# HugoVuach/Dense-linear-app

Measured on AMD Instinct MI355X. Metric: fp64 TFLOP/s for NxN SPD Cholesky (N^3/3 flops / factorisation time), higher is better.
Workload: dtype f64

## Files before the change

### dense_linear_app_amd/_lib.py

```python
from __future__ import annotations

import ctypes as C
import os

_HERE = os.path.dirname(os.path.abspath(__file__))
LIB_PATH = os.environ.get("LIBCHOLMI_PATH") or os.path.join(_HERE, "libcholmi.so")

_lib = None


class CholmiError(RuntimeError):

    def __init__(self, fn: str, code: int, msg: str):
        super().__init__(f"{fn} failed with status {code}: {msg}")
        self.fn, self.code, self.msg = fn, code, msg


def lib() -> C.CDLL:
    global _lib
    if _lib is not None:
        return _lib
    if not os.path.exists(LIB_PATH):
        raise ImportError(
            f"{LIB_PATH} is missing: build it with `python -c 'import __graft_entry__ as g; g.build()'` "
# ... 14 lines not shown
        "chol_desc_destroy": ([pp], i),
        "chol_potrf_tile": ([i, vp], i),
        "chol_trsm_tile": ([i, i, i, i, d, vp, vp], i),
        "chol_syrk_tile": ([i, i, d, vp, d, vp], i),
        "chol_gemm_tile": ([i, i, d, vp, vp, d, vp], i),
        "chol_plgsy_tile": ([d, i, vp, u64], i),
        "chol_lacpy_tile": ([i, vp, vp], i),
        "chol_lange_tile": ([i, vp, C.POINTER(d)], i),
        "chol_lauum_tile": ([i, vp], i),
        "chol_geadd_tile": ([i, d, vp, d, vp], i),
        "chol_potrs_tile": ([i, vp, vp], i),
        "chol_posv_tile": ([i, vp, vp], i),
        "chol_dsposv_tile": ([i, vp, vp, vp, C.POINTER(i)], i),
        "chol_last_dsposv_stats": ([C.POINTER(d)], i),
        "chol_trtri_tile": ([i, i, vp], i),
        "chol_potri_tile": ([i, vp], i),
        "chol_poinv_tile": ([i, vp], i),
        "chol_lansy_tile": ([i, i, vp, C.POINTER(d)], i),
        "chol_pocon_tile": ([i, vp, d, C.POINTER(d)], i),
        "chol_last_pocon_stats": ([C.POINTER(d)], i),
        "chol_poequ_tile": ([vp, vp, C.POINTER(d), C.POINTER(d)], i),
        "chol_laqsy_tile": ([i, vp, vp, d, d, C.POINTER(i)], i),
        "chol_porfs_tile": ([i, vp, vp, vp, vp, C.POINTER(d), C.POINTER(d)], i),
        "chol_posvx_tile": ([i, i, vp, vp, C.POINTER(i), vp, vp, vp, C.POINTER(d), C.POINTER(d), C.POINTER(d)], i),
        "chol_last_posvx_stats": ([C.POINTER(d)], i),
        "chol_bench_refine": ([i, vp, vp, vp, i, i, C.POINTER(d)], i),
        "chol_pstrf_tile": ([i, vp, C.POINTER(i), C.POINTER(i), d], i),
        "chol_last_pstrf_stats": ([C.POINTER(d)], i),
        "chol_sygst_tile": ([i, i, vp, vp], i),
        "chol_last_sygst_stats": ([C.POINTER(d)], i),
        "chol_sytrf_nopiv_tile": ([i, vp], i),
        "chol_sytrs_nopiv_tile": ([i, vp, vp], i),
        "chol_sysv_nopiv_tile": ([i, vp, vp], i),
        "chol_last_sytrf_stats": ([C.POINTER(d)], i),
        "chol_rbt_apply_tile": ([i, vp, vp, i], i),
        "chol_sytrf_rbt_tile": ([i, vp, vp, i, u64], i),
        "chol_sytrs_rbt_tile": ([i, vp, vp, i, vp], i),
        "chol_sysv_rbt_tile": ([i, vp, vp, vp, i, u64, vp, vp, C.POINTER(i), C.POINTER(d)], i),
        "chol_last_rbt_stats": ([C.POINTER(d)], i),
        "chol_lapack_to_tile": ([vp, i, vp], i),
        "chol_tile_to_lapack": ([vp, vp, i], i),
        "chol_tile_upload": ([vp, i, i, vp], i),
        "chol_tile_download": ([vp, i, i, vp], i),
        "chol_residual_plgsy": ([vp, d, u64, C.POINTER(d)], i),
        "chol_residual_plgsy_inf": ([vp, d, u64, C.POINTER(d)], i),
        "chol_make_spd_like_chameleon": ([vp, i, i, d, C.c_char, u64], None),
        "chol_enforce_strict_diag_dominance": ([vp, i, i, d], None),
        "chol_extract_block": ([vp, i, i, i, i, i, vp], None),
        "chol_parse_payloads": ([C.c_char_p, vp, i, vp, vp, vp, vp], i),
        "chol_debug_flow_waves": ([], i),
        "chol_last_potrf_regimes": ([C.POINTER(i), C.POINTER(i)], i),
        "chol_debug_schedule_check": ([i, i, d, d, i, C.c_char_p, i], i),
        "chol_debug_schedule_check_grid": ([i, i, i, i, i, d, d, i, C.c_char_p, i], i),
        "chol_debug_comm_trace": ([i, i, i, i, i, d, d, C.c_char_p, i], i),
        "chol_debug_task_record": ([i, i], i),
        "chol_debug_task_check": ([C.POINTER(C.c_longlong)], i),
        "chol_last_potrf_stats": ([C.POINTER(d), C.POINTER(d), C.POINTER(i), C.POINTER(d)], i),
        "chol_set_profiling": ([i], i),
        "chol_debug_stamps": ([i, C.POINTER(C.c_ulonglong), i], i),
        "chol_mfma_probe": ([i, i, C.POINTER(d)], i),
        "chol_bench_update": ([vp, i, i, i, C.POINTER(d), C.POINTER(d)], i),
        "chol_desc_local_ptr": ([vp, C.POINTER(C.c_size_t)], vp),
        "chol_desc_local_tiles": ([vp, C.POINTER(i), C.POINTER(i)], i),
        "chol_set_transport": ([vp], i),
        "chol_transport_rccl_unique_id": ([vp], i),
        "chol_transport_rccl_init": ([vp, i, i], i),
        "chol_transport_rccl_finalize": ([], i),
        "chol_transport_rccl_version": ([], i),
        "chol_set_transport_channel": ([i, vp], i),
        "chol_transport_selftest": ([i, C.c_size_t], i),
        "chol_set_transport_null": ([], i),
        "chol_dist_rehearse": ([i, i, i, i, i, d, u64, vp, C.POINTER(d)], i),
        "chol_desc_set_version": ([vp, u64], i),
        "chol_tile_batch": ([i, i, i, i, vp, vp, vp, vp, vp, i], i),
        "chol_sync": ([], i),
        "chol_potrf_batch": ([i, i, i, vp, vp, vp, C.POINTER(i), i], i),
        "chol_batch_info": ([i, C.POINTER(i)], i),
        "chol_batch_stats": ([C.POINTER(C.c_longlong)], i),
        "chol_batch_mark": ([C.POINTER(C.c_ulonglong)], i),
        "chol_batch_wait": ([C.POINTER(C.c_ulonglong)], i),
        "chol_debug_calibration": ([C.POINTER(d)], i),
        "chol_debug_update_kernel": ([i, C.c_char_p, i], i),
        "chol_debug_device_counters": ([], i),
        "chol_dist_last_stats": ([C.POINTER(d), C.POINTER(C.c_longlong), C.POINTER(C.c_longlong), C.POINTER(C.c_longlong)], i),
        "chol_dist_factorize_with": ([vp, vp, i, i, i, i, i, i], i),
        "chol_dist_gather_lower": ([vp, vp, i], i),
    }
    for name, (argt, rest) in sig.items():
        try:
            fn = getattr(L, name)
        except AttributeError:
            if os.environ.get("LIBCHOLMI_PATH"):
                continue
            raise
        fn.argtypes = argt
        fn.restype = rest
    _lib = L
    return L


ABI_SYMBOLS = None


def abi_symbols() -> list[str]:
    import re

    hdr = os.path.join(_HERE, "..", "include", "cholmi.h")
    text = open(hdr).read()
    text = re.sub(r"/\*.*?\*/", "", text, flags=re.S)
    return sorted(set(re.findall(r"\b(chol_[a-z_0-9]+)\s*\(", text)))


def check(fn: str, code: int) -> int:
    if code < 0:
        raise CholmiError(fn, code, lib().chol_last_error().decode(errors="replace"))
    return code
```

### dense_linear_app_amd/csrc/api.hip

```cpp
#include <hip/hip_runtime.h>

#include <algorithm>
#include <array>
#include <cmath>
#include <cstdarg>
#include <cstdio>
#include <cstdlib>
#include <cstring>
#include <deque>
#include <mutex>
#include <string>
#include <unordered_map>
#include <vector>

#include "../../include/cholmi.h"
#include "api_internal.h"
#include "cholmi_internal.h"

using namespace cholmi;

extern "C" int chol_internal_walk(chol_desc *d, void *base, cholmi::RankCtx *r, int rank);
extern "C" void chol_internal_dist_finalize(void);
extern "C" int chol_internal_desc_create(chol_desc_t **desc, void *mat, int dtype, int mb, int nb, int bsiz, int lm, int ln,
                                         int i, int j, int m, int n, int p, int q, int my_rank, int nranks);
// ... 651 lines not shown
  return through_lower(true, {A},
                       [&] { return A->dtype == CHOL_REAL_DOUBLE ? potrf_impl<double>(A) : potrf_impl<float>(A); });
}

void *DevPool::get(size_t bytes) {
  for (auto &b : blks)
    if (!b.used && b.bytes >= bytes) {
      b.used = true;
      return b.p;
    }
  void *p = nullptr;
  if (hipMalloc(&p, bytes) != hipSuccess) {
    (void)hipGetLastError();
    return nullptr;
  }
  blks.push_back({p, bytes, true});
  return p;
}
void DevPool::free_all() {
  for (auto &b : blks) (void)hipFree(b.p);
  blks.clear();
}

RankCtx *main_rank_ctx() { return &g.r; }
int main_rank(int *nranks) {
  if (nranks) *nranks = g.nranks;
  return g.rank;
}

int rank_ctx_create(RankCtx *r, int device, const RankCtx *calib_from) {
  r->device = device;
  int lo = 0, hi = 0;
  HIPCHECK(hipDeviceGetStreamPriorityRange(&lo, &hi));
  HIPCHECK(hipStreamCreateWithPriority(&r->st[ST_MAIN], hipStreamNonBlocking, lo));
  HIPCHECK(hipStreamCreateWithPriority(&r->st[ST_PANEL], hipStreamNonBlocking, hi));
  HIPCHECK(hipStreamCreateWithPriority(&r->st[ST_TRSM], hipStreamNonBlocking, hi));
  HIPCHECK(hipStreamCreateWithPriority(&r->st[ST_U1], hipStreamNonBlocking, lo - 1 > hi ? lo - 1 : hi));
  HIPCHECK(hipStreamCreateWithPriority(&r->st[ST_CX], hipStreamNonBlocking, hi));
  HIPCHECK(hipStreamCreateWithPriority(&r->st[ST_PX], hipStreamNonBlocking, hi));
  {
    {
      hipDeviceProp_t prop;
      HIPCHECK(hipGetDeviceProperties(&prop, device));
      unsigned long long *t = nullptr;
      HIPCHECK(hipMalloc(&t, 64));
      auto blocked = [&](int big, int small, bool *out) -> int {
        HIPCHECK(hipMemset(t, 0, 64));
        cholmi::launch_pipe_probe(r->st[big], r->st[small], t, prop.multiProcessorCount);
        HIPCHECK(hipStreamSynchronize(r->st[big]));
        HIPCHECK(hipStreamSynchronize(r->st[small]));
        unsigned long long h[2];
        HIPCHECK(hipMemcpy(h, t, sizeof h, hipMemcpyDeviceToHost));
        *out = h[1] > h[0] + 3000;
        return 0;
      };
      const int victims[4] = {ST_PANEL, ST_TRSM, ST_CX, ST_U1};
      const int mid = lo - 1 > hi ? lo - 1 : hi;
      const int prio_of[ST_COUNT] = {lo, hi, hi, mid, hi, hi};
      for (int vi = 0; vi < 4; ++vi) {
        const int v = victims[vi];
        for (int attempt = 0;; ++attempt) {
          bool b1 = false, b2 = false;
          int rc = blocked(ST_MAIN, v, &b1);
          if (rc) return rc;
          if (v != ST_U1) rc = blocked(ST_U1, v, &b2);
          if (rc) return rc;
          if (!b1 && !b2) break;
          if (attempt == 6) {
            ++r->stream_collisions;
            break;
          }
          r->retired.push_back(r->st[v]);
          HIPCHECK(hipStreamCreateWithPriority(&r->st[v], hipStreamNonBlocking, prio_of[v]));
          ++r->stream_swaps;
        }
      }
      (void)hipFree(t);
      if (getenv("CHOLMI_VERBOSE"))
        fprintf(stderr, "[cholmi] stream pipe probe: %d stream(s) replaced, %d pair(s) still colliding\n", r->stream_swaps, r->stream_collisions);
    }
  }
  r->winv_bytes = (size_t)32 * MACRO * MACRO * sizeof(double);
  HIPCHECK(hipMalloc(&r->winv, 2 * r->winv_bytes));
  HIPCHECK(hipMalloc(&r->d_info, sizeof(int)));
  HIPCHECK(hipMemset(r->d_info, 0, sizeof(int)));
  {
    const char *e = getenv("CHOLMI_DEVICE_FLAGS");
    if (!e || atoi(e) != 0) {
      HIPCHECK(hipMalloc(&r->d_sem, SEM_INTS * sizeof(int)));
      HIPCHECK(hipMemset(r->d_sem, 0, SEM_INTS * sizeof(int)));
      bool ok = true;
      const hipStream_t pairs[4][2] = {{r->st[ST_TRSM], r->st[ST_PANEL]}, {r->st[ST_U1], r->st[ST_TRSM]},
                                       {r->st[ST_PANEL], r->st[ST_U1]}, {r->st[ST_PANEL], r->st[ST_TRSM]}};
      for (int t = 0; t < 4 && ok; ++t) {
        int *sem = r->d_sem + 64 * t, *res = r->d_sem + 64 * t + 32;
        cholmi::launch_sem_probe(pairs[t][0], pairs[t][1], sem, res);
        HIPCHECK(hipStreamSynchronize(pairs[t][0]));
        HIPCHECK(hipStreamSynchronize(pairs[t][1]));
        int v = 0;
        HIPCHECK(hipMemcpy(&v, res, sizeof(int), hipMemcpyDeviceToHost));
        ok = (v == 1);
      }
      if (!ok) {
        (void)hipFree(r->d_sem);
        r->d_sem = nullptr;
      } else {
        r->flow_ok = true;
        const hipStream_t fpairs[2][2] = {{r->st[ST_CX], r->st[ST_PANEL]}, {r->st[ST_PANEL], r->st[ST_CX]}};
        for (int t = 0; t < 2 && r->flow_ok; ++t) {
          int *sem = r->d_sem + 64 * (4 + t), *res = r->d_sem + 64 * (4 + t) + 32;
          cholmi::launch_sem_probe(fpairs[t][0], fpairs[t][1], sem, res);
          HIPCHECK(hipStreamSynchronize(fpairs[t][0]));
          HIPCHECK(hipStreamSynchronize(fpairs[t][1]));
          int v = 0;
          HIPCHECK(hipMemcpy(&v, res, sizeof(int), hipMemcpyDeviceToHost));
          r->flow_ok = (v == 1);
        }
        HIPCHECK(hipMemset(r->d_sem, 0, 1024 * sizeof(int)));
      }
    }
  }
  if (calib_from) {
    for (int i = 0; i < 2; ++i) r->probe_tflops[i] = calib_from->probe_tflops[i], r->diag_us[i] = calib_from->diag_us[i];
    return 0;
  }
  if (const char *e = getenv("CHOLMI_CALIB")) {
    double v[4];
    if (sscanf(e, "%lf,%lf,%lf,%lf", &v[0], &v[1], &v[2], &v[3]) == 4) {
      r->probe_tflops[0] = v[0], r->diag_us[0] = v[1], r->probe_tflops[1] = v[2], r->diag_us[1] = v[3];
      return 0;
    }
  }
  int rc = mfma_probe_on(r, CHOL_REAL_DOUBLE, 4, 1000, &r->probe_tflops[0]);
  if (!rc) rc = mfma_probe_on(r, CHOL_REAL_FLOAT, 4, 2000, &r->probe_tflops[1]);
  if (!rc) rc = time_diag_step<double>(r, &r->diag_us[0]);
  if (!rc) rc = time_diag_step<float>(r, &r->diag_us[1]);
  return rc;
}

void rank_ctx_destroy(RankCtx *r) {
  for (auto e : r->events) (void)hipEventDestroy(e);
  r->events.clear();
  if (r->ev_flow) (void)hipEventDestroy(r->ev_flow);
  r->ev_flow = nullptr;
  r->pool.free_all();
  if (r->winv) (void)hipFree(r->winv);
  if (r->d_info) (void)hipFree(r->d_info);
  if (r->d_sem) (void)hipFree(r->d_sem);
  r->winv = nullptr;
  r->d_info = nullptr;
  r->d_sem = nullptr;
  for (int i = 0; i < ST_COUNT; ++i) {
    if (r->st[i]) (void)hipStreamDestroy(r->st[i]);
    r->st[i] = nullptr;
  }
  for (hipStream_t s : r->retired) (void)hipStreamDestroy(s);
  r->retired.clear();
}

}

extern "C" {

int chol_internal_fail(int code, const char *msg) { return fail(code, msg); }

const char *chol_version(void) { return "cholmi 0.3 (gfx950)"; }

const char *chol_last_error(void) {
  static thread_local std::string copy;
  std::lock_guard<std::mutex> lk(g_err_mu);
  copy = g.last_error;
  return copy.c_str();
}

int chol_set_device(int device) {
  std::lock_guard<std::recursive_mutex> lk(g_mu);
  if (g.inited && device != g.r.device) return fail(-1, "chol_set_device after chol_init");
  g.r.device = device;
  return 0;
}

int chol_set_rank(int rank, int nranks) {
  if (nranks < 1 || rank < 0 || rank >= nranks) return fail(-1, "chol_set_rank: bad rank");
  g.rank = rank;
  g.nranks = nranks;
  return 0;
}

int chol_init(int ncpu, int ngpu) {
  (void)ncpu;
  std::lock_guard<std::recursive_mutex> lk(g_mu);
  if (g.inited) return 0;
  if (ngpu < 1)
    return fail(CHOL_ERR_NO_GPU, "chol_init: ngpu must be >= 1 (this library has no CPU backend)");
  int count = 0;
  hipError_t e = hipGetDeviceCount(&count);
  if (e != hipSuccess || count < 1) {
    (void)hipGetLastError();
    return fail(CHOL_ERR_NO_GPU, "chol_init: no HIP device visible");
  }
  if (g.r.device < 0) {
    const char *lr = getenv("LOCAL_RANK");
    g.r.device = lr ? atoi(lr) % count : 0;
  }
  if (g.r.device >= count) return fail(CHOL_ERR_NO_GPU, "chol_init: device index out of range");
  HIPCHECK(hipSetDevice(g.r.device));
  if (const char *e = getenv("CHOLMI_TRSM_SMALL_MAX")) cholmi::g_trsm_small_max = atoi(e);
  {
    hipDeviceProp_t prop;
    HIPCHECK(hipGetDeviceProperties(&prop, g.r.device));
    const int room = (prop.multiProcessorCount - 32) / 4;
    cholmi::g_poll_max_wgs = room < 0 ? 0 : (room < 48 ? room : 48);
  }
  if (const char *e = getenv("CHOLMI_POLL_MAX_WGS")) cholmi::g_poll_max_wgs = atoi(e);
  if (const char *e = getenv("CHOLMI_FLOW")) cholmi::g_flow = atoi(e);
  if (const char *e = getenv("CHOLMI_FLOW_NBM")) {
    int lo = 0, hi = 0;
    if (sscanf(e, "%d:%d", &lo, &hi) == 2) cholmi::g_flow_min_nbm = std::max(2, lo), cholmi::g_flow_max_nbm = std::min(8, hi);
  }
  if (const char *e = getenv("CHOLMI_FLOW_FENCES")) cholmi::g_flow_fences = atoi(e);
  if (const char *e = getenv("CHOLMI_INTILE_FUSED")) cholmi::g_intile_fused = atoi(e);
  if (const char *e = getenv("CHOLMI_MIN_UNITS")) cholmi::g_min_units = atoi(e);
  HIPCHECK(hipMalloc(&g.d_acc, 2 * sizeof(double)));
  HIPCHECK(hipMalloc(&g.d_ytab, YTAB_ENTRIES * sizeof(int)));
  HIPCHECK(hipMemset(g.d_ytab, 0, YTAB_ENTRIES * sizeof(int)));
  cholmi::g_ytab = g.d_ytab;
  int rc = rank_ctx_create(&g.r, g.r.device, nullptr);
  if (rc) return rc;
  g.inited = true;
  return 0;
}

int chol_finalize(void) {
  std::lock_guard<std::recursive_mutex> lk(g_mu);
  if (!g.inited) return 0;
  (void)hipDeviceSynchronize();
  chol_internal_dist_finalize();
  g.stage.release();
  g.work.release();
  spd_release();
  if (g.wc_winv) (void)hipFree(g.wc_winv);
  g.wc_winv = nullptr;
  if (g.d_binfo) (void)hipFree(g.d_binfo);
  g.d_binfo = nullptr;
  tx_destroy();
  g.wc_ptr = nullptr;
  g.wc_version = 0;
  (void)hipFree(g.d_acc);
  if (g.d_ytab) (void)hipFree(g.d_ytab);
  g.d_ytab = nullptr;
  cholmi::g_ytab = nullptr;
  rank_ctx_destroy(&g.r);
  g.d_acc = nullptr;
  g.inited = false;
  return 0;
}

int chol_desc_create(chol_desc_t **desc, void *mat, int dtype, int mb, int nb, int bsiz, int lm,
                     int ln, int i, int j, int m, int n, int p, int q) {
  return chol_internal_desc_create(desc, mat, dtype, mb, nb, bsiz, lm, ln, i, j, m, n, p, q, g.rank, g.nranks);
}

int chol_internal_desc_create(chol_desc_t **desc, void *mat, int dtype, int mb, int nb, int bsiz, int lm, int ln,
                              int i, int j, int m, int n, int p, int q, int my_rank, int nranks) {
  if (!desc) return fail(-1, "desc_create: desc is NULL");
  *desc = nullptr;
  if (dtype != CHOL_REAL_DOUBLE && dtype != CHOL_REAL_FLOAT) return fail(-3, "desc_create: dtype");
  if (mb <= 0) return fail(-4, "desc_create: mb");
  if (nb <= 0) return fail(-5, "desc_create: nb");
  if (bsiz != mb * nb) return fail(-6, "desc_create: bsiz != mb*nb");
  if (lm <= 0) return fail(-7, "desc_create: lm");
  if (ln <= 0) return fail(-8, "desc_create: ln");
  if (i < 0 || i >= lm) return fail(-9, "desc_create: i");
  if (j < 0 || j >= ln) return fail(-10, "desc_create: j");
  if (m <= 0 || i + m > lm) return fail(-11, "desc_create: m");
  if (n <= 0 || j + n > ln) return fail(-12, "desc_create: n");
  if (p <= 0 || p > MAXP) return fail(-13, "desc_create: p");
  if (q <= 0) return fail(-14, "desc_create: q");
  if (!g.inited) return fail(CHOL_ERR_NOT_INITIALIZED, "desc_create before chol_init");
  void *view_user = nullptr;
  int view_lmt = 0, view_oi = 0, view_oj = 0;
  if (i != 0 || j != 0 || m != lm || n != ln) {
    if (p * q != 1) return fail(CHOL_ERR_NOT_SUPPORTED, "desc_create: sub-matrix views of distributed matrices are not supported");
    if (mat) {
      if (lm % mb || ln % nb || mb != nb)
        return fail(CHOL_ERR_NOT_SUPPORTED, "desc_create: a view over a user buffer needs a user matrix of whole square tiles (lm, ln multiples of mb = nb)");
      view_user = mat;
      view_lmt = lm / mb;
      view_oi = i;
      view_oj = j;
// ... 62 lines not shown
  if (multi || d->padded) {
    int rc = build_worklist(d);
    if (rc) {
      if (d->owns) (void)hipFree(d->mat);
      delete d;
      return rc;
    }
  }
  d->user_mat = view_user;
  d->user_lmt = view_lmt;
  d->user_i = view_oi;
  d->user_j = view_oj;
  *desc = d;
  return 0;
}

int chol_desc_destroy(chol_desc_t **desc) {
  if (!desc || !*desc) return fail(-1, "desc_destroy: NULL");
  chol_desc *d = *desc;
  if (d->owns) forget_winv(d->mat);
  if (d->d_list) (void)hipFree(d->d_list);
  if (d->owns && d->mat) (void)hipFree(d->mat);
  delete d;
  *desc = nullptr;
  return 0;
}

void *chol_desc_local_ptr(chol_desc_t *d, size_t *bytes) {
  if (!d) return nullptr;
  if (bytes) *bytes = (size_t)d->lmt * d->lnt * (size_t)d->bsizi * d->esize;
  return d->mat;
}

int chol_desc_local_tiles(chol_desc_t *d, int *lmt, int *lnt) {
  if (!d) return fail(-1, "NULL desc");
  if (lmt) *lmt = d->lmt;
  if (lnt) *lnt = d->lnt;
  return 0;
}

int chol_desc_set_version(chol_desc_t *d, unsigned long long version) {
  if (!d) return fail(-1, "desc_set_version: NULL descriptor");
  d->version = version;
  return 0;
}

int chol_sync(void) {
  if (tx_rec.on) {
    std::lock_guard<std::recursive_mutex> lk(g_mu);
    return tx_quiesce();
  }
  if (!g.inited) return fail(CHOL_ERR_NOT_INITIALIZED, "chol_sync before chol_init");
  std::lock_guard<std::recursive_mutex> lk(g_mu);
  HIPCHECK(hipStreamSynchronize(g.r.st[ST_MAIN]));
  return tx_quiesce();
}

}


template <typename T>
static int flush_pending_t() {
  const TaskExec::Pending p = tx.pend;
  tx.pend.on = false;
  hipStream_t s = tx.st[TaskExec::CHAIN];
  TXHIP(hipMemsetAsync(g.d_binfo + p.slot, 0, sizeof(int), s));
  TXHIP(hipMemcpyAsync(p.a_out, p.a_in, (size_t)p.mb * p.mb * sizeof(T), hipMemcpyDeviceToDevice, s));
  T *wset = reinterpret_cast<T *>(tx_winv_set());
  if (!tx_rec.on) launch_potrf_tile<T>(s, reinterpret_cast<T *>(p.a_out), p.mb, wset, g.d_binfo + p.slot, 0, tile_sems());
  forget_winv(p.a_out);
  tx_remember_winv(p.a_out, p.version, p.mb, p.dtype, wset);
  TXHIP(hipGetLastError());
  void *outs[1] = {p.a_out};
  return tx_commit(TaskExec::CHAIN, outs, 1, 0, 0);
}
namespace {
int tx_flush_pending() {
  if (!tx.ready || !tx.pend.on) return 0;
  return tx.pend.dtype == CHOL_REAL_DOUBLE ? flush_pending_t<double>() : flush_pending_t<float>();
}
}

template <typename T>
static int panel_fused_impl(int dtype, int mb, int n, const void *const *c_in, void *const *c_out) {
  const TaskExec::Pending p = tx.pend;
  tx.pend.on = false;
  const int X = TaskExec::CHAIN, nbm = mb / MACRO;
  hipStream_t sp = tx.st[X], st = tx.st_trsm;
  const size_t tb = (size_t)mb * mb * sizeof(T), lb = (size_t)n * sizeof(void *);
  size_t off = 0;
  int rc = tx_take(2 * lb, &off);
  if (rc) return rc;
  char *hl = tx.h_ring + off, *dl = tx.d_ring + off;
  memcpy(hl, c_in, lb);
  memcpy(hl + lb, c_out, lb);
  const void *const *ins[1] = {c_in};
  rc = tx_follow(X, ins, 1, n);
  if (rc) return rc;
  hipEvent_t ev_pre = tx.pev[34], ev_join = tx.pev[35];
  TXHIP(hipEventRecord(ev_pre, sp));
  TXHIP(hipStreamWaitEvent(st, ev_pre, 0));
  TXHIP(hipMemsetAsync(g.d_binfo + p.slot, 0, sizeof(int), sp));
  TXHIP(hipMemcpyAsync(p.a_out, p.a_in, tb, hipMemcpyDeviceToDevice, sp));
  TXHIP(hipMemcpyAsync(dl, hl, 2 * lb, hipMemcpyHostToDevice, st));
  T *wset = reinterpret_cast<T *>(tx_winv_set());
  if (!tx_rec.on) {
    launch_copy_ptrs(st, (const void *const *)dl, (void *const *)(dl + lb), n, (long)tb);
    launch_panel_pipelined<T>(sp, st, tx.pev, reinterpret_cast<T *>(p.a_out), mb, wset, g.d_binfo + p.slot, 0,
                              reinterpret_cast<T *>(c_out[0]), (long)mb * mb, n, nullptr, nullptr, nullptr, 0, tile_sems());
  }
  (void)nbm;
  TXHIP(hipEventRecord(ev_join, st));
  TXHIP(hipStreamWaitEvent(sp, ev_join, 0));
  forget_winv(p.a_out);
  for (int t = 0; t < n; ++t) forget_winv(c_out[t]);
  tx_remember_winv(p.a_out, p.version, mb, dtype, wset);
  TXHIP(hipGetLastError());
  ++tx.fused_panels;
  void *outs1[1] = {p.a_out};
  rc = tx_commit(X, outs1, 1, 0, 0);
  if (rc) return rc;
  if (tx_rec.on) tx_rec.rd.push_back(p.a_out);
  return tx_commit(X, c_out, n, off, off + 2 * lb);
}

template <typename T>
static int tile_batch_impl(int op, int dtype, int mb, int n, const void *const *c_in, const void *const *a, const void *const *b,
                           void *const *c_out, const unsigned long long *a_versions, int flags) {
  int rc = tx_init();
  if (rc) return rc;
  const bool update = op != CHOL_BATCH_TRSM;
  if (tx.pend.on) {
    bool fuse = !update && tx.pend.dtype == dtype && tx.pend.mb == mb;
    for (int t = 0; fuse && t < n; ++t)
      fuse = a[t] == tx.pend.a_out && (t == 0 || (const char *)c_out[t] == (const char *)c_out[t - 1] + (size_t)mb * mb * sizeof(T));
    if (fuse) return panel_fused_impl<T>(dtype, mb, n, c_in, c_out);
    rc = tx_flush_pending();
    if (rc) return rc;
  }
  const int X = (!update || (flags & CHOL_BATCH_URGENT)) ? TaskExec::CHAIN : TaskExec::BULK;
  hipStream_t s = tx.st[X];
  const size_t tb = (size_t)mb * mb * sizeof(T), lb = (size_t)n * sizeof(void *);
  size_t off = 0;
  rc = tx_take(4 * lb, &off);
  if (rc) return rc;
  char *hl = tx.h_ring + off, *dl = tx.d_ring + off;
  memcpy(hl, c_in, lb);
  memcpy(hl + lb, a, lb);
  if (op == CHOL_BATCH_SYRK || !b) memset(hl + 2 * lb, 0, lb);
  else memcpy(hl + 2 * lb, b, lb);
  memcpy(hl + 3 * lb, c_out, lb);
  const void *const *ins[3] = {c_in, a, op == CHOL_BATCH_SYRK ? nullptr : b};
  rc = tx_follow(X, ins, 3, n);
  if (rc) return rc;
  TXHIP(hipMemcpyAsync(dl, hl, 4 * lb, hipMemcpyHostToDevice, s));
  const void *const *d_cin = (const void *const *)dl, *const *d_a = (const void *const *)(dl + lb),
                    *const *d_b = (const void *const *)(dl + 2 * lb);
  void *const *d_out = (void *const *)(dl + 3 * lb);
  for (int t = 0; t < n; ++t) forget_winv(c_out[t]);
  if (update) {
    const int f = dtype == CHOL_REAL_DOUBLE ? 0 : 1;
    const double t_tile = 2.0 * mb * (double)mb * mb / (g.r.probe_tflops[f] * CHOLMI_UPDATE_EFF * 1e12);
    const double t_panel = g.r.diag_us[f] * 1e-6 * CHOLMI_STEP_FACTOR * (mb / MACRO);
    const bool yield = X == TaskExec::BULK && g.r.probe_tflops[f] > 0 && n * t_tile < g_task_yield_factor * t_panel;
    if (!tx_rec.on)
      launch_update_ptrs<T>(s, (const T *const *)d_cin, (const T *const *)d_a, (const T *const *)d_b, (T *const *)d_out, n, mb, yield);
  } else {
    if (!tx_rec.on) launch_copy_ptrs(s, d_cin, d_out, n, (long)tb);
    int t0 = 0;
    while (t0 < n) {
      int t1 = t0 + 1;
      while (t1 < n && a[t1] == a[t0] && (const char *)c_out[t1] == (const char *)c_out[t1 - 1] + tb) ++t1;
      const T *L = reinterpret_cast<const T *>(a[t0]);
      const T *w = reinterpret_cast<const T *>(tx_cached_winv(a[t0], a_versions ? a_versions[t0] : 0, mb, dtype));
      if (!w) w = reinterpret_cast<const T *>(cached_winv(a[t0], a_versions ? a_versions[t0] : 0, mb, dtype));
      if (!w) {
        T *wn = reinterpret_cast<T *>(tx_winv_set());
        if (!tx_rec.on) launch_invert_diag<T>(s, L, mb, wn);
        tx_remember_winv(a[t0], a_versions ? a_versions[t0] : 0, mb, dtype, wn);
        w = wn;
      }
      if (!tx_rec.on) launch_trsm_panel<T>(s, reinterpret_cast<T *>(c_out[t0]), (long)mb * mb, t1 - t0, L, w, mb, T(1));
      t0 = t1;
    }
  }
  TXHIP(hipGetLastError());
  return tx_commit(X, c_out, n, off, off + 4 * lb);
}

template <typename T>
static int potrf_batch_impl(int dtype, int mb, int n, const void *const *a_in, void *const *a_out,
                            const unsigned long long *versions, int *slots, bool defer) {
// ... 494 lines not shown
int chol_residual_plgsy(chol_desc_t *L, double bump, unsigned long long seed, double *rel) {
  return residual_common(L, bump, seed, rel, nullptr);
}

int chol_residual_plgsy_inf(chol_desc_t *L, double bump, unsigned long long seed, double *rel_inf) {
  return residual_common(L, bump, seed, nullptr, rel_inf);
}

int chol_last_potrf_stats(double *total_ms, double *update_ms, int *update_launches, double *update_flops) {
  if (total_ms) *total_ms = g.r.total_ms;
  if (update_ms) *update_ms = g.r.update_ms;
  if (update_launches) *update_launches = g.r.update_launches;
  if (update_flops) *update_flops = g.r.update_flops;
  return 0;
}

int chol_set_profiling(int on) {
  g.r.profiling = on != 0;
  return 0;
}

int chol_bench_update(chol_desc_t *d, int k, int ablate, int reps, double *ms, double *flops) {
  if (!g.inited) return fail(CHOL_ERR_NOT_INITIALIZED, "bench_update before chol_init");
  if (!d || !ms || d->p * d->q != 1 || !d->on_device || d->mt != d->nt || k < 0 || k + 1 >= d->nt || reps < 1)
    return fail(-1, "bench_update: arguments");
  if (ablate != 0)
    return fail(CHOL_ERR_NOT_SUPPORTED, "bench_update: ablate must be 0");
  std::lock_guard<std::recursive_mutex> lk(g_mu);
  int rc = ensure_events(2);
  if (rc) return rc;
  const PanelRef pan = one_panel((char *)d->mat + (size_t)k * d->nt * d->bsizi * d->esize);
  const LocalMat C = local_mat(d, d->mat);
  const ColRange rr = col_range(d, k + 1, d->nt);
  float best = 1e30f;
  for (int r = 0; r <= reps; ++r) {
    HIPCHECK(hipEventRecord(g.r.events[0], g.r.st[ST_MAIN]));
    if (d->dtype == CHOL_REAL_DOUBLE)
      launch_trail_update<double>(g.r.st[ST_MAIN], C, d->d_list, rr.off, rr.na, rr.offb, rr.nb, pan);
    else
      launch_trail_update<float>(g.r.st[ST_MAIN], C, d->d_list, rr.off, rr.na, rr.offb, rr.nb, pan);
    HIPCHECK(hipEventRecord(g.r.events[1], g.r.st[ST_MAIN]));
    HIPCHECK(hipStreamSynchronize(g.r.st[ST_MAIN]));
    float t = 0;
    HIPCHECK(hipEventElapsedTime(&t, g.r.events[0], g.r.events[1]));
    if (r > 0 && t < best) best = t;
  }
  *ms = best;
  const double ntl = (double)(d->nt - 1 - k);
  if (flops) *flops = (ntl * (ntl - 1) + ntl) * (double)d->mbi * d->mbi * d->mbi;
  return 0;
}

int chol_debug_stamps(int enable, unsigned long long *out, int max_pairs) {
  if (!g.inited) return fail(CHOL_ERR_NOT_INITIALIZED, "debug_stamps before chol_init");
  static unsigned long long *buf = nullptr;
  const size_t bytes = (1 + 8 * 1000) * sizeof(unsigned long long);
  HIPCHECK(hipDeviceSynchronize());
  if (enable) {
    if (!buf) HIPCHECK(hipMalloc(&buf, bytes));
    HIPCHECK(hipMemset(buf, 0, bytes));
    cholmi::g_dbg = buf;
    return 0;
  }
  int n = 0;
  if (buf && out) {
    std::vector<unsigned long long> h(1 + 8 * 1000);
    HIPCHECK(hipMemcpy(h.data(), buf, bytes, hipMemcpyDeviceToHost));
    n = (int)std::min<unsigned long long>(h[0], (unsigned long long)std::min(max_pairs, 1000));
    memcpy(out, h.data() + 1, (size_t)n * 8 * sizeof(unsigned long long));
  }
  cholmi::g_dbg = nullptr;
  return n;
}

int chol_mfma_probe(int dtype, int waves_per_simd, double *tflops) {
  if (!g.inited) return fail(CHOL_ERR_NOT_INITIALIZED, "mfma_probe before chol_init");
  if (!tflops || waves_per_simd < 1 || waves_per_simd > 8) return fail(-2, "mfma_probe: arguments");
  std::lock_guard<std::recursive_mutex> lk(g_mu);
  return mfma_probe_on(&g.r, dtype, waves_per_simd, 4000, tflops);
}

int chol_debug_device_counters(void) { return g.inited && g.r.d_sem ? 1 : 0; }

int chol_debug_update_kernel(int dtype, char *buf, int buflen) {
  if (!buf || buflen < 8) return fail(-2, "debug_update_kernel: buffer");
  const bool f64 = dtype == CHOL_REAL_DOUBLE;
  if (!f64 && dtype != CHOL_REAL_FLOAT) return fail(-1, "debug_update_kernel: dtype");
  snprintf(buf, buflen, f64 ? "cholmi::k_trail_update_w8<double, 3>" : "cholmi::k_trail_update_w8f");
  return 0;
}

int chol_debug_flow_waves(void) { return g.r.flow_waves; }

int chol_last_potrf_regimes(int *out8, int *nt) {
  if (!out8) return fail(-1, "last_potrf_regimes: NULL");
  for (int i = 0; i < 8; ++i) out8[i] = g.r.regimes[i];
  if (nt) *nt = g.r.regimes_nt;
  return 0;
}

int chol_debug_calibration(double *out8) {
  if (!g.inited) return fail(CHOL_ERR_NOT_INITIALIZED, "debug_calibration before chol_init");
  if (!out8) return fail(-1, "debug_calibration: NULL");
  for (int i = 0; i < 2; ++i) {
    out8[2 * i] = g.r.probe_tflops[i];
    out8[2 * i + 1] = g.r.diag_us[i];
    out8[4 + 2 * i] = g.r.probe_tflops[i] * CHOLMI_UPDATE_EFF;
    out8[5 + 2 * i] = g.r.diag_us[i] * CHOLMI_STEP_FACTOR;
  }
  return 0;
}

}
```

### dense_linear_app_amd/csrc/cholmi_internal.h

```cpp
#pragma once
#include <hip/hip_runtime.h>
#include <stdint.h>
#include <algorithm>
#include <vector>

#include "../../include/cholmi.h"

struct chol_desc {
  int dtype, mb, nb, bsiz, lm, ln, i, j, m, n, p, q;
  int mbi, bsizi;
  bool padded;
  int mt, nt;
  int prow, pcol;
  int lmt, lnt;
  size_t esize;
  void *mat;
  bool on_device;
  bool owns;
  int2 *d_list = nullptr;
  std::vector<int> ge, gd;
  int n_off = 0;
  unsigned long long version = 0;
  void *user_mat = nullptr;
  int user_lmt = 0;
  int user_i = 0, user_j = 0;
};

extern "C" int chol_internal_fail(int code, const char *msg);

namespace cholmi {

enum { ST_MAIN = 0, ST_PANEL, ST_TRSM, ST_U1, ST_CX, ST_PX, ST_COUNT };

constexpr int SEM_SLOTS = 65536;
constexpr int TILE_SEM_SETS = 8;
constexpr int SEM_INTS = (SEM_SLOTS + TILE_SEM_SETS * 32) * 32;

struct DevPool {
  struct Blk {
    void *p;
    size_t bytes;
    bool used;
  };
  std::vector<Blk> blks;
  void *get(size_t bytes);
  void release_all() {
    for (auto &b : blks) b.used = false;
  }
  void free_all();
};

struct RankCtx {
  int device = -1;
  hipStream_t st[ST_COUNT] = {};
  void *winv = nullptr;
  size_t winv_bytes = 0;
  int *d_info = nullptr;
  int *d_sem = nullptr;
  bool flow_ok = false;
  unsigned tile_sem_next = 0;
  std::vector<hipEvent_t> events;
  std::vector<hipStream_t> retired;
  int stream_swaps = 0;
  int stream_collisions = 0;
  hipEvent_t ev_flow = nullptr;
  bool profiling = false;
  double total_ms = 0, update_ms = 0, update_flops = 0, issue_us = 0;
  int update_launches = 0;
  int flow_waves = 0;
  int regimes[8] = {};
  int regimes_nt = 0;
  long long sends = 0, recvs = 0, bytes_sent = 0;
  DevPool pool;
  double probe_tflops[2] = {0, 0}, diag_us[2] = {0, 0};
};
int rank_ctx_create(RankCtx *r, int device, const RankCtx *calib_from);
void rank_ctx_destroy(RankCtx *r);
RankCtx *main_rank_ctx();
int main_rank(int *nranks);

constexpr double CHOLMI_UPDATE_EFF = 0.85, CHOLMI_STEP_FACTOR = 2.65;

constexpr int MACRO = 128;
constexpr int MAXP = 8;

struct PanelRef {
  const void *base[MAXP];
  int first[MAXP];
  int P;
};

struct LocalMat {
  void *base;
  int lmt;
  int P, Q;
  int mb;
  long bsiz;
};

extern int g_trsm_small_max;
extern int g_poll_max_wgs;
bool flow_applies(int nbm);
extern int g_flow;
extern int g_flow_min_nbm;
extern int g_flow_max_nbm;
extern int g_flow_fences;
extern int g_intile_fused;
extern int g_min_units;
extern unsigned long long *g_dbg;
extern int *g_ytab;
constexpr int YTAB_ENTRIES = 2048;

template <typename T>
void launch_trail_update(hipStream_t s, const LocalMat &C, const int2 *d_list, int off, int na, int offb,
                         int nb, const PanelRef &pan, bool yield = false, const PanelRef *pan2 = nullptr);

template <typename T>
void launch_syr2k_update(hipStream_t s, const LocalMat &C, const int2 *d_list, int off, int na, int offb, int nb,
                         const PanelRef &pan, const PanelRef &qan);

template <typename T>
void launch_ldl_update(hipStream_t s, const LocalMat &C, const int2 *d_list, int off, int na, int offb, int nb,
                       const PanelRef &pan, const PanelRef &qan);

template <typename T>
void launch_potrf_tile(hipStream_t s, T *tile, int mb, T *winv, int *d_info, int info_base, int *sem = nullptr);

template <typename T>
void launch_diag_syrk(hipStream_t s, T *C, const T *A, int mb);

void launch_sem_probe(hipStream_t consumer, hipStream_t producer, int *sem, int *result);
void launch_pipe_probe(hipStream_t big, hipStream_t small, unsigned long long *t, int cus);

struct SyrkPipe {
  void *c;
  hipStream_t su;
  int *sem;
  int *fc = nullptr;
  hipStream_t sflow = nullptr;
  hipEvent_t ev_flow = nullptr;
  bool join_flow = false;
};
inline int flow_ctl_lines(int nbm) { return nbm >= 2 && nbm <= 8 ? 1 + nbm + 2 * nbm * nbm : 0; }

template <typename T>
void launch_panel_pipelined(hipStream_t sp, hipStream_t st, hipEvent_t *ev, T *lkk, int mb, T *winv,
                            int *d_info, int info_base, T *tiles, long bsiz, int ntiles,
                            hipEvent_t ev_head = nullptr, const SyrkPipe *sy = nullptr, const int *wait_sem = nullptr,
                            int wait_target = 0, int *tile_sem = nullptr);

template <typename T>
void launch_col_update_small(hipStream_t s, T *C, const T *A, const T *B, int mb, int ntiles, long bsiz, int *done);

template <typename T>
void launch_invert_diag(hipStream_t s, const T *tile, int mb, T *winv);
template <typename T>
void launch_invert_diag_batch(hipStream_t s, const T *A, long tstride, int nt, int mb, T *winv);

template <typename T>
void launch_trsm_panel(hipStream_t s, T *tiles, long bsiz, int ntiles, const T *lkk, const T *winv,
                       int mb, T alpha);

template <typename T>
void launch_gemm_nt_tile(hipStream_t s, const T *A, const T *B, T *C, int mb, T alpha, T beta,
                         bool lower_only);

template <typename T>
void launch_gemm_nt_batch(hipStream_t s, const T *A, long sA, int nz1, const T *B, long sB, int nz2, T *C, long sC1,
                          long sC2, int mb, T alpha, T beta);

template <typename T>
void launch_update_ptrs(hipStream_t s, const T *const *cin, const T *const *a, const T *const *b, T *const *cout, int n, int mb,
                        bool yield);
void launch_copy_ptrs(hipStream_t s, const void *const *src, void *const *dst, int n, long bytes);

template <typename T>
void launch_plgsy(hipStream_t s, const LocalMat &A, int lnt, int prow, int pcol, double bump,
                  unsigned long long seed, int mbu, long nglob, int side);

template <typename T>
void launch_residual(hipStream_t s, const T *Lbase, int Nb, int mb, double bump,
                     unsigned long long seed, double *d_acc, int mbu, long nglob,
                     double *rowsum = nullptr);

template <typename T>
void launch_pad_identity(hipStream_t s, T *dst, int n, int ldp);

template <typename T>
void launch_transpose_inplace(hipStream_t s, T *M, int nt, int mb);

struct TileGeo {
  int lmt, lnt, mbs, mbu;
  long m, n;
};
template <typename T>
void launch_lacpy(hipStream_t s, const TileGeo &g, int side, const T *A, T *B);
template <typename T>
void launch_geadd(hipStream_t s, const TileGeo &g, double alpha, const T *A, double beta, T *B);
template <typename T>
void launch_lange(hipStream_t s, const TileGeo &g, int kind, const T *A, double *work);
template <typename T>
void launch_lauum_lower(hipStream_t s, const T *L, T *out, int nt, int mbs);

int sym_resid_width(int nrhs);
size_t sym_resid_part_bytes(const TileGeo &ga, int nrhs);
void launch_sym_resid(hipStream_t s, const TileGeo &ga, int upper, const double *A, const TileGeo &gx, const double *X,
                      const double *B, double *part, float *Rf, unsigned long long *colmax, int *flag);
void launch_sym_resid_f64(hipStream_t s, const TileGeo &ga, int upper, const double *A, const TileGeo &gx,
                          const double *X, const double *B, double *part, double *R, unsigned long long *colmax);
void launch_sym_inf_norm(hipStream_t s, const TileGeo &ga, int upper, const double *A, double *part,
                         unsigned long long *colmax);
void launch_sym_to_f32(hipStream_t s, const TileGeo &ga, int upper, const double *A, float *Af, int *flag);
void launch_vec_to_f32(hipStream_t s, const TileGeo &gx, const double *B, float *Bf, int *flag);
void launch_vec_update(hipStream_t s, const TileGeo &gx, const float *C, double *X, bool assign);

template <typename T>
struct TriLevel {
  T *base;
  long si, sj, sz;
  int ld;
  const T *dg;
  long dsi, dsz;
  int dld;
  T *y;
  long ysi, ysz;
  int E;
};
template <typename T>
void launch_tri_column(hipStream_t s, const TriLevel<T> &L, int n, int nbatch, int c);
template <typename T>
void launch_tri_put_diag(hipStream_t s, T *A, long tstride, int mb, int nt, const T *winv);
template <typename T>
void launch_diag_zero(hipStream_t s, const T *A, long tstride, int mbs, int mbu, long n, int *first);

int condest_edge(const TileGeo &g);
size_t condest_vec_elems(const TileGeo &g);
size_t lansy_part_bytes(const TileGeo &g);
template <typename T>
void launch_lansy(hipStream_t s, const TileGeo &g, int upper, const T *A, double *part, double *res);
template <typename T>
void launch_stage_diag(hipStream_t s, const TileGeo &g, int upper, const T *A, T *Dv);
template <typename T>
struct SweepBufs {
  T *x, *y, *pg, *pd;
// ... 93 lines not shown
```

### dense_linear_app_amd/csrc/dist.hip

```cpp
#include <hip/hip_runtime.h>

#include <dlfcn.h>

#include <condition_variable>
#include <cstdio>
#include <deque>
#include <map>
#include <mutex>
#include <string>
#include <thread>
#include <tuple>
#include <vector>

#if __has_include(<rccl/rccl.h>)
#include <rccl/rccl.h>
#define CHOLMI_RCCL_HEADER 1
#else
typedef struct {
  char internal[128];
} ncclUniqueId;
typedef void *ncclComm_t;
typedef int ncclResult_t;
enum { ncclInt8 = 0, ncclInt64 = 4 };
enum { ncclMax = 2 };
// ... 11 lines not shown
                                         int i, int j, int m, int n, int p, int q, int rank, int nranks);

namespace {

int hip_fail(hipError_t e, const char *what) {
  char buf[256];
  snprintf(buf, sizeof buf, "%s failed (walker): %s", what, hipGetErrorString(e));
  return chol_internal_fail(CHOL_ERR_HIP, buf);
}
#define HIPRC(call)                                      \
  do {                                                   \
    hipError_t e_ = (call);                              \
    if (e_ != hipSuccess) return hip_fail(e_, #call);    \
  } while (0)

struct ColRange {
  int off, na, offb, nb;
};
inline ColRange col_range(const chol_desc *d, int jlo, int jhi) {
  jlo = std::min(jlo, d->nt), jhi = std::min(jhi, d->nt);
  ColRange r;
  r.off = d->ge[jhi];
  r.na = d->ge[jlo] - d->ge[jhi];
  r.offb = d->n_off + d->gd[jhi];
  r.nb = d->gd[jlo] - d->gd[jhi];
  return r;
}

template <typename T>
struct HipOps {
  RankCtx &r;
  chol_desc *d;
  char *base;
  const WaveGeo &g;
  bool reset_ytab;
  bool sem_ok = false;
  LocalMat C;
  HipOps(RankCtx &rc, chol_desc *desc, void *b, const WaveGeo &geo, bool ry) : r(rc), d(desc), base((char *)b), g(geo), reset_ytab(ry) {
    C.base = b;
    C.lmt = desc->lmt;
    C.P = desc->p;
    C.Q = desc->q;
    C.mb = desc->mbi;
    C.bsiz = desc->bsizi;
  }
  bool profiling() const { return r.profiling; }
  bool pipe_ok() const { return true; }
  bool counters() const { return sem_ok; }
  bool can_split_trsm() const { return true; }
  void *stream(int st) { return r.st[st]; }
  char *tile(int il, int jl) { return base + ((size_t)il + (size_t)jl * g.lmt) * g.tile_bytes; }
  void *winv(int par) { return (char *)r.winv + (size_t)par * r.winv_bytes; }
  void *alloc(size_t bytes) { return r.pool.get(bytes); }
  int *sem(int k, int which, int per_wave) { return r.d_sem + ((size_t)per_wave * k + which) * 32; }
  bool flow_ok() const { return r.flow_ok; }
  void *flow_event() {
    if (!r.ev_flow) (void)hipEventCreateWithFlags(&r.ev_flow, hipEventDisableTiming);
    return r.ev_flow;
  }
  int launched() {
    const hipError_t e = hipGetLastError();
    return e == hipSuccess ? 0 : hip_fail(e, "kernel launch");
  }
  int begin(int nevents, int nt, int sem_per_wave) {
    while ((int)r.events.size() < nevents) {
      hipEvent_t e;
      HIPRC(hipEventCreate(&e));
      r.events.push_back(e);
    }
    HIPRC(hipMemsetAsync(r.d_info, 0, sizeof(int), r.st[ST_MAIN]));
    if (g_ytab && reset_ytab) HIPRC(hipMemsetAsync(g_ytab, 0, YTAB_ENTRIES * sizeof(int), r.st[ST_MAIN]));
    sem_ok = r.d_sem && (long)nt * sem_per_wave <= SEM_SLOTS;
    if (sem_ok) HIPRC(hipMemsetAsync(r.d_sem, 0, (size_t)nt * sem_per_wave * 32 * sizeof(int), r.st[ST_MAIN]));
    return 0;
  }
  int rec(int ev, int st) {
    HIPRC(hipEventRecord(r.events[ev], r.st[st]));
    return 0;
  }
  int wt(int st, int ev) {
    HIPRC(hipStreamWaitEvent(r.st[st], r.events[ev], 0));
    return 0;
  }
  int panel(int k, char *lkk, void *wv, char *tiles, int ntiles, int ev_steps, int ev_head, const SyrkPipe *sy,
            const int *wait_sem, int wait_target) {
    launch_panel_pipelined<T>(r.st[ST_PANEL], r.st[ST_TRSM], &r.events[ev_steps], (T *)lkk, g.mb, (T *)wv, r.d_info,
                              k * g.mb, (T *)tiles, (long)g.mb * g.mb, ntiles, ev_head >= 0 ? r.events[ev_head] : nullptr,
                              sy, wait_sem, wait_target);
    return launched();
  }
  int trsm(int, char *tiles, int ntiles, const char *lkk, const char *wv, int st) {
    launch_trsm_panel<T>(r.st[st], (T *)tiles, (long)g.mb * g.mb, ntiles, (const T *)lkk, (const T *)wv, g.mb, T(1));
    return launched();
  }
  int diag_syrk(int, int, char *Cjj, const char *A, int st) {
    launch_diag_syrk<T>(r.st[st], (T *)Cjj, (const T *)A, g.mb);
    return launched();
  }
  int update(int, int, int jlo, int jhi, int what, const PanelRef &p1, const PanelRef *p2, bool yield, int st) {
    const ColRange c = col_range(d, jlo, jhi);
    launch_trail_update<T>(r.st[st], C, d->d_list, c.off, (what & 1) ? c.na : 0, c.offb, (what & 2) ? c.nb : 0, p1, yield, p2);
    return launched();
  }
  int update_col_small(int k, int st) {
    launch_col_update_small<T>(r.st[st], (T *)tile(k + 2, k + 1), (const T *)tile(k + 2, k), (const T *)tile(k + 1, k), g.mb,
                               g.nt - k - 2, (long)g.mb * g.mb, nullptr);
    return launched();
  }
  int finish(int ev_start, int ev_stop, const std::vector<std::pair<int, int>> &brackets, int *info) {
    HIPRC(hipStreamSynchronize(r.st[ST_MAIN]));
    float ms = 0;
    HIPRC(hipEventElapsedTime(&ms, r.events[ev_start], r.events[ev_stop]));
    r.total_ms = ms;
    r.update_ms = 0;
    if (r.profiling) {
      std::vector<std::pair<float, float>> iv;
      for (auto &b : brackets) {
        float t0 = 0, t1 = 0;
        if (hipEventElapsedTime(&t0, r.events[ev_start], r.events[b.first]) != hipSuccess ||
            hipEventElapsedTime(&t1, r.events[ev_start], r.events[b.second]) != hipSuccess) {
          (void)hipGetLastError();
          continue;
        }
        if (t1 > t0) iv.emplace_back(t0, t1);
      }
      std::sort(iv.begin(), iv.end());
      float hi = -1;
      for (auto &p : iv) {
        if (p.first > hi) r.update_ms += p.second - p.first;
        else if (p.second > hi) r.update_ms += p.second - hi;
        hi = std::max(hi, p.second);
      }
    }
    HIPRC(hipMemcpy(info, r.d_info, sizeof(int), hipMemcpyDeviceToHost));
    return 0;
  }
};

struct CbOps {
  chol_test_engine_t cb;
  const WaveGeo &g;
  CbOps(const chol_test_engine_t &c, const WaveGeo &geo) : cb(c), g(geo) {}
  bool profiling() const { return false; }
  bool pipe_ok() const { return false; }
  bool counters() const { return false; }
  bool can_split_trsm() const { return false; }
  void *stream(int) { return nullptr; }
  char *tile(int il, int jl) { return (char *)cb.store + ((size_t)il + (size_t)jl * g.lmt) * g.tile_bytes; }
  void *winv(int) { return nullptr; }
  void *alloc(size_t bytes) { return cb.alloc(cb.ctx, bytes); }
  int *sem(int, int, int) { return nullptr; }
  bool flow_ok() const { return false; }
  void *flow_event() { return nullptr; }
  int update_col_small(int, int) { return 0; }
  int begin(int, int, int) { return 0; }
  int rec(int, int) { return 0; }
  int wt(int, int) { return 0; }
  int panel(int k, char *lkk, void *, char *, int ntiles, int, int, const SyrkPipe *, const int *, int) {
    WRC(cb.potrf(cb.ctx, k, lkk));
    return ntiles > 0 ? cb.trsm(cb.ctx, k, lkk) : 0;
  }
  int trsm(int k, char *, int, const char *lkk, const char *, int) { return cb.trsm(cb.ctx, k, lkk); }
  int diag_syrk(int k, int j, char *, const char *A, int) {
    std::vector<const void *> hb(g.P, A);
    std::vector<int> hf(g.P, 0);
    hf[j % g.P] = j / g.P;
    return cb.update_diag(cb.ctx, k, j, hb.data(), hf.data());
  }
  int update(int k1, int k2, int jlo, int jhi, int what, const PanelRef &p1, const PanelRef *p2, bool, int) {
    const PanelRef *ps[2] = {&p1, p2};
    const int ks[2] = {k1, k2};
    for (int t = 0; t < 2; ++t) {
      if (!ps[t] || ks[t] < 0) continue;
      if (what == 3) {
        WRC(cb.update(cb.ctx, ks[t], jlo, jhi, ps[t]->base, ps[t]->first, 0));
      } else if (what == 1) {
        if (jhi != jlo + 1) return chol_internal_fail(-1, "CbOps: off-diagonal-only update of more than one column");
        WRC(cb.update(cb.ctx, ks[t], jlo, jhi, ps[t]->base, ps[t]->first, 1));
      } else if (what == 2) {
        for (int j = jlo; j < std::min(jhi, g.nt); ++j)
          if (j % g.P == g.pr && j % g.Q == g.pc) WRC(cb.update_diag(cb.ctx, ks[t], j, ps[t]->base, ps[t]->first));
      }
    }
    return 0;
  }
  int finish(int, int, const std::vector<std::pair<int, int>> &, int *info) {
    *info = cb.info(cb.ctx);
    return 0;
  }
};

chol_transport_t g_tr[2];
bool g_tr_set = false;

struct Rccl {
  void *lib = nullptr;
  ncclComm_t comm[2] = {nullptr, nullptr};
  int which[2] = {0, 1};
  ncclResult_t (*GetVersion)(int *) = nullptr;
  ncclResult_t (*GetUniqueId)(ncclUniqueId *) = nullptr;
  ncclResult_t (*CommInitRank)(ncclComm_t *, int, ncclUniqueId, int) = nullptr;
  ncclResult_t (*CommDestroy)(ncclComm_t) = nullptr;
  ncclResult_t (*GroupStart)() = nullptr;
  ncclResult_t (*GroupEnd)() = nullptr;
  ncclResult_t (*Send)(const void *, size_t, decltype(ncclInt8), int, ncclComm_t, hipStream_t) = nullptr;
  ncclResult_t (*Recv)(void *, size_t, decltype(ncclInt8), int, ncclComm_t, hipStream_t) = nullptr;
  ncclResult_t (*AllReduce)(const void *, void *, size_t, decltype(ncclInt8), decltype(ncclMax), ncclComm_t, hipStream_t) = nullptr;
  const char *(*GetErrorString)(ncclResult_t) = nullptr;
  long long *d_red = nullptr;
  int version = 0;
} g_rccl;

int rccl_fail(const char *what, int rc) {
  char buf[256];
  snprintf(buf, sizeof buf, "RCCL %s failed: %s", what, g_rccl.GetErrorString ? g_rccl.GetErrorString((ncclResult_t)rc) : "?");
  return chol_internal_fail(CHOL_ERR_HIP, buf);
}
int rccl_load() {
  if (g_rccl.lib) return 0;
  const char *names[] = {"librccl.so", "librccl.so.1"};
  for (int pass = 0; pass < 2 && !g_rccl.lib; ++pass)
    for (const char *n : names) {
      g_rccl.lib = dlopen(n, RTLD_NOW | RTLD_GLOBAL | (pass == 0 ? RTLD_NOLOAD : 0));
      if (g_rccl.lib) break;
    }
  if (!g_rccl.lib) g_rccl.lib = dlopen("/opt/rocm/lib/librccl.so.1", RTLD_NOW | RTLD_GLOBAL);
  if (!g_rccl.lib) return chol_internal_fail(CHOL_ERR_NOT_SUPPORTED, "librccl.so not found");
#define SYM(field, name)                                                  \
  *(void **)(&g_rccl.field) = dlsym(g_rccl.lib, name);                    \
  if (!g_rccl.field) return chol_internal_fail(CHOL_ERR_NOT_SUPPORTED, "librccl.so lacks " name)
  SYM(GetVersion, "ncclGetVersion");
  SYM(GetUniqueId, "ncclGetUniqueId");
  SYM(CommInitRank, "ncclCommInitRank");
  SYM(CommDestroy, "ncclCommDestroy");
  SYM(GroupStart, "ncclGroupStart");
  SYM(GroupEnd, "ncclGroupEnd");
  SYM(Send, "ncclSend");
  SYM(Recv, "ncclRecv");
  SYM(AllReduce, "ncclAllReduce");
  SYM(GetErrorString, "ncclGetErrorString");
#undef SYM
  int v = 0;
  const int rc = g_rccl.GetVersion(&v);
  if (rc) return rccl_fail("ncclGetVersion", rc);
  g_rccl.version = v;
// ... 521 lines not shown
```

### dense_linear_app_amd/csrc/kernels.hip

```cpp
#include "cholmi_internal.h"
#include "mfma_traits.h"

#include <type_traits>

#if defined(__HIP_DEVICE_COMPILE__) && !defined(__gfx950__)
#error "libcholmi's kernels target gfx950 (MI355X) only: build with --offload-arch=gfx950"
#endif

namespace cholmi {

constexpr int BK = 16;
constexpr int LROW = MACRO + 16;

template <int I, int N, typename F>
__device__ __forceinline__ void static_for(F &&f) {
  if constexpr (I < N) {
    f(std::integral_constant<int, I>{});
    static_for<I + 1, N>(f);
  }
}


template <typename T>
struct alignas(16) Smem {
  T a[2][BK][LROW];
  T b[2][BK][LROW];
};

template <typename T, bool MASKA, bool MASKB>
__device__ __forceinline__ void nt_kloop(const T *__restrict__ A, int lda, const T *__restrict__ B,
                                         int ldb, int K, Acc<T> &acc, Smem<T> &sm, int amask,
                                         int bmask) {
  using vec_t = typename Tr<T>::vec_t;
  constexpr int EPV = Tr<T>::EPV;
  constexpr int TPC = MACRO / EPV;
  constexpr int CPP = 256 / TPC;
  constexpr int NP = BK / CPP;
  const int t = threadIdx.x, lane = t & 63, w = t >> 6, wr = w & 1, wc = w >> 1;
  const int lrow = (t % TPC) * EPV, lcol = t / TPC;
  vec_t ra[NP], rb[NP];

  auto gload = [&](int k0) {
#pragma unroll
    for (int p = 0; p < NP; ++p) {
      const int kk = k0 + p * CPP + lcol;
      ra[p] = *reinterpret_cast<const vec_t *>(A + lrow + (size_t)kk * lda);
      rb[p] = *reinterpret_cast<const vec_t *>(B + lrow + (size_t)kk * ldb);
      if (MASKA) {
#pragma unroll
        for (int e = 0; e < EPV; ++e)
          if (kk > amask + lrow + e) ra[p][e] = T(0);
      }
      if (MASKB) {
#pragma unroll
        for (int e = 0; e < EPV; ++e)
          if (kk > bmask + lrow + e) rb[p][e] = T(0);
      }
    }
  };
  auto lstore = [&](int buf) {
#pragma unroll
    for (int p = 0; p < NP; ++p) {
      *reinterpret_cast<vec_t *>(&sm.a[buf][p * CPP + lcol][lrow]) = ra[p];
      *reinterpret_cast<vec_t *>(&sm.b[buf][p * CPP + lcol][lrow]) = rb[p];
    }
  };

  gload(0);
  lstore(0);
  __syncthreads();
  const int nk = K / BK;
  for (int kt = 0; kt < nk; ++kt) {
    const int cur = kt & 1;
    if (kt + 1 < nk) gload((kt + 1) * BK);
    T af[4], bf[4];
#pragma unroll
    for (int ks = 0; ks < BK / 4; ++ks) {
      const int kk = ks * 4 + (lane >> 4);
#pragma unroll
      for (int a = 0; a < 4; ++a) af[a] = sm.a[cur][kk][wr * 64 + a * 16 + (lane & 15)];
#pragma unroll
      for (int b = 0; b < 4; ++b) bf[b] = sm.b[cur][kk][wc * 64 + b * 16 + (lane & 15)];
      if (ks == BK / 4 - 1 && kt + 1 < nk) lstore(cur ^ 1);
#pragma unroll
// ... 388 lines not shown
      mfma_rest(0);
      __builtin_amdgcn_sched_barrier(0);
      KSTAMP(st, 4 + 5 * s + 2);
      __builtin_amdgcn_s_waitcnt(VMCNT0 + ((j < 2 || MORE) ? 2 : 0));
      if ((j & 1) && yslot && __builtin_amdgcn_readfirstlane(guest) != 0) yield_to_guest(yslot);
      asm volatile("s_barrier" ::: "memory");
      KSTAMP(st, 4 + 5 * s + 3);
      KSTAMP(st, 4 + 5 * s + 4);
      __builtin_amdgcn_sched_barrier(0);
      acc[0][0] = Tr<T>::mfma(fb[1][0], fa[1][0][0], acc[0][0]);
      __builtin_amdgcn_sched_barrier(0);
      if (j < NST - 1 || MORE) fread(0, (j + 1) % NST, 0);
      if (!(j & 1)) guest = __hip_atomic_load(poll, __ATOMIC_RELAXED, __HIP_MEMORY_SCOPE_AGENT);
      if (j == 0 || MORE) dma((j + 3) % NST);
      __builtin_amdgcn_sched_barrier(0);
      KSTAMP(st, 4 + 5 * s + 1);
      mfma_rest(1);
      __builtin_amdgcn_sched_barrier(0);
    });
  };
  int s0 = 0;
  for (; s0 < ns - NST; s0 += NST) quad(s0, std::true_type{});
  quad(s0, std::false_type{});
#ifdef CHOLMI_KLOOP_STAMPS
  if (kst_on && lane == 0) {
    kst[2] = __builtin_amdgcn_s_memtime();
    kst[3] = __builtin_amdgcn_s_memrealtime();
  }
#endif
}
#ifdef CHOLMI_KLOOP_STAMPS
}
extern "C" __attribute__((visibility("default"))) int chol_debug_kloop_stamps(unsigned long long *out, int n) {
  const int all = cholmi::KST_WGS * 8 * cholmi::KST_REC;
  if (n > all) n = all;
  if (hipDeviceSynchronize() != hipSuccess ||
      hipMemcpyFromSymbol(out, HIP_SYMBOL(cholmi::g_kloop_stamps), (size_t)n * sizeof(unsigned long long)) != hipSuccess)
    return -1;
  return n;
}
namespace cholmi {
#endif

template <typename T, bool OOP>
__device__ __forceinline__ void w8_epilogue(const T *Cin, T *Cout, int ld,
                                            typename Tr<T>::acc_t (&acc)[4][2], bool lower) {
  using vec_t = typename Tr<T>::vec_t;
  const int t = threadIdx.x, lane = t & 63, w = t >> 6, wr = w & 1, wc = w >> 1, i = lane & 15, q = lane >> 4;
  const int m0 = wr * 64 + 2 * i;
#pragma unroll
  for (int b = 0; b < 2; ++b) {
    vec_t cv[4][2];
#pragma unroll
    for (int r = 0; r < 4; ++r)
#pragma unroll
      for (int g = 0; g < 2; ++g)
        cv[r][g] = *reinterpret_cast<const vec_t *>(Cin + (long)(wc * 32 + 2 * (q + 4 * r) + b) * ld + m0 + 32 * g);
#pragma unroll
    for (int r = 0; r < 4; ++r) {
      const int n = wc * 32 + 2 * (q + 4 * r) + b;
      T *col = Cout + (long)n * ld;
#pragma unroll
      for (int g = 0; g < 2; ++g) {
        const int m = m0 + 32 * g;
        vec_t v = cv[r][g];
        if (OOP && lower && m < n) {
          if (m + 1 >= n) v[1] -= acc[2 * g + 1][b][r];
          *reinterpret_cast<vec_t *>(col + m) = v;
          continue;
        }
        v[0] -= acc[2 * g][b][r];
        v[1] -= acc[2 * g + 1][b][r];
        if (!lower || m >= n) {
          *reinterpret_cast<vec_t *>(col + m) = v;
        } else {
          if (m + 1 >= n) col[m + 1] = v[1];
        }
      }
    }
    __builtin_amdgcn_sched_barrier(0);
  }
}

constexpr int BKF = 32;
struct alignas(16) SmemF {
  float a[2][BKF][MACRO];
  float b[2][BKF][MACRO];
};
typedef float f2_t __attribute__((ext_vector_type(2)));

__device__ __forceinline__ void nt_kloop_w8f(const float *__restrict__ A, int lda, const float *__restrict__ B,
                                             int ldb, int K, f4_t (&acc)[4][2], SmemF &sm, const int *yslot) {
  const int t = threadIdx.x, lane = t & 63, w = t >> 6, wr = w & 1, wc = w >> 1, i = lane & 15, q = lane >> 4;
  constexpr int PIECES = BKF * MACRO * 4 / 1024, EPP = 256;
  auto dma = [&](int buf, int k0) {
#pragma unroll
    for (int p = 0; p < PIECES / 8; ++p) {
      const int piece = p * 8 + w;
      const int e = piece * EPP + lane * 4;
      const int kk = e / MACRO, r = e % MACRO;
      __builtin_amdgcn_global_load_lds(
          (const __attribute__((address_space(1))) void *)(A + r + (size_t)(k0 + kk) * lda),
          (__attribute__((address_space(3))) void *)(&sm.a[buf][0][0] + piece * EPP), 16, 0, 0);
      __builtin_amdgcn_global_load_lds(
          (const __attribute__((address_space(1))) void *)(B + ((r + 32 * (kk & 1)) & (MACRO - 1)) + (size_t)(k0 + kk) * ldb),
          (__attribute__((address_space(3))) void *)(&sm.b[buf][0][0] + piece * EPP), 16, 0, 0);
    }
  };
  f4_t fa[2];
  f2_t fb[2];
  const int arow = wr * 64 + 4 * i, brow = (wc * 32 + 2 * i - 32 * (q & 1)) & (MACRO - 1);
  auto fread = [&](int set, int cur, int ks) {
    fa[set] = *reinterpret_cast<const f4_t *>(&sm.a[cur][ks * 4 + q][arow]);
    fb[set] = *reinterpret_cast<const f2_t *>(&sm.b[cur][ks * 4 + q][brow]);
  };
  dma(0, 0);
  __syncthreads();
  const int nk = K / BKF;
  for (int kt = 0; kt < nk; ++kt) {
    const int cur = kt & 1;
    int guest = 0;
    if (yslot) guest = __hip_atomic_load(yslot, __ATOMIC_RELAXED, __HIP_MEMORY_SCOPE_AGENT);
    fread(0, cur, 0);
    if (kt + 1 < nk) dma(cur ^ 1, (kt + 1) * BKF);
#pragma unroll
    for (int ks = 0; ks < BKF / 4; ++ks) {
      __builtin_amdgcn_sched_barrier(0);
      acc[0][0] = Tr<float>::mfma(fb[ks & 1][0], fa[ks & 1][0], acc[0][0]);
      __builtin_amdgcn_sched_barrier(0);
      if (ks + 1 < BKF / 4) fread((ks + 1) & 1, cur, ks + 1);
      __builtin_amdgcn_sched_barrier(0);
#pragma unroll
      for (int a = 0; a < 4; ++a)
#pragma unroll
        for (int b = 0; b < 2; ++b)
          if (a + b > 0) acc[a][b] = Tr<float>::mfma(fb[ks & 1][b], fa[ks & 1][a], acc[a][b]);
      __builtin_amdgcn_sched_barrier(0);
    }
    if (yslot && __builtin_amdgcn_readfirstlane(guest) != 0) yield_to_guest(yslot);
    __syncthreads();
  }
}

template <bool OOP>
__device__ __forceinline__ void w8f_epilogue(const float *Cin, float *Cout, int ld, f4_t (&acc)[4][2], bool lower) {
  const int t = threadIdx.x, lane = t & 63, w = t >> 6, wr = w & 1, wc = w >> 1, i = lane & 15, q = lane >> 4;
  const int m0 = wr * 64 + 4 * i;
  f4_t cv[2][4];
#pragma unroll
  for (int b = 0; b < 2; ++b)
#pragma unroll
    for (int r = 0; r < 4; ++r)
      cv[b][r] = *reinterpret_cast<const f4_t *>(Cin + (long)(wc * 32 + 2 * (4 * q + r) + b) * ld + m0);
#pragma unroll
  for (int b = 0; b < 2; ++b)
#pragma unroll
    for (int r = 0; r < 4; ++r) {
      const int n = wc * 32 + 2 * (4 * q + r) + b;
      float *col = Cout + (long)n * ld;
      f4_t v = cv[b][r];
      if (OOP && lower && m0 < n) {
#pragma unroll
        for (int a = 0; a < 4; ++a)
          if (m0 + a >= n) v[a] -= acc[a][b][r];
        *reinterpret_cast<f4_t *>(col + m0) = v;
        continue;
      }
#pragma unroll
      for (int a = 0; a < 4; ++a) v[a] -= acc[a][b][r];
      if (!lower || m0 >= n) {
        *reinterpret_cast<f4_t *>(col + m0) = v;
      } else {
#pragma unroll
        for (int a = 0; a < 4; ++a)
          if (m0 + a >= n) col[m0 + a] = v[a];
      }
    }
}

template <typename T_, int MODE>
struct CoreW8 {
  using T = T_;
  using Smem = SmemR<T>;
  using Acc = typename Tr<T>::acc_t[4][2];
  static __device__ __forceinline__ void kloop(const T *A, int lda, const T *B, int ldb, int K, Acc &acc, Smem &sm,
                                               const int *yslot) {
    nt_kloop_w8<T, MODE>(A, lda, B, ldb, K, acc, sm, yslot);
  }
  template <bool OOP>
  static __device__ __forceinline__ void epilogue(const T *Cin, T *Cout, int ld, Acc &acc, bool lower) {
    w8_epilogue<T, OOP>(Cin, Cout, ld, acc, lower);
  }
};
struct CoreW8F {
  using T = float;
  using Smem = SmemF;
  using Acc = f4_t[4][2];
  static __device__ __forceinline__ void kloop(const float *A, int lda, const float *B, int ldb, int K, Acc &acc,
                                               Smem &sm, const int *yslot) {
    nt_kloop_w8f(A, lda, B, ldb, K, acc, sm, yslot);
  }
  template <bool OOP>
  static __device__ __forceinline__ void epilogue(const float *Cin, float *Cout, int ld, Acc &acc, bool lower) {
    w8f_epilogue<OOP>(Cin, Cout, ld, acc, lower);
  }
};

template <typename Core>
__device__ __forceinline__ void update_list_block(const LocalMat &C, const int2 *list, int na, int offb, int nb,
                                                  int blocks_a, int nbm, int unit, const int *ytab,
                                                  typename Core::Smem &sm, const PanelRef &P1, const PanelRef &Q1,
                                                  const PanelRef &P2, const PanelRef &Q2, int npairs) {
  using T = typename Core::T;
  BlockMap bm;
  if (!map_update_block(list, na, offb, nb, nbm, blocks_a, unit, bm)) return;
  const int2 ij = bm.ij;
  const int mi = bm.mi, mj = bm.mj;
  const bool lower = (ij.x == ij.y) && mi == mj;
  T *Cp = reinterpret_cast<T *>(C.base) + ((long)(ij.x / C.P) + (long)(ij.y / C.Q) * C.lmt) * C.bsiz + mi * MACRO +
          (long)mj * MACRO * C.mb;
  typename Core::Acc acc;
#pragma unroll
  for (int a = 0; a < 4; ++a)
#pragma unroll
    for (int b = 0; b < 2; ++b)
#pragma unroll
      for (int r = 0; r < 4; ++r) acc[a][b][r] = T(0);
  const int *yslot = ytab ? ytab + cu_slot() : nullptr;
  Core::kloop(panel_tile<T>(P1, ij.x, C.bsiz) + mi * MACRO, C.mb, panel_tile<T>(Q1, ij.y, C.bsiz) + mj * MACRO, C.mb, C.mb,
              acc, sm, yslot);
  if (npairs > 1)
    Core::kloop(panel_tile<T>(P2, ij.x, C.bsiz) + mi * MACRO, C.mb, panel_tile<T>(Q2, ij.y, C.bsiz) + mj * MACRO, C.mb,
                C.mb, acc, sm, yslot);
  Core::template epilogue<false>(Cp, Cp, C.mb, acc, lower);
}

template <typename T, int MODE>
__global__ __launch_bounds__(512, 4) void k_trail_update_w8(LocalMat C, const int2 *__restrict__ list, int na,
                                                             int offb, int nb, int blocks_a, PanelRef pan, int nbm,
                                                             int unit, const int *ytab, PanelRef pan2, int npan) {
  __shared__ SmemR<T> sm;
  update_list_block<CoreW8<T, MODE>>(C, list, na, offb, nb, blocks_a, nbm, unit, ytab, sm, pan, pan, pan2, pan2, npan);
}
__global__ __launch_bounds__(512, 4) void k_trail_update_w8f(LocalMat C, const int2 *__restrict__ list, int na,
                                                              int offb, int nb, int blocks_a, PanelRef pan, int nbm,
                                                              int unit, const int *ytab, PanelRef pan2, int npan) {
  __shared__ SmemF sm;
  update_list_block<CoreW8F>(C, list, na, offb, nb, blocks_a, nbm, unit, ytab, sm, pan, pan, pan2, pan2, npan);
}

template <typename T, int MODE>
__global__ __launch_bounds__(512, 4) void k_syr2k_w8(LocalMat C, const int2 *__restrict__ list, int na, int offb,
                                                     int nb, int blocks_a, PanelRef pan, PanelRef qan, int nbm,
                                                     int unit) {
  __shared__ SmemR<T> sm;
  update_list_block<CoreW8<T, MODE>>(C, list, na, offb, nb, blocks_a, nbm, unit, nullptr, sm, pan, qan, qan, pan, 2);
}
__global__ __launch_bounds__(512, 4) void k_syr2k_w8f(LocalMat C, const int2 *__restrict__ list, int na, int offb,
                                                      int nb, int blocks_a, PanelRef pan, PanelRef qan, int nbm,
                                                      int unit) {
  __shared__ SmemF sm;
  update_list_block<CoreW8F>(C, list, na, offb, nb, blocks_a, nbm, unit, nullptr, sm, pan, qan, qan, pan, 2);
}

template <typename T, int MODE>
__global__ __launch_bounds__(512, 4) void k_ldl_update_w8(LocalMat C, const int2 *__restrict__ list, int na, int offb,
                                                          int nb, int blocks_a, PanelRef pan, PanelRef qan, int nbm,
                                                          int unit) {
  __shared__ SmemR<T> sm;
  update_list_block<CoreW8<T, MODE>>(C, list, na, offb, nb, blocks_a, nbm, unit, nullptr, sm, pan, qan, pan, qan, 1);
}
__global__ __launch_bounds__(512, 4) void k_ldl_update_w8f(LocalMat C, const int2 *__restrict__ list, int na, int offb,
                                                           int nb, int blocks_a, PanelRef pan, PanelRef qan, int nbm,
                                                           int unit) {
  __shared__ SmemF sm;
  update_list_block<CoreW8F>(C, list, na, offb, nb, blocks_a, nbm, unit, nullptr, sm, pan, qan, pan, qan, 1);
}

__device__ __forceinline__ bool map_ptr_block(int n, int nbm, int unit, int &t, int &mi, int &mj) {
  const int b = blockIdx.x, x = b & 7, sidx = b >> 3, MT = nbm * nbm;
  const long lin = ((long)(sidx / unit) * 8 + x) * unit + sidx % unit;
  if (lin >= (long)n * MT) return false;
  t = (int)(lin / MT);
  const int macro = (int)(lin - (long)t * MT);
  mi = macro % nbm;
  mj = macro / nbm;
  return true;
}
// ... 11 lines not shown
                                                 typename Core::Smem &sm) {
  int t, mi, mj;
  if (!map_ptr_block(n, nbm, unit, t, mi, mj)) return;
  const T *A = ap[t], *B = bp[t];
  const bool syrk = B == nullptr;
  const long off = mi * MACRO + (long)mj * MACRO * mb;
  const T *Ci = cin[t] + off;
  T *Co = cout[t] + off;
  if (syrk && mi < mj) {
    copy_block_512<T>(Ci, Co, mb);
    return;
  }
  if (syrk) B = A;
  typename Core::Acc acc;
#pragma unroll
  for (int a = 0; a < 4; ++a)
#pragma unroll
    for (int b = 0; b < 2; ++b)
#pragma unroll
      for (int r = 0; r < 4; ++r) acc[a][b][r] = T(0);
  const int *yslot = ytab ? ytab + cu_slot() : nullptr;
  Core::kloop(A + mi * MACRO, mb, B + mj * MACRO, mb, mb, acc, sm, yslot);
  Core::template epilogue<true>(Ci, Co, mb, acc, syrk && mi == mj);
}
template <typename T, int MODE>
__global__ __launch_bounds__(512, 4) void k_update_ptrs_w8(const T *const *__restrict__ cin, const T *const *__restrict__ ap,
                                                            const T *const *__restrict__ bp, T *const *__restrict__ cout,
                                                            int n, int mb, int nbm, int unit, const int *ytab) {
  __shared__ SmemR<T> sm;
  update_ptr_block<CoreW8<T, MODE>>(cin, ap, bp, cout, n, mb, nbm, unit, ytab, sm);
}
__global__ __launch_bounds__(512, 4) void k_update_ptrs_w8f(const float *const *__restrict__ cin, const float *const *__restrict__ ap,
                                                             const float *const *__restrict__ bp, float *const *__restrict__ cout,
                                                             int n, int mb, int nbm, int unit, const int *ytab) {
  __shared__ SmemF sm;
  update_ptr_block<CoreW8F>(cin, ap, bp, cout, n, mb, nbm, unit, ytab, sm);
}

template <typename T>
__global__ __launch_bounds__(256, 2) void k_panel_solve(T *tiles, long bsiz, int mb, int nbm, int r0,
                                                        int s, const T *__restrict__ winv, T alpha,
                                                        int *ytab, const int *wait_sem = nullptr,
                                                        int wait_target = 0, int *fail = nullptr,
                                                        int *head_sem = nullptr) {
  __shared__ SmemP<T> sm;
  sem_wait(wait_sem, wait_target, fail);
  GuestOnCu guest(ytab);
  __builtin_amdgcn_s_setprio(2);
  const int nr = nbm - r0;
  const int tix = blockIdx.x / nr, r = r0 + blockIdx.x % nr;
  T *Ap = tiles + (long)tix * bsiz + r * MACRO + (long)s * MACRO * mb;
  const T *Bp = winv + (long)s * MACRO * MACRO;
  Acc<T> acc;
  acc_zero<T>(acc);
  nt_kloop_paired<T>(Ap, mb, Bp, MACRO, MACRO, acc, sm);
  nt_epilogue_paired<T>(Ap, mb, acc, alpha, T(0), false);
  guest.leave();
  if (tix == 0) sem_signal(head_sem);
}

template <typename T>
__global__ __launch_bounds__(256, 2) void k_panel_update(T *tiles, long bsiz, int mb, int nbm, int s,
                                                         const T *__restrict__ lkk, T beta, int *ytab,
                                                         const int *wait_sem = nullptr, int wait_target = 0,
                                                         int *fail = nullptr) {
  __shared__ SmemP<T> sm;
  sem_wait(wait_sem, wait_target, fail);
  GuestOnCu guest(ytab);
  __builtin_amdgcn_s_setprio(2);
  const int nc = nbm - 1 - s;
  int b = blockIdx.x;
  const int c = s + 1 + b % nc;
  b /= nc;
  const int r = b % nbm, tix = b / nbm;
  T *tile = tiles + (long)tix * bsiz;
  const T *Ap = tile + r * MACRO + (long)s * MACRO * mb;
  const T *Bp = lkk + c * MACRO + (long)s * MACRO * mb;
  T *Cp = tile + r * MACRO + (long)c * MACRO * mb;
  Acc<T> acc;
  acc_zero<T>(acc);
  nt_kloop_paired<T>(Ap, mb, Bp, mb, MACRO, acc, sm);
  nt_epilogue_paired<T>(Cp, mb, acc, T(-1), beta, false);
  guest.leave();
}

constexpr int SK = 32;
template <typename T, int ROWS>
struct SmallImg {
  T v[SK][ROWS + 16];
};
template <typename T, int ROWS>
__device__ __forceinline__ void small_gload(const T *__restrict__ P, int ld, int k0, T (&r)[ROWS * SK / 256]) {
#pragma unroll
  for (int q = 0; q < ROWS * SK / 256; ++q) {
    const int e = threadIdx.x + 256 * q;
    r[q] = P[(e % ROWS) + (long)(k0 + e / ROWS) * ld];
  }
}
template <typename T, int ROWS>
__device__ __forceinline__ void small_lstore(SmallImg<T, ROWS> &img, const T (&r)[ROWS * SK / 256]) {
#pragma unroll
  for (int q = 0; q < ROWS * SK / 256; ++q) {
    const int e = threadIdx.x + 256 * q;
    img.v[e / ROWS][e % ROWS] = r[q];
  }
}
template <typename T, int RA, int RB>
__device__ __forceinline__ void small_mma(const SmallImg<T, RA> &ia, const SmallImg<T, RB> &ib, int i0, int j0,
                                          typename Tr<T>::acc_t (&acc)[2][2]) {
  const int lane = threadIdx.x & 63, lo = lane & 15, kq = lane >> 4;
#pragma unroll
  for (int ks = 0; ks < SK / 4; ++ks) {
    const int k = 4 * ks + kq;
    T af[2], bf[2];
#pragma unroll
    for (int a = 0; a < 2; ++a) af[a] = ia.v[k][i0 + 16 * a + lo];
#pragma unroll
    for (int b = 0; b < 2; ++b) bf[b] = ib.v[k][j0 + 16 * b + lo];
#pragma unroll
    for (int a = 0; a < 2; ++a)
#pragma unroll
      for (int b = 0; b < 2; ++b) acc[a][b] = Tr<T>::mfma(bf[b], af[a], acc[a][b]);
  }
}

template <typename T>
__global__ __launch_bounds__(256, 2) void k_solve_small(T *tiles, long bsiz, int mb, int nbm, int r0, int s,
                                                        const T *__restrict__ winv, T alpha, int *ytab,
                                                        const int *wait_sem = nullptr, int wait_target = 0,
                                                        int *fail = nullptr, int *head_sem = nullptr) {
  __shared__ SmallImg<T, 32> ia;
  __shared__ SmallImg<T, MACRO> ib;
  sem_wait(wait_sem, wait_target, fail);
  GuestOnCu guest(ytab);
  __builtin_amdgcn_s_setprio(2);
  const int per_tile = 4 * (nbm - r0);
  const int tix = blockIdx.x / per_tile, slab = blockIdx.x % per_tile;
  T *Ap = tiles + (long)tix * bsiz + (long)r0 * MACRO + 32 * slab + (long)s * MACRO * mb;
  const T *Bp = winv + (long)s * MACRO * MACRO;
  const int lane = threadIdx.x & 63, w = threadIdx.x >> 6, lo = lane & 15;
  T ra[32 * SK / 256], rb[MACRO * SK / 256];
  typename Tr<T>::acc_t acc[2][2];
#pragma unroll
  for (int a = 0; a < 2; ++a)
#pragma unroll
    for (int b = 0; b < 2; ++b)
#pragma unroll
      for (int r = 0; r < 4; ++r) acc[a][b][r] = T(0);
  small_gload<T, 32>(Ap, mb, 0, ra);
  small_gload<T, MACRO>(Bp, MACRO, 0, rb);
  for (int ph = 0; ph < MACRO / SK; ++ph) {
    small_lstore<T, 32>(ia, ra);
    small_lstore<T, MACRO>(ib, rb);
    __syncthreads();
    if (ph + 1 < MACRO / SK) {
      small_gload<T, 32>(Ap, mb, (ph + 1) * SK, ra);
      small_gload<T, MACRO>(Bp, MACRO, (ph + 1) * SK, rb);
    }
    small_mma<T, 32, MACRO>(ia, ib, 0, 32 * w, acc);
    __syncthreads();
  }
#pragma unroll
  for (int a = 0; a < 2; ++a)
#pragma unroll
    for (int b = 0; b < 2; ++b)
#pragma unroll
// ... 1141 lines not shown
    red[0][w] = num;
    red[1][w] = den;
  }
  __syncthreads();
  if (t == 0) {
    atomicAdd(&acc_out[0], red[0][0] + red[0][1] + red[0][2] + red[0][3]);
    atomicAdd(&acc_out[1], red[1][0] + red[1][1] + red[1][2] + red[1][3]);
  }
}

template <typename T>
__global__ __launch_bounds__(256) void k_transpose_inplace(T *M, int nt, int mb) {
  __shared__ T sa[64][65], sb[64][65];
  const int nsub = mb / 64;
  const long per_pair = (long)nsub * nsub;
  const long pair = blockIdx.x / per_pair, sub = blockIdx.x % per_pair;
  int I = (int)((sqrt(8.0 * (double)pair + 1.0) - 1.0) * 0.5);
  while ((long)I * (I + 1) / 2 > pair) --I;
  while ((long)(I + 1) * (I + 2) / 2 <= pair) ++I;
  const int J = (int)(pair - (long)I * (I + 1) / 2);
  const int si = (int)(sub % nsub), sj = (int)(sub / nsub);
  if (I == J && si < sj) return;
  const long bsiz = (long)mb * mb;
  T *ta = M + ((long)I + (long)J * nt) * bsiz + si * 64 + (long)sj * 64 * mb;
  T *tb = M + ((long)J + (long)I * nt) * bsiz + sj * 64 + (long)si * 64 * mb;
  const int tx = threadIdx.x & 63, ty = threadIdx.x >> 6;
  for (int c = ty; c < 64; c += 4) {
    sa[c][tx] = ta[tx + (long)c * mb];
    sb[c][tx] = tb[tx + (long)c * mb];
  }
  __syncthreads();
  for (int c = ty; c < 64; c += 4) {
    ta[tx + (long)c * mb] = sb[tx][c];
    tb[tx + (long)c * mb] = sa[tx][c];
  }
}

template <typename T>
void launch_transpose_inplace(hipStream_t s, T *M, int nt, int mb) {
  const long pairs = (long)nt * (nt + 1) / 2, nsub = mb / 64;
  k_transpose_inplace<T><<<dim3((unsigned)(pairs * nsub * nsub)), 256, 0, s>>>(M, nt, mb);
}
template void launch_transpose_inplace<double>(hipStream_t, double *, int, int);
template void launch_transpose_inplace<float>(hipStream_t, float *, int, int);

template <typename T>
__global__ void k_pad_identity(T *dst, int n, int ldp) {
  const int i = n + blockIdx.x * blockDim.x + threadIdx.x;
  if (i < ldp) dst[i + (size_t)i * ldp] = T(1);
}

__global__ __launch_bounds__(256) void k_pipe_big(unsigned long long *t, int spin_ticks) {
  __shared__ char lds[65536];
  lds[threadIdx.x] = 1;
  const unsigned long long t0 = __builtin_amdgcn_s_memrealtime();
  if (blockIdx.x == 0 && threadIdx.x == 0) t[0] = t0;
  while (__builtin_amdgcn_s_memrealtime() - t0 < (unsigned long long)spin_ticks) __builtin_amdgcn_s_sleep(16);
  if (lds[(threadIdx.x + 1) & 255] == 7) t[2] = 0;
}
__global__ void k_pipe_small(unsigned long long *t) {
  if (threadIdx.x == 0) t[1] = __builtin_amdgcn_s_memrealtime();
}
void launch_pipe_probe(hipStream_t big, hipStream_t small, unsigned long long *t, int cus) {
  k_pipe_big<<<8 * cus, 256, 0, big>>>(t, 2000);
  k_pipe_small<<<1, 64, 0, small>>>(t);
}

void launch_sem_probe(hipStream_t consumer, hipStream_t producer, int *sem, int *result) {
  k_sem_probe_wait<<<1, 1, 0, consumer>>>(sem, result);
  k_sem_probe_set<<<1, 64, 0, producer>>>(sem);
}

int *g_ytab = nullptr;
unsigned long long *g_dbg = nullptr;
int g_min_units = 128;
int g_intile_fused = 1;
constexpr int INTILE_FUSED_MAX = 256;
bool flow_applies(int nbm) { return g_flow && nbm >= g_flow_min_nbm && nbm <= g_flow_max_nbm; }
int g_flow = 1;
int g_flow_min_nbm = 3, g_flow_max_nbm = 4;
int g_flow_fences = 0;
int g_poll_max_wgs = 48;
int g_trsm_small_max = 64;

struct UpdateGrid {
  int unit;
  long blocks_a, blocks_b;
};
inline UpdateGrid update_grid(long tot_a, long tot_b, bool single_diag) {
  UpdateGrid u;
  u.unit = 64;
  while (u.unit > 8 && (tot_a + tot_b) / u.unit < g_min_units) u.unit >>= 1;
  u.blocks_a = ((tot_a + u.unit - 1) / u.unit + 7) / 8 * 8 * u.unit;
  u.blocks_b = ((tot_b + u.unit - 1) / u.unit + 7) / 8 * 8 * u.unit;
  if (single_diag) u.blocks_a = 0, u.blocks_b = tot_b;
  return u;
}

struct UpdateLaunch {
  int offb, nbm, blocks_a, unit;
  dim3 grid;
};
inline UpdateLaunch update_launch(const LocalMat &C, int off, int na, int offb, int nb) {
  const int nbm = C.mb / MACRO, MT = nbm * nbm, MTd = nbm * (nbm + 1) / 2;
  const UpdateGrid u = update_grid((long)na * MT, (long)nb * MTd, na == 0 && nb == 1);
  return {offb - off, nbm, (int)u.blocks_a, u.unit, dim3((unsigned)(u.blocks_a + u.blocks_b))};
}

template <typename T>
void launch_trail_update(hipStream_t s, const LocalMat &C, const int2 *d_list, int off, int na, int offb,
                         int nb, const PanelRef &pan, bool yield, const PanelRef *pan2) {
  if (na + nb <= 0) return;
  const int npan = pan2 ? 2 : 1;
  const PanelRef &p2 = pan2 ? *pan2 : pan;
  const UpdateLaunch l = update_launch(C, off, na, offb, nb);
  if constexpr (sizeof(T) == 4)
    k_trail_update_w8f<<<l.grid, dim3(512), 0, s>>>(C, d_list + off, na, l.offb, nb, l.blocks_a, pan, l.nbm, l.unit,
                                                   yield ? g_ytab : nullptr, p2, npan);
  else
    k_trail_update_w8<T, 3><<<l.grid, dim3(512), 0, s>>>(C, d_list + off, na, l.offb, nb, l.blocks_a, pan, l.nbm, l.unit,
                                                         yield ? g_ytab : nullptr, p2, npan);
}

template <typename T>
void launch_syr2k_update(hipStream_t s, const LocalMat &C, const int2 *d_list, int off, int na, int offb, int nb,
                         const PanelRef &pan, const PanelRef &qan) {
  if (na + nb <= 0) return;
  const UpdateLaunch l = update_launch(C, off, na, offb, nb);
  if constexpr (sizeof(T) == 4)
    k_syr2k_w8f<<<l.grid, dim3(512), 0, s>>>(C, d_list + off, na, l.offb, nb, l.blocks_a, pan, qan, l.nbm, l.unit);
  else
    k_syr2k_w8<T, 3><<<l.grid, dim3(512), 0, s>>>(C, d_list + off, na, l.offb, nb, l.blocks_a, pan, qan, l.nbm, l.unit);
}

template <typename T>
void launch_ldl_update(hipStream_t s, const LocalMat &C, const int2 *d_list, int off, int na, int offb, int nb,
                       const PanelRef &pan, const PanelRef &qan) {
  if (na + nb <= 0) return;
  const UpdateLaunch l = update_launch(C, off, na, offb, nb);
  if constexpr (sizeof(T) == 4)
    k_ldl_update_w8f<<<l.grid, dim3(512), 0, s>>>(C, d_list + off, na, l.offb, nb, l.blocks_a, pan, qan, l.nbm, l.unit);
  else
    k_ldl_update_w8<T, 3><<<l.grid, dim3(512), 0, s>>>(C, d_list + off, na, l.offb, nb, l.blocks_a, pan, qan, l.nbm, l.unit);
}

struct StepSems {
  const int *diag = nullptr;
  const int *intile = nullptr;
  int intile_target = 0;
  int *head = nullptr;
  int *fail = nullptr;
};
template <typename T>
int trsm_step(hipStream_t s, T *tiles, long bsiz, int ntiles, const T *lkk, const T *winv, int mb, int st,
              T alpha, const StepSems &sm = StepSems()) {
  const int nbm = mb / MACRO, nc = nbm - 1 - st;
  if (alpha == T(1) && ntiles * nbm <= g_trsm_small_max) {
    const bool p1 = poll_in_kernel(s, sm.diag, 1, sm.fail, (long)ntiles * nbm * 4);
    k_solve_small<T><<<ntiles * nbm * 4, 256, 0, s>>>(tiles, bsiz, mb, nbm, 0, st, winv, T(1), g_ytab,
                                                      p1 ? sm.diag : nullptr, 1, sm.fail, sm.head);
    if (nc > 0) {
      const bool p2 = poll_in_kernel(s, sm.intile, sm.intile_target, sm.fail, 4L * nbm * nc * ntiles);
      k_small_update<T><<<dim3(2 * nbm, 2 * nc, ntiles), 256, 0, s>>>(
          tiles + (long)(st + 1) * MACRO * mb, mb, tiles + (long)st * MACRO * mb,
          lkk + (long)(st + 1) * MACRO + (long)st * MACRO * mb, mb, MACRO, g_ytab, 1, bsiz, bsiz, nullptr,
          p2 ? sm.intile : nullptr, sm.intile_target, sm.fail);
    }
    return 4 * nbm;
  }
  const bool p1 = poll_in_kernel(s, sm.diag, 1, sm.fail, (long)ntiles * nbm);
  k_panel_solve<T><<<ntiles * nbm, 256, 0, s>>>(tiles, bsiz, mb, nbm, 0, st, winv, st == 0 ? alpha : T(1), g_ytab,
                                                p1 ? sm.diag : nullptr, 1, sm.fail, sm.head);
  if (nc > 0) {
    const bool p2 = poll_in_kernel(s, sm.intile, sm.intile_target, sm.fail, (long)ntiles * nbm * nc);
    k_panel_update<T><<<ntiles * nbm * nc, 256, 0, s>>>(tiles, bsiz, mb, nbm, st, lkk, st == 0 ? alpha : T(1), g_ytab,
                                                        p2 ? sm.intile : nullptr, sm.intile_target, sm.fail);
  }
  return nbm;
}

template <typename T>
void launch_col_update_small(hipStream_t s, T *C, const T *A, const T *B, int mb, int ntiles, long bsiz, int *done) {
  if (ntiles > 0) k_small_update<T><<<dim3(mb / 64, mb / 64, ntiles), 256, 0, s>>>(C, mb, A, B, mb, mb, g_ytab, 1, bsiz, bsiz, done);
}
template void launch_col_update_small<double>(hipStream_t, double *, const double *, const double *, int, int, long, int *);
template void launch_col_update_small<float>(hipStream_t, float *, const float *, const float *, int, int, long, int *);

template <typename T>
void launch_diag_syrk(hipStream_t s, T *C, const T *A, int mb) {
  k_small_update<T><<<dim3(mb / 64, mb / 64), 256, 0, s>>>(C, mb, A, A, mb, mb, g_ytab, 0, 0, 0);
}

template <typename T>
void launch_potrf_tile(hipStream_t s, T *tile, int mb, T *winv, int *d_info, int info_base, int *sem) {
  const int nbm = mb / MACRO;
  const bool fused_steps = sem && g_intile_fused && nbm > 1;
  if (fused_steps) (void)hipMemsetAsync(sem, 0, (size_t)nbm * 32 * sizeof(int), s);
  for (int st = 0; st < nbm; ++st) {
    k_potrf_diag<T><<<1, 256, 0, s>>>(tile + (long)st * MACRO * (mb + 1), mb,
                                      winv + (long)st * MACRO * MACRO, d_info, info_base + st * MACRO, 1, g_dbg, g_ytab);
    const int nr = nbm - 1 - st;
    if (nr > 0) {
      if (fused_steps && nr * (2 * nr + 1) <= INTILE_FUSED_MAX) {
        k_intile_step<T><<<4 * nr + nr * (2 * nr + 1), 256, 0, s>>>(tile, mb, nbm, st, winv, g_ytab, sem + 32 * st, d_info);
      } else {
        k_solve_small<T><<<4 * nr, 256, 0, s>>>(tile, 0, mb, nbm, st + 1, st, winv, T(1), g_ytab);
        T *tr = tile + (long)(st + 1) * MACRO * (mb + 1);
        const T *xs = tile + (long)(st + 1) * MACRO + (long)st * MACRO * mb;
        k_small_update<T><<<dim3(2 * nr, 2 * nr), 256, 0, s>>>(tr, mb, xs, xs, mb, MACRO, g_ytab, 0, 0, 0);
      }
    }
  }
}

template <typename T>
void launch_panel_pipelined(hipStream_t sp, hipStream_t st, hipEvent_t *ev, T *lkk, int mb, T *winv,
                            int *d_info, int info_base, T *tiles, long bsiz, int ntiles, hipEvent_t ev_head,
                            const SyrkPipe *sy, const int *wait_sem, int wait_target, int *tile_sem) {
  const int nbm = mb / MACRO;
  const bool pipe = sy && ntiles > 0;
  const bool fused_plain = !pipe && tile_sem && g_intile_fused && nbm > 1;
  if (fused_plain) (void)hipMemsetAsync(tile_sem, 0, (size_t)nbm * 32 * sizeof(int), sp);
  auto slot = [&](int i) { return sy->sem + 32 * i; };
  const bool flow = pipe && sy->fc && sy->sflow && flow_applies(nbm);
  if (flow) {
    if (sy->join_flow && sy->ev_flow) {
      (void)hipEventRecord(sy->ev_flow, sp);
      (void)hipStreamWaitEvent(sy->sflow, sy->ev_flow, 0);
    }
    k_flow_factor<T><<<nbm, 256, 0, sp>>>(lkk, mb, nbm, winv, d_info, info_base, sy->fc, g_ytab, wait_sem, wait_target,
                                          slot(0), g_flow_fences, g_dbg);
    k_flow_rows<T><<<(mb - MACRO) / 64, 256, 0, sy->sflow>>>(lkk, mb, nbm, winv, d_info, sy->fc, g_ytab, wait_sem, wait_target,
                                                           slot(nbm), g_flow_fences, g_dbg);
  }
  for (int s = 0; s < nbm; ++s) {
    const int nr = nbm - 1 - s;
    if (!flow)
      k_potrf_diag<T><<<1, 256, 0, sp>>>(lkk + (long)s * MACRO * (mb + 1), mb, winv + (long)s * MACRO * MACRO,
                                         d_info, info_base + s * MACRO, 1, g_dbg, g_ytab, s == 0 ? wait_sem : nullptr,
                                         wait_target, pipe ? slot(s) : nullptr);
    if (nr > 0 && !flow) {
      if ((pipe || fused_plain) && g_intile_fused && nr * (2 * nr + 1) <= INTILE_FUSED_MAX) {
        k_intile_step<T><<<4 * nr + nr * (2 * nr + 1), 256, 0, sp>>>(lkk, mb, nbm, s, winv, g_ytab,
                                                                     pipe ? slot(nbm + s) : tile_sem + 32 * s, d_info);
      } else {
        k_solve_small<T><<<4 * nr, 256, 0, sp>>>(lkk, 0, mb, nbm, s + 1, s, winv, T(1), g_ytab, nullptr, 0, nullptr,
                                                 pipe ? slot(nbm + s) : nullptr);
        T *tr = lkk + (long)(s + 1) * MACRO * (mb + 1);
        const T *xs = lkk + (long)(s + 1) * MACRO + (long)s * MACRO * mb;
        k_small_update<T><<<dim3(2 * nr, 2 * nr), 256, 0, sp>>>(tr, mb, xs, xs, mb, MACRO, g_ytab, 0, 0, 0);
      }
    }
    if (ntiles <= 0) continue;
    if (pipe) {
      StepSems ss;
      ss.diag = slot(s);
      ss.intile = slot(nbm + s);
      ss.intile_target = (flow ? 8 : 4) * nr;
      ss.head = sy->c ? slot(2 * nbm + s) : nullptr;
      ss.fail = d_info;
      const int head_wgs = trsm_step<T>(st, tiles, bsiz, ntiles, lkk, winv, mb, s, T(1), ss);
      if (!sy->c) continue;
      const T *xs = tiles + (long)s * MACRO * mb;
      const int n64 = mb / 64;
      const long nslice = (long)n64 * (n64 + 1) / 2;
      int *done = s == nbm - 1 ? slot(3 * nbm) : nullptr;
      const bool ps = poll_in_kernel(sy->su, slot(2 * nbm + s), head_wgs, d_info, nslice);
      k_small_update<T><<<dim3(n64, n64), 256, 0, sy->su>>>(reinterpret_cast<T *>(sy->c), mb, xs, xs, mb, MACRO, g_ytab, 0, 0,
                                                           0, done, ps ? slot(2 * nbm + s) : nullptr, head_wgs, d_info);
      continue;
    }
    (void)hipEventRecord(ev[s], sp);
    (void)hipStreamWaitEvent(st, ev[s], 0);
    trsm_step<T>(st, tiles, bsiz, ntiles, lkk, winv, mb, s, T(1));
  }
  if (ev_head) (void)hipEventRecord(ev_head, st);
}
template void launch_panel_pipelined<double>(hipStream_t, hipStream_t, hipEvent_t *, double *, int, double *,
                                             int *, int, double *, long, int, hipEvent_t, const SyrkPipe *, const int *, int, int *);
template void launch_panel_pipelined<float>(hipStream_t, hipStream_t, hipEvent_t *, float *, int, float *, int *,
                                            int, float *, long, int, hipEvent_t, const SyrkPipe *, const int *, int, int *);

template <typename T>
void launch_invert_diag(hipStream_t s, const T *tile, int mb, T *winv) {
  const int nbm = mb / MACRO;
  for (int st = 0; st < nbm; ++st)
    k_potrf_diag<T><<<1, 256, 0, s>>>(const_cast<T *>(tile) + (long)st * MACRO * (mb + 1), mb,
                                      winv + (long)st * MACRO * MACRO, nullptr, 0, 0, nullptr, g_ytab);
}

template <typename T>
__global__ __launch_bounds__(256, 2) void k_invert_diag_batch(const T *A, long tstride, int mb, T *__restrict__ winv) {
  __shared__ DiagLds<T> L;
  const int nbm = mb / MACRO, t = blockIdx.x / nbm, s = blockIdx.x % nbm;
  potrf_diag_body<T>(const_cast<T *>(A) + t * tstride + (long)s * MACRO * (mb + 1), mb,
                     winv + ((long)t * nbm + s) * MACRO * MACRO, nullptr, 0, 0, L);
}

template <typename T>
void launch_invert_diag_batch(hipStream_t s, const T *A, long tstride, int nt, int mb, T *winv) {
  if (nt > 0) k_invert_diag_batch<T><<<(unsigned)(nt * (mb / MACRO)), 256, 0, s>>>(A, tstride, mb, winv);
}

template <typename T>
void launch_trsm_panel(hipStream_t s, T *tiles, long bsiz, int ntiles, const T *lkk, const T *winv,
                       int mb, T alpha) {
  if (ntiles <= 0) return;
  const int nbm = mb / MACRO;
  for (int st = 0; st < nbm; ++st) trsm_step<T>(s, tiles, bsiz, ntiles, lkk, winv, mb, st, alpha);
}

template <typename T>
void launch_gemm_nt_tile(hipStream_t s, const T *A, const T *B, T *C, int mb, T alpha, T beta,
                         bool lower_only) {
  const int nbm = mb / MACRO;
  k_gemm_nt_tile<T><<<dim3(nbm, nbm), 256, 0, s>>>(A, B, C, mb, nbm, alpha, beta, lower_only ? 1 : 0, 1, 0, 0, 0, 0);
}

template <typename T>
void launch_gemm_nt_batch(hipStream_t s, const T *A, long sA, int nz1, const T *B, long sB, int nz2, T *C, long sC1,
                          long sC2, int mb, T alpha, T beta) {
  const int nbm = mb / MACRO;
  if (nz1 <= 0 || nz2 <= 0) return;
  if (nz1 <= 65535) {
    const int per = std::max(1, 65535 / nz1);
    for (int z2 = 0; z2 < nz2; z2 += per) {
      const int c = std::min(per, nz2 - z2);
      k_gemm_nt_tile<T><<<dim3(nbm, nbm, nz1 * c), 256, 0, s>>>(A, B + (long)z2 * sB, C + (long)z2 * sC2, mb, nbm, alpha, beta, 0,
                                                               nz1, sA, sB, sC1, sC2);
    }
  } else {
    for (int z2 = 0; z2 < nz2; ++z2)
      for (int z1 = 0; z1 < nz1; z1 += 65535) {
        const int c = std::min(65535, nz1 - z1);
        k_gemm_nt_tile<T><<<dim3(nbm, nbm, c), 256, 0, s>>>(A + (long)z1 * sA, B + (long)z2 * sB, C + (long)z1 * sC1 + (long)z2 * sC2,
                                                          mb, nbm, alpha, beta, 0, c, sA, sB, sC1, sC2);
      }
  }
}

template <typename T>
void launch_update_ptrs(hipStream_t s, const T *const *cin, const T *const *a, const T *const *b, T *const *cout, int n, int mb,
                        bool yield) {
  if (n <= 0) return;
  const int nbm = mb / MACRO;
  const UpdateGrid u = update_grid((long)n * nbm * nbm, 0, false);
  const dim3 grid((unsigned)u.blocks_a);
  if constexpr (sizeof(T) == 4)
    k_update_ptrs_w8f<<<grid, dim3(512), 0, s>>>(cin, a, b, cout, n, mb, nbm, u.unit, yield ? g_ytab : nullptr);
  else
    k_update_ptrs_w8<T, 3><<<grid, dim3(512), 0, s>>>(cin, a, b, cout, n, mb, nbm, u.unit, yield ? g_ytab : nullptr);
}
template void launch_update_ptrs<double>(hipStream_t, const double *const *, const double *const *, const double *const *, double *const *, int, int, bool);
template void launch_update_ptrs<float>(hipStream_t, const float *const *, const float *const *, const float *const *, float *const *, int, int, bool);

void launch_copy_ptrs(hipStream_t s, const void *const *src, void *const *dst, int n, long bytes) {
  for (int z0 = 0; z0 < n; z0 += 65535) {
    const int nz = std::min(65535, n - z0);
    k_copy_ptrs<<<dim3((unsigned)std::max(1L, std::min(64L, bytes / (16 * 256 * 4))), nz), 256, 0, s>>>(src + z0, dst + z0, bytes);
  }
}

template <typename T>
void launch_plgsy(hipStream_t s, const LocalMat &A, int lnt, int prow, int pcol, double bump,
                  unsigned long long seed, int mbu, long nglob, int side) {
  k_plgsy<T><<<4096, 256, 0, s>>>(A, lnt, prow, pcol, bump, seed, mbu, nglob, side);
}

template <typename T>
void launch_residual(hipStream_t s, const T *Lbase, int Nb, int mb, double bump,
                     unsigned long long seed, double *d_acc, int mbu, long nglob, double *rowsum) {
  const int nbm = mb / MACRO;
  const long ntile = (long)Nb * (Nb + 1) / 2;
  k_residual<T><<<dim3((unsigned)(ntile * nbm * nbm)), 256, 0, s>>>(Lbase, Nb, mb, nbm, bump, seed, d_acc, mbu, nglob, rowsum);
}

template <typename T>
void launch_pad_identity(hipStream_t s, T *dst, int n, int ldp) {
  if (ldp > n) k_pad_identity<T><<<(ldp - n + 127) / 128, 128, 0, s>>>(dst, n, ldp);
}


template <typename T>
__global__ __launch_bounds__(256, 2) void k_mfma_probe(T *out, int iters) {
  typename Tr<T>::acc_t acc[16];
  const int t = threadIdx.x + blockIdx.x * 256;
  T a = T((t * 2654435761u >> 8) & 0xffff) * T(1.0 / 65536) - T(0.5);
  T b = T((t * 40503u >> 4) & 0xffff) * T(1.0 / 65536) - T(0.5);
#pragma unroll
  for (int u = 0; u < 16; ++u)
#pragma unroll
    for (int r = 0; r < 4; ++r) acc[u][r] = T(u + r);
  for (int it = 0; it < iters; ++it) {
#pragma unroll
    for (int u = 0; u < 16; ++u) acc[u] = Tr<T>::mfma(a, b, acc[u]);
    a = -a;
  }
  T s = T(0);
#pragma unroll
  for (int u = 0; u < 16; ++u)
#pragma unroll
    for (int r = 0; r < 4; ++r) s += acc[u][r];
  out[t] = s;
}

template <typename T>
void launch_mfma_probe(hipStream_t s, T *out, int blocks, int iters) {
  k_mfma_probe<T><<<blocks, 256, 0, s>>>(out, iters);
}
template void launch_mfma_probe<double>(hipStream_t, double *, int, int);
template void launch_mfma_probe<float>(hipStream_t, float *, int, int);

#define INSTANTIATE(T)                                                                              \
  template void launch_trail_update<T>(hipStream_t, const LocalMat &, const int2 *, int, int, int,  \
                                       int, const PanelRef &, bool, const PanelRef *);              \
  template void launch_syr2k_update<T>(hipStream_t, const LocalMat &, const int2 *, int, int, int,  \
                                       int, const PanelRef &, const PanelRef &);                    \
  template void launch_ldl_update<T>(hipStream_t, const LocalMat &, const int2 *, int, int, int,    \
                                     int, const PanelRef &, const PanelRef &);                      \
  template void launch_potrf_tile<T>(hipStream_t, T *, int, T *, int *, int, int *);                \
  template void launch_diag_syrk<T>(hipStream_t, T *, const T *, int);                               \
  template void launch_invert_diag<T>(hipStream_t, const T *, int, T *);                            \
  template void launch_invert_diag_batch<T>(hipStream_t, const T *, long, int, int, T *);            \
  template void launch_trsm_panel<T>(hipStream_t, T *, long, int, const T *, const T *, int, T);    \
  template void launch_gemm_nt_tile<T>(hipStream_t, const T *, const T *, T *, int, T, T, bool);    \
  template void launch_gemm_nt_batch<T>(hipStream_t, const T *, long, int, const T *, long, int, T *, long, long, \
                                        int, T, T);                                                 \
  template void launch_plgsy<T>(hipStream_t, const LocalMat &, int, int, int, double,               \
                                unsigned long long, int, long, int);                                \
  template void launch_residual<T>(hipStream_t, const T *, int, int, double, unsigned long long,    \
                                   double *, int, long, double *);                                  \
  template void launch_pad_identity<T>(hipStream_t, T *, int, int);
INSTANTIATE(double)
INSTANTIATE(float)

}
```

### dense_linear_app_amd/csrc/sched_check.hip

```cpp
#include <bitset>
#include <cstdint>
#include <cstdio>
#include <cstring>
#include <map>
#include <set>
#include <string>
#include <vector>

#include "../../include/cholmi.h"
#include "cholmi_internal.h"
#include "walker.h"

using namespace cholmi;

namespace {

struct TraceOps {
  const WaveGeo &g;
  bool prof;
  struct Op {
    std::string name;
    std::vector<std::pair<long, bool>> acc;
    std::vector<int> deps;
    int ch = -1, peer = -1, group = -1;
    bool is_send = false;
    size_t bytes = 0;
    char kind = '-';
    double cost = 0;
  };
  double t_tile = 0, t_panel = 0;
  double t_round() const { return t_tile * 512.0 / (g.nbm * g.nbm); }
  void cost_of(int id, char kind, double cost) {
    if (id >= 0 && id < (int)ops.size()) ops[id].kind = kind, ops[id].cost = cost;
  }
  std::vector<Op> ops;
  int last_on[ST_COUNT];
  std::set<int> pending[ST_COUNT];
  std::map<int, std::set<int>> ev_deps;
  std::map<const int *, int> producer;
  std::vector<int> sems;
  std::vector<std::string> findings;
  std::set<std::pair<int, int>> coop;
  int drop_wait = -1, drop_gate = -1, nwaits = 0, ngates = 0;
  std::string dropped;
  char *const fake_base = reinterpret_cast<char *>(uintptr_t(1) << 40);
  long local_slots = 0, next_slot = 0;

  TraceOps(const WaveGeo &geo, bool profiling) : g(geo), prof(profiling) {
    for (int &l : last_on) l = -1;
    local_slots = (long)g.lmt * std::max(1, g.lnt);
    next_slot = local_slots + 2;
  }
  bool profiling() const { return prof; }
  bool pipe_ok() const { return true; }
  bool counters() const { return !sems.empty(); }
  bool can_split_trsm() const { return true; }
  bool flow_ok() const { return true; }
  void *flow_event() { return nullptr; }
  void *stream(int st) { return reinterpret_cast<void *>(uintptr_t(st + 1)); }
  static int stream_id(void *s) { return (int)reinterpret_cast<uintptr_t>(s) - 1; }
  char *tile(int il, int jl) { return fake_base + ((size_t)il + (size_t)jl * g.lmt) * g.tile_bytes; }
  void *winv(int par) { return fake_base + (size_t)(local_slots + par) * g.tile_bytes; }
  void *alloc(size_t bytes) {
    char *p = fake_base + (size_t)next_slot * g.tile_bytes;
    next_slot += (long)((bytes + g.tile_bytes - 1) / g.tile_bytes);
    return p;
  }
  int *sem(int k, int which, int per_wave) { return sems.data() + ((size_t)per_wave * k + which) * 32; }
  using Acc = std::vector<std::pair<long, bool>>;
  void touch(Acc &a, const void *ptr, size_t bytes, bool write) const {
    if (!ptr || !bytes) return;
    const long s0 = (long)(((const char *)ptr - fake_base) / (long)g.tile_bytes);
    const long s1 = (long)(((const char *)ptr + bytes - 1 - fake_base) / (long)g.tile_bytes);
    for (long t = s0; t <= s1; ++t) a.push_back({t, write});
  }
  std::string slot_name(long t) const {
    char b[96];
    if (t < local_slots) {
      const int il = (int)(t % g.lmt), jl = (int)(t / g.lmt);
      snprintf(b, sizeof b, "tile (%d,%d)", il * g.P + g.pr, jl * g.Q + g.pc);
    } else if (t < local_slots + 2) {
      snprintf(b, sizeof b, "block inverses %ld", t - local_slots);
    } else {
      snprintf(b, sizeof b, "receive buffer slot %ld", t - local_slots - 2);
    }
    return b;
  }

  int begin(int, int nt, int sem_per_wave) {
    sems.assign((size_t)nt * sem_per_wave * 32 + 32, 0);
    return 0;
  }
  int add(unsigned mask, std::string name, Acc acc, std::vector<int> extra = {}) {
    Op op;
    op.name = std::move(name);
    op.acc = std::move(acc);
    std::set<int> d(extra.begin(), extra.end());
    for (int st = 0; st < ST_COUNT; ++st)
      if (mask & (1u << st)) {
        if (last_on[st] >= 0) d.insert(last_on[st]);
        d.insert(pending[st].begin(), pending[st].end());
        pending[st].clear();
      }
    d.erase(-1);
    op.deps.assign(d.begin(), d.end());
    ops.push_back(std::move(op));
    const int id = (int)ops.size() - 1;
    for (int st = 0; st < ST_COUNT; ++st)
      if (mask & (1u << st)) last_on[st] = id;
    return id;
  }
  int rec(int ev, int st) {
    std::set<int> d = pending[st];
    if (last_on[st] >= 0) d.insert(last_on[st]);
    ev_deps[ev] = std::move(d);
    return 0;
  }
  int wt(int st, int ev) {
    if (nwaits++ == drop_wait) {
      char b[120];
      snprintf(b, sizeof b, "(dropped: stream %d's wait for event %d = wave %d kind %d)", st, ev, ev / 15, ev % 15);
      dropped = b;
      return 0;
    }
    auto it = ev_deps.find(ev);
    if (it == ev_deps.end()) {
      char b[160];
      snprintf(b, sizeof b, "stream %d waits for event %d (wave %d, kind %d), which has not been recorded in this factorisation", st, ev,
               ev / 15, ev % 15);
      findings.push_back(b);
      return 0;
    }
    pending[st].insert(it->second.begin(), it->second.end());
    return 0;
  }
  int panel(int k, char *lkk, void *wv, char *tiles, int ntiles, int, int ev_head, const SyrkPipe *sy, const int *wait_sem, int) {
    std::vector<int> extra;
    if (wait_sem && ngates++ != drop_gate) {
      auto it = producer.find(wait_sem);
      if (it == producer.end()) findings.push_back("POTRF(" + std::to_string(k) + ") polls a counter nobody raises");
      else extra.push_back(it->second);
    }
    const bool flow = sy && sy->fc && sy->sflow && flow_applies(g.nbm);
    std::vector<int> rows_extra = extra;
    if (flow && sy->join_flow) {
      if (nwaits++ == drop_wait) {
        dropped = "(dropped: the flow stream's join of wave " + std::to_string(k) + ")";
      } else {
        if (last_on[ST_PANEL] >= 0) rows_extra.push_back(last_on[ST_PANEL]);
        rows_extra.insert(rows_extra.end(), pending[ST_PANEL].begin(), pending[ST_PANEL].end());
      }
    }
    Acc pa;
    touch(pa, lkk, g.tile_bytes, true);
    touch(pa, wv, std::max<size_t>(1, g.winv_bytes), true);
    const int potrf = add(1u << ST_PANEL, "POTRF(" + std::to_string(k) + ")" + (flow ? " [flow: factor]" : ""), pa, extra);
    cost_of(potrf, 'P', t_panel);
    std::vector<int> after = {potrf};
    if (flow) {
      Acc ra;
      touch(ra, lkk, g.tile_bytes, true);
      touch(ra, wv, std::max<size_t>(1, g.winv_bytes), false);
      const int rows = add(1u << ST_CX, "POTRF(" + std::to_string(k) + ") [flow: row slabs]", ra, rows_extra);
      coop.insert({potrf, rows});
      after.push_back(rows);
    }
    if (ntiles <= 0) return 0;
    Acc acc;
    touch(acc, lkk, g.tile_bytes, false);
    touch(acc, wv, std::max<size_t>(1, g.winv_bytes), false);
    touch(acc, tiles, (size_t)ntiles * g.tile_bytes, true);
    const int trsm = add(1u << ST_TRSM, "TRSM(" + std::to_string(k) + ")", acc, after);
    cost_of(trsm, 'T', t_panel / g.nbm + 0.5 * ntiles * t_tile / g.nbm);
    if (ev_head >= 0) ev_deps[ev_head] = {trsm};
    if (sy && sy->c && sy->su) {
      Acc sa;
      touch(sa, tiles, g.tile_bytes, false);
      touch(sa, sy->c, g.tile_bytes, true);
      const int sl = add(1u << ST_U1, "SYRK slices(" + std::to_string(k) + ")", sa, {trsm});
      cost_of(sl, 'Y', t_panel / g.nbm);
      producer[sy->sem + 32 * (3 * g.nbm)] = sl;
    }
    return 0;
  }
  int trsm(int k, char *tiles, int ntiles, const char *lkk, const char *wv, int st) {
    Acc acc;
    touch(acc, lkk, g.tile_bytes, false);
    touch(acc, wv, std::max<size_t>(1, g.winv_bytes), false);
    touch(acc, tiles, (size_t)ntiles * g.tile_bytes, true);
    cost_of(add(1u << st, "TRSM(" + std::to_string(k) + ") of " + std::to_string(ntiles) + " tiles [received diagonal tile]", acc), 'T',
            std::max(t_panel / g.nbm * g.nbm * 0.5, 0.5 * ntiles * t_tile));
    return 0;
  }
  int diag_syrk(int k, int j, char *Cjj, const char *A, int st) {
    Acc acc;
    touch(acc, A, g.tile_bytes, false);
    touch(acc, Cjj, g.tile_bytes, true);
    cost_of(add(1u << st, "SYRK(" + std::to_string(j) + "," + std::to_string(j) + ") by panel " + std::to_string(k), acc), 'Y', t_round());
    return 0;
  }
  const char *ptile(const PanelRef &p, int i) const {
    return (const char *)p.base[i % g.P] + (size_t)(i / g.P - p.first[i % g.P]) * g.tile_bytes;
  }
  int update(int k1, int k2, int jlo, int jhi, int what, const PanelRef &p1, const PanelRef *p2, bool, int st) {
    const int nt = g.nt;
    jlo = std::min(jlo, nt), jhi = std::min(jhi, nt);
    Acc acc;
    std::set<int> rows;
    double tiles_eq = 0;
    for (int j = jlo; j < jhi; ++j) {
      if (j % g.Q != g.pc) continue;
      for (int i = j; i < nt; ++i) {
        if (i % g.P != g.pr || !(i == j ? (what & 2) : (what & 1))) continue;
        touch(acc, tile(i / g.P, j / g.Q), g.tile_bytes, true);
        rows.insert(i), rows.insert(j);
        tiles_eq += i == j ? 0.5 * (1.0 + 1.0 / g.nbm) : 1.0;
      }
    }
    if (acc.empty()) return 0;
    const PanelRef *ps[2] = {&p1, (p2 && k2 >= 0) ? p2 : nullptr};
    for (const PanelRef *p : ps)
      if (p)
        for (int i : rows) touch(acc, ptile(*p, i), g.tile_bytes, false);
    char b[120];
    snprintf(b, sizeof b, "update columns [%d,%d) %sby panel %d%s", jlo, jhi, what == 3 ? "" : what == 1 ? "(off-diagonal) " : "(diagonal) ", k1,
             ps[1] ? (" and " + std::to_string(k2)).c_str() : "");
    const int np = ps[1] ? 2 : 1;
    cost_of(add(1u << st, b, acc), 'U', std::max(t_round() * np, tiles_eq * t_tile * np));
    return 0;
  }
  int update_col_small(int k, int st) {
    const int n = g.nt - k - 2;
    Acc acc;
    touch(acc, tile(k + 1, k), g.tile_bytes, false);
    touch(acc, tile(k + 2, k), (size_t)n * g.tile_bytes, false);
    touch(acc, tile(k + 2, k + 1), (size_t)n * g.tile_bytes, true);
    cost_of(add(1u << st, "column " + std::to_string(k + 1) + " (latency form) by panel " + std::to_string(k), acc), 'L', 0.6 * t_round());
    return 0;
  }
  struct Chan {
    TraceOps *o;
    int id;
  } chan[2] = {{this, 0}, {this, 1}};
  int ngroups[2] = {0, 0};
  static int t_begin(void *ctx) {
    Chan *c = (Chan *)ctx;
    ++c->o->ngroups[c->id];
    return 0;
  }
  static int t_end(void *) { return 0; }
  void mark_comm(int id, int ch, bool is_send, int peer, size_t bytes) {
    Op &op = ops[id];
    op.ch = ch, op.is_send = is_send, op.peer = peer, op.bytes = bytes, op.group = ngroups[ch] - 1;
  }
  std::string op_graph() const {
    std::string out;
    char b[128];
    for (size_t i = 0; i < ops.size(); ++i) {
      const Op &op = ops[i];
      snprintf(b, sizeof b, "%zu %d %s %d %zu %d ", i, op.ch, op.ch < 0 ? "-" : (op.is_send ? "S" : "R"), op.peer, op.bytes, op.group);
      out += b;
      for (size_t d = 0; d < op.deps.size(); ++d) out += (d ? "," : "") + std::to_string(op.deps[d]);
      if (op.deps.empty()) out += "-";
      snprintf(b, sizeof b, " %c %.9f\n", op.kind, op.cost);
      out += b;
    }
    return out;
  }
  static int t_allreduce(void *, long long *) { return 0; }
  static int t_send(void *ctx, const void *buf, size_t bytes, int peer, void *stream) {
    Chan *c = (Chan *)ctx;
    TraceOps *o = c->o;
    Acc acc;
// ... 2 lines not shown
    return 0;
  }
  static int t_recv(void *ctx, void *buf, size_t bytes, int peer, void *stream) {
    Chan *c = (Chan *)ctx;
    TraceOps *o = c->o;
    Acc acc;
    o->touch(acc, buf, bytes, true);
    o->mark_comm(o->add(1u << stream_id(stream), "receive from rank " + std::to_string(peer), acc), c->id, false, peer, bytes);
    return 0;
  }
  int finish(int, int, const std::vector<std::pair<int, int>> &, int *info) {
    *info = 0;
    const int n = (int)ops.size();
    constexpr int MAXOPS = 32768;
    if (n > MAXOPS) {
      findings.push_back("too many launches for the checker");
      return 0;
    }
    std::vector<std::bitset<MAXOPS>> *reach = new std::vector<std::bitset<MAXOPS>>(n);
    for (int i = 0; i < n; ++i)
      for (int d : ops[i].deps) {
        (*reach)[i] |= (*reach)[d];
        (*reach)[i].set(d);
      }
    std::map<long, std::vector<std::pair<int, bool>>> by_res;
    for (int i = 0; i < n; ++i)
      for (auto &a : ops[i].acc) by_res[a.first].push_back({i, a.second});
    for (auto &kv : by_res) {
      auto &v = kv.second;
      for (size_t b = 1; b < v.size(); ++b)
        for (size_t a = 0; a < b; ++a) {
          if (v[a].first == v[b].first || (!v[a].second && !v[b].second)) continue;
          if (coop.count({v[a].first, v[b].first})) continue;
          if (!(*reach)[v[b].first].test(v[a].first)) {
            char buf[480];
            snprintf(buf, sizeof buf, "%s: '%s' (%s) and '%s' (%s) are not ordered", slot_name(kv.first).c_str(), ops[v[a].first].name.c_str(),
                     v[a].second ? "writes" : "reads", ops[v[b].first].name.c_str(), v[b].second ? "writes" : "reads");
            if (findings.size() < 64) findings.push_back(buf);
          }
        }
    }
    delete reach;
    return 0;
  }
};

}

static int schedule_check_impl(int nt, int mb, int p, int q, int rank, double t_tile, double t_panel, int profiling, char *report, int cap,
                               bool comm_trace) {
  if (nt <= 0 || mb < MACRO || mb % MACRO) return chol_internal_fail(-1, "schedule_check: nt > 0, mb a multiple of 128");
  if (p < 1 || q < 1 || p > MAXP || rank < 0 || rank >= p * q) return chol_internal_fail(-2, "schedule_check: grid");
  WaveGeo g;
  g.init(nt, mb, p, q, rank, 8);
  TraceOps ops(g, profiling != 0);
  ops.t_tile = t_tile, ops.t_panel = t_panel;
  WaveCalib c;
  c.t_tile = t_tile, c.t_panel = t_panel;
  if (const char *e = getenv("CHOLMI_CHECK_DROP_WAIT")) ops.drop_wait = atoi(e);
  if (const char *e = getenv("CHOLMI_CHECK_DROP_GATE")) ops.drop_gate = atoi(e);
  WaveComm cm;
  for (int ch = 0; ch < 2; ++ch) {
    cm.ch[ch].ctx = &ops.chan[ch];
    cm.ch[ch].group_begin = TraceOps::t_begin;
    cm.ch[ch].send = TraceOps::t_send;
    cm.ch[ch].recv = TraceOps::t_recv;
    cm.ch[ch].group_end = TraceOps::t_end;
    cm.ch[ch].allreduce_max = TraceOps::t_allreduce;
  }
  Walker<TraceOps> w(ops, g, p * q > 1 ? &cm : nullptr, c);
  long long info = 0;
  int rc = w.setup();
  if (!rc) rc = w.run(&info);
  if (rc) return rc < 0 ? rc : -rc;
  if (comm_trace) {
    const std::string gr = ops.op_graph();
    if (!report || (size_t)cap <= gr.size()) return chol_internal_fail(-3, "comm_trace: buffer too small");
    memcpy(report, gr.c_str(), gr.size() + 1);
    return (int)ops.findings.size();
  }
  std::string out;
  for (auto &f : ops.findings) out += f + "\n";
  char tail[200];
  snprintf(tail, sizeof tail, "%zu launches, %d event waits, %d counter edges, %d flow-form waves, %zu findings\n", ops.ops.size(), ops.nwaits,
           ops.ngates, w.flow_waves, ops.findings.size());
  out += tail;
  if (!ops.dropped.empty()) out += ops.dropped + "\n";
  if (report && cap > 0) snprintf(report, (size_t)cap, "%s", out.size() < (size_t)cap ? out.c_str() : out.substr(out.size() - cap + 1).c_str());
  return (int)ops.findings.size();
}
extern "C" int chol_debug_schedule_check_grid(int nt, int mb, int p, int q, int rank, double t_tile, double t_panel, int profiling,
                                              char *report, int cap) {
  return schedule_check_impl(nt, mb, p, q, rank, t_tile, t_panel, profiling, report, cap, false);
}
extern "C" int chol_debug_comm_trace(int nt, int mb, int p, int q, int rank, double t_tile, double t_panel, char *out, int cap) {
  return schedule_check_impl(nt, mb, p, q, rank, t_tile, t_panel, 0, out, cap, true);
}
extern "C" int chol_debug_schedule_check(int nt, int mb, double t_tile, double t_panel, int profiling, char *report, int cap) {
  return chol_debug_schedule_check_grid(nt, mb, 1, 1, 0, t_tile, t_panel, profiling, report, cap);
}
```

### dense_linear_app_amd/csrc/spd.hip

```cpp
#include <hip/hip_runtime.h>

#include <algorithm>
#include <cmath>
#include <cstdio>
#include <cstring>
#include <map>
#include <numeric>
#include <vector>

#include "api_internal.h"

using namespace cholmi;

namespace {

ScratchPool<1> work;
ScratchPool<4, true> mx;
ScratchPool<4> iv;
ScratchPool<7> cn;
ScratchPool<8, true> rf;
ScratchPool<3> ps;
ScratchPool<3> sg;
ScratchPool<4> sy;
ScratchPool<4> rb;

struct LastStats {
  double v[8] = {};
  void clear() { std::fill(v, v + 8, 0.0); }
  int read(const char *name, double *out, int n = 8) const {
    if (!ctx_inited()) return failf(CHOL_ERR_NOT_INITIALIZED, "last_%s_stats before chol_init", name);
    if (!out) return failf(-1, "last_%s_stats: NULL", name);
    std::lock_guard<std::recursive_mutex> lk(ctx_mutex());
    std::copy(v, v + n, out);
    return 0;
  }
};
LastStats mx_stats, cn_stats, rf_stats, ps_stats, sg_stats, sy_stats, rb_stats;

hipStream_t main_stream() { return main_rank_ctx()->st[ST_MAIN]; }

template <typename Launch, typename... Panels>
void update_cols(Launch launch, const chol_desc *d, int jlo, int jhi, const Panels &...pans) {
  const WorkRange rr = whole_col_range(d, jlo, jhi);
  launch(main_stream(), whole_local_mat(d), d->d_list, rr.off, rr.na, rr.offb, rr.nb, pans...);
}

struct EventTimer {
  hipEvent_t e[2] = {nullptr, nullptr};
  ~EventTimer() {
    for (hipEvent_t x : e)
      if (x) (void)hipEventDestroy(x);
  }
  int start() {
    for (hipEvent_t &x : e)
      if (!x) HIPCHECK(hipEventCreate(&x));
    HIPCHECK(hipEventRecord(e[0], main_stream()));
    return 0;
  }
  int mark() {
    HIPCHECK(hipEventRecord(e[1], main_stream()));
    return 0;
  }
  int add(double *acc) {
    float ms = 0;
    HIPCHECK(hipEventElapsedTime(&ms, e[0], e[1]));
    *acc += ms;
    return 0;
  }
  int stop(double *acc) {
    if (int rc = mark()) return rc;
    HIPCHECK(hipEventSynchronize(e[1]));
    return add(acc);
  }
};

template <typename T>
int potrs_impl(chol_desc *A, chol_desc *B, const T *udiag = nullptr, const T *rdiag = nullptr) {
  const int nt = A->nt, nr = B->nt, mb = A->mbi;
  const long bs = A->bsizi;
  const size_t tb = (size_t)bs * sizeof(T);
  T *La = reinterpret_cast<T *>(A->mat), *Bm = reinterpret_cast<T *>(B->mat);
  if (int rc = work.ensure_bytes(0, ((size_t)nr * nt + 2 + (size_t)nr + (size_t)nt) * tb, "potrs_tile")) return rc;
  T *scr = work.as<T>(0);
  T *Z = scr, *Wt = scr + (size_t)nr * nt * bs, *Tt = Wt + bs, *tmp = Tt + (size_t)nt * bs;
  hipStream_t s = main_stream();
  T *winv = reinterpret_cast<T *>(main_rank_ctx()->winv);
  auto Ltile = [&](int i, int j) { return La + ((long)i + (long)j * A->lmt) * bs; };
  auto Ztile = [&](int r, int i) { return Z + ((long)r + (long)i * nr) * bs; };
  auto Dtile = [&](int k) { return udiag ? udiag + (long)k * bs : Ltile(k, k); };
  for (int r = 0; r < nr; ++r)
    launch_tiles_transpose<T>(s, Bm + (long)r * B->lmt * bs, bs, Ztile(r, 0), (long)nr * bs, mb, nt);
  for (int k = 0; k < nt; ++k) {
    launch_invert_diag<T>(s, Dtile(k), mb, winv);
    launch_trsm_panel<T>(s, Ztile(0, k), bs, nr, Dtile(k), winv, mb, T(1));
    launch_gemm_nt_batch<T>(s, Ztile(0, k), bs, nr, Ltile(k + 1, k), bs, nt - 1 - k, Ztile(0, k + 1), bs, (long)nr * bs, mb,
                            T(-1), T(1));
  }
  if (rdiag) launch_ldl_zscale<T>(s, Z, (long)nr * nt * bs, bs, mb, nr, rdiag);
  for (int k = nt - 1; k >= 0; --k) {
    HIPCHECK(hipMemsetAsync(Wt, 0, tb, s));
    launch_pad_identity<T>(s, Wt, 0, mb);
    launch_invert_diag<T>(s, Dtile(k), mb, winv);
    launch_trsm_panel<T>(s, Wt, bs, 1, Dtile(k), winv, mb, T(1));
    launch_gemm_nt_batch<T>(s, Ztile(0, k), bs, nr, Wt, 0, 1, tmp, bs, 0, mb, T(1), T(0));
    HIPCHECK(hipMemcpyAsync(Ztile(0, k), tmp, (size_t)nr * tb, hipMemcpyDeviceToDevice, s));
    if (k > 0) {
      launch_tiles_transpose<T>(s, Ltile(k, 0), (long)A->lmt * bs, Tt, bs, mb, k);
      launch_gemm_nt_batch<T>(s, Ztile(0, k), bs, nr, Tt, bs, k, Ztile(0, 0), bs, (long)nr * bs, mb, T(-1), T(1));
    }
  }
  for (int r = 0; r < nr; ++r)
    launch_tiles_transpose<T>(s, Ztile(r, 0), (long)nr * bs, Bm + (long)r * B->lmt * bs, bs, mb, nt);
  HIPCHECK(hipGetLastError());
  HIPCHECK(hipStreamSynchronize(s));
  return 0;
}

template <typename T>
int potrs_uplo(int upper, chol_desc *A, chol_desc *B) {
  return through_lower(upper, {A}, [&] { return potrs_impl<T>(A, B); }, false);
}

constexpr int DSPOSV_ITMAX = 30;

chol_desc scratch_view(const chol_desc *d, void *mat) {
  chol_desc v = *d;
  v.mat = mat;
  v.user_mat = nullptr;
  v.owns = false;
  v.version = 0;
  v.d_list = nullptr;
  return v;
}

size_t colmax_bytes(int nrhs) { return (size_t)(2 * nrhs + 2) * sizeof(unsigned long long); }

struct RefineTol {
  double anrm, cte;
  RefineTol(unsigned long long anrm_bits, long n) {
    memcpy(&anrm, &anrm_bits, sizeof anrm);
    cte = anrm * std::ldexp(1.0, -53) * std::sqrt((double)n);
  }
  bool converged(const unsigned long long *hmax, int nrhs, double *berr = nullptr) const {
    bool done = true;
    for (int j = 0; j < nrhs; ++j) {
      double rn, xn;
      memcpy(&rn, &hmax[j], sizeof rn);
      memcpy(&xn, &hmax[nrhs + j], sizeof xn);
      if (berr) berr[j] = rn == 0 ? 0.0 : rn / (anrm * xn);
      if (!(rn <= xn * cte)) done = false;
    }
    return done;
  }
};

int dsposv_mixed(int uplo, chol_desc *A, chol_desc *B, chol_desc *X, int *iter) {
  hipStream_t s = main_stream();
  const int up = uplo == CHOL_UPPER ? 1 : 0, nrhs = B->ln;
  const TileGeo ga = geo_of(A), gx = geo_of(B);
  mx_stats.clear();
  double *st = mx_stats.v;
  const size_t rf_bytes = (size_t)B->lmt * B->lnt * B->bsizi * sizeof(float);
  const char *what = "dsposv_tile";
  int rc = mx.ensure_bytes(0, (size_t)A->lmt * A->lnt * A->bsizi * sizeof(float), what);
  if (!rc) rc = mx.ensure_bytes(1, rf_bytes, what);
  if (!rc) rc = mx.ensure_bytes(2, sym_resid_part_bytes(ga, nrhs), what);
  if (!rc) rc = mx.ensure_bytes(3, colmax_bytes(nrhs), what);
  if (rc) return rc;
  float *Af = mx.as<float>(0), *Rf = mx.as<float>(1);
  double *part = mx.as<double>(2);
  unsigned long long *colmax = mx.as<unsigned long long>(3);
  int *flag = reinterpret_cast<int *>(colmax + 2 * nrhs);
  std::vector<unsigned long long> hmax(2 * nrhs + 1);
  chol_desc Ad = scratch_view(A, Af), Rd = scratch_view(B, Rf);
  Ad.dtype = Rd.dtype = CHOL_REAL_FLOAT;
  Ad.esize = Rd.esize = sizeof(float);
  Ad.d_list = A->d_list;
// ... 804 lines not shown
  return *rank < n ? 1 : 0;
}

void pstrf_flip(chol_desc *A) {
  if (A->mbi % 64 == 0) return transpose_storage(A);
  const PsGeo g{A->lm, A->mb, A->mbi, A->lmt, (long)A->bsizi};
  if (A->dtype == CHOL_REAL_DOUBLE) launch_pstrf_transpose<double>(main_stream(), g, (double *)A->mat);
  else launch_pstrf_transpose<float>(main_stream(), g, (float *)A->mat);
}

int pstrf_run(int uplo, chol_desc *A, int *piv, int *rank, double tol) {
  const bool up = uplo == CHOL_UPPER;
  const int rc = through_lower(up, {A}, [&] {
    return A->dtype == CHOL_REAL_DOUBLE ? pstrf_impl<double>(A, piv, rank, tol) : pstrf_impl<float>(A, piv, rank, tol);
  }, true, pstrf_flip);
  if (up) HIPCHECK(hipGetLastError());
  return rc;
}

struct PhaseMarks {
  std::vector<hipEvent_t> ev;
  std::vector<int> ph;
  ~PhaseMarks() {
    for (hipEvent_t e : ev) (void)hipEventDestroy(e);
  }
  int mark(int p) {
    hipEvent_t e;
    HIPCHECK(hipEventCreate(&e));
    ev.push_back(e);
    ph.push_back(p);
    HIPCHECK(hipEventRecord(e, main_stream()));
    return 0;
  }
  int sum(double *st) {
    if (ev.size() < 2) return 0;
    HIPCHECK(hipEventSynchronize(ev.back()));
    for (size_t i = 1; i < ev.size(); ++i) {
      float ms = 0;
      HIPCHECK(hipEventElapsedTime(&ms, ev[i - 1], ev[i]));
      st[ph[i]] += ms;
    }
    float ms = 0;
    HIPCHECK(hipEventElapsedTime(&ms, ev.front(), ev.back()));
    st[0] += ms;
    return 0;
  }
};

template <typename T>
int sygst_impl(chol_desc *A, chol_desc *B) {
  hipStream_t s = main_stream();
  sg_stats.clear();
  double *st = sg_stats.v;
  const long n = A->lm;
  if (n == 0) return 0;
  const int nt = A->nt, mb = A->mb, e = A->mbi, lmt = A->lmt;
  const int E = condest_edge(geo_of(A)), nbm = E / MACRO;
  if (nt > 1 && e != E) return fail(CHOL_ERR_NOT_SUPPORTED, "sygst_tile: stored tile edge");
  const long bs = A->bsizi, blk = (long)MACRO * MACRO, EE = (long)E * E;
  const char *what = "sygst_tile";
  int rc = sg.ensure_bytes(0, (size_t)nt * EE * sizeof(T), what);
  if (!rc) rc = sg.ensure_bytes(1, 2 * (size_t)nt * nbm * blk * sizeof(T), what);
  if (!rc) rc = sg.ensure_bytes(2, (3 * (size_t)EE + (size_t)(nt - 1) * bs) * sizeof(T), what);
  if (rc) return rc;
  T *Dv = sg.as<T>(0), *W = sg.as<T>(1), *Yi = W + (size_t)nt * nbm * blk;
  T *S = sg.as<T>(2), *W2 = S + EE, *Cs = W2 + EE, *yrow = Cs + EE;
  T *Am = reinterpret_cast<T *>(A->mat);
  const T *Bm = reinterpret_cast<const T *>(B->mat);
  auto tile = [&](const T *p, int i, int j) { return const_cast<T *>(p) + ((long)i + (long)j * lmt) * bs; };
  forget_winv(A->mat);
  PhaseMarks pm;
  enum { P_DIAG = 1, P_CHAIN, P_SYR2K, P_SOLVE };
  if ((rc = pm.mark(0))) return rc;
  stage_factor_diag_into<T>(B, 0, Dv, W, Yi);
  if ((rc = pm.mark(P_DIAG))) return rc;
  for (int k = 0; k < nt; ++k) {
    const int nv = (int)std::min<long>(mb, n - (long)k * mb);
    launch_sygst_diag<T>(s, tile(Am, k, k), e, nv, Dv + k * EE, E, S, W2, Cs);
    st[5] += 1;
    if (k + 1 < nt) {
      const int nr = nt - 1 - k;
      T *P = tile(Am, k + 1, k);
      T *Lt = tile(Bm, k + 1, k);
      launch_trsm_panel<T>(s, P, bs, nr, tile(Bm, k, k), W + (long)k * nbm * blk, e, T(1));
      launch_gemm_nt_batch<T>(s, Lt, bs, nr, Cs, 0, 1, P, bs, 0, e, T(-0.5), T(1));
      if ((rc = pm.mark(P_CHAIN))) return rc;
      update_cols(launch_syr2k_update<T>, A, k + 1, nt, one_panel(tile(Am, 0, k)), one_panel(tile(Bm, 0, k)));
      if ((rc = pm.mark(P_SYR2K))) return rc;
      launch_gemm_nt_batch<T>(s, Lt, bs, nr, Cs, 0, 1, P, bs, 0, e, T(-0.5), T(1));
    }
    HIPCHECK(hipGetLastError());
    if ((rc = pm.mark(P_CHAIN))) return rc;
  }
  for (int m = 1; m < nt; ++m) launch_sygst_solve_row<T>(s, Am, Bm, bs, lmt, E, m, Dv + m * EE, yrow);
  HIPCHECK(hipGetLastError());
  if ((rc = pm.mark(P_SOLVE))) return rc;
  return pm.sum(st);
}

int sygst_run(int uplo, chol_desc *A, chol_desc *B) {
  const bool dbl = A->dtype == CHOL_REAL_DOUBLE;
  int info = 0;
  int rc = dbl ? diag_zero<double>(B, &info, "sygst_tile") : diag_zero<float>(B, &info, "sygst_tile");
  if (rc) return rc;
  if (info) return info;
  rc = through_lower(uplo == CHOL_UPPER, {A, B},
                     [&] { return dbl ? sygst_impl<double>(A, B) : sygst_impl<float>(A, B); });
  HIPCHECK(hipGetLastError());
  HIPCHECK(hipStreamSynchronize(main_stream()));
  return rc;
}

template <typename T>
int sytrf_impl(chol_desc *A, int *info) {
  hipStream_t s = main_stream();
  sy_stats.clear();
  double *st = sy_stats.v;
  *info = 0;
  const long n = A->lm;
  if (n == 0) return 0;
  const int nt = A->nt, mb = A->mb, e = A->mbi, lmt = A->lmt, nbm = e / MACRO;
  const long bs = A->bsizi, blk = (long)MACRO * MACRO;
  const char *what = "sytrf_nopiv_tile";
  const int npm = ldl_partials();
  int rc = sy.ensure_bytes(0, (size_t)std::max(1, nt - 1) * bs * sizeof(T), what);
  if (!rc) rc = sy.ensure_bytes(1, ((size_t)bs + 2 * (size_t)nbm * blk + 2 * (size_t)nt * e) * sizeof(T), what);
  if (!rc) rc = sy.ensure_bytes(2, ((size_t)npm + 8) * sizeof(double) + sizeof(int), what);
  if (rc) return rc;
  T *Wscr = sy.as<T>(0), *Wt = sy.as<T>(1), *Lc = Wt + bs, *winv = Lc + nbm * blk, *dv = winv + nbm * blk, *rv = dv + (long)nt * e;
  double *pmax = sy.as<double>(2), *out = pmax + npm;
  int *d_info = reinterpret_cast<int *>(out + 8);
  T *Am = reinterpret_cast<T *>(A->mat);
  auto tile = [&](int i, int j) { return Am + ((long)i + (long)j * lmt) * bs; };
  forget_winv(A->mat);
  HIPCHECK(hipMemsetAsync(pmax, 0, ((size_t)npm + 8) * sizeof(double) + sizeof(int), s));
  PhaseMarks pm;
  enum { P_CHAIN = 1, P_UPDATE };
  if ((rc = pm.mark(0))) return rc;
  int hinfo = 0;
  for (int k = 0; k < nt && !hinfo; ++k) {
    const int nr = nt - 1 - k;
    launch_ldl_tile<T>(s, tile(k, k), e, Wt, Lc, winv, dv + (long)k * e, rv + (long)k * e, d_info, k * mb, pmax);
    if (nr > 0) {
      launch_trsm_panel<T>(s, tile(k + 1, k), bs, nr, tile(k, k), winv, e, T(1));
      launch_ldl_scale<T>(s, tile(k + 1, k), Wscr, (long)nr * bs, bs, e, rv + (long)k * e, pmax);
    }
    HIPCHECK(hipGetLastError());
    HIPCHECK(hipMemcpyAsync(&hinfo, d_info, sizeof hinfo, hipMemcpyDeviceToHost, s));
    if ((rc = pm.mark(P_CHAIN))) return rc;
    const hipEvent_t chain_end = pm.ev.back();
    if (nr > 0) {
      update_cols(launch_ldl_update<T>, A, k + 1, nt, one_panel(Wscr, k + 1), one_panel(tile(0, k)));
      HIPCHECK(hipGetLastError());
      if ((rc = pm.mark(P_UPDATE))) return rc;
    }
    HIPCHECK(hipEventSynchronize(chain_end));
  }
  launch_ldl_stats<T>(s, dv, n, mb, e, pmax, out);
  HIPCHECK(hipGetLastError());
  double h[5] = {};
  HIPCHECK(hipMemcpyAsync(h, out, sizeof h, hipMemcpyDeviceToHost, s));
  if ((rc = pm.mark(P_CHAIN))) return rc;
  if ((rc = pm.sum(st))) return rc;
  HIPCHECK(hipStreamSynchronize(s));
  for (int i = 0; i < 5; ++i) st[3 + i] = h[i];
  *info = hinfo;
  return 0;
}

int sytrf_run(int uplo, chol_desc *A) {
  if (A->mbi % MACRO) return fail(CHOL_ERR_NOT_SUPPORTED, "sytrf_nopiv_tile: stored tile edge must be a multiple of 128");
  int info = 0;
  const int rc = through_lower(uplo == CHOL_UPPER, {A}, [&] {
    return A->dtype == CHOL_REAL_DOUBLE ? sytrf_impl<double>(A, &info) : sytrf_impl<float>(A, &info);
  });
  HIPCHECK(hipGetLastError());
  HIPCHECK(hipStreamSynchronize(main_stream()));
  return rc ? rc : info;
}

template <typename T>
int sytrs_impl(int upper, chol_desc *A, chol_desc *B, bool diag_checked = false) {
  int info = 0;
  int rc = diag_checked ? 0 : diag_zero<T>(A, &info, "sytrs_nopiv_tile");
  if (rc) return rc;
  if (info) return info;
  const int nt = A->nt, e = A->mbi;
  const long bs = A->bsizi;
  if ((rc = sy.ensure_bytes(3, ((size_t)nt * bs + (size_t)nt * e) * sizeof(T), "sytrs_nopiv_tile"))) return rc;
  T *U = sy.as<T>(3), *rv = U + (long)nt * bs;
  return through_lower(upper, {A}, [&] {
    launch_ldl_stage<T>(main_stream(), reinterpret_cast<const T *>(A->mat), (long)(A->lmt + 1) * bs, bs, e, nt, U, rv);
    return potrs_impl<T>(A, B, U, rv);
  });
}

enum { RB_TOTAL = 0, RB_GEN, RB_XFORM, RB_FACT, RB_SOLVE, RB_RESID, RB_VEC, RB_STEPS };
constexpr int RBT_ITMAX = 10;

template <typename T>
int rbt_generate(chol_desc *W, long n, int depth, unsigned long long seed) {
  hipStream_t s = main_stream();
  std::vector<T> h((size_t)n * depth);
  unsigned long long ran = seed;
  for (size_t x = 0; x < h.size(); ++x) {
    ran = 6364136223846793005ULL * ran + 1ULL;
    const double r = 0.5 - (double)ran * 5.4210108624275222e-20;
    h[x] = (T)std::exp(r / 10.0);
  }
  if (int rc = rb.ensure_bytes(0, h.size() * sizeof(T), "sytrf_rbt_tile")) return rc;
  HIPCHECK(hipMemcpyAsync(rb.p[0], h.data(), h.size() * sizeof(T), hipMemcpyHostToDevice, s));
  launch_rbt_put<T>(s, geo_of(W), reinterpret_cast<T *>(W->mat), rb.as<T>(0), n, depth);
  HIPCHECK(hipGetLastError());
  HIPCHECK(hipStreamSynchronize(s));
  return 0;
}

template <typename T>
void rbt_transform(chol_desc *A, const chol_desc *W, int depth) {
  for (int k = depth - 1; k >= 0; --k)
    launch_rbt_sym<T>(main_stream(), geo_of(A), reinterpret_cast<T *>(A->mat), geo_of(W), reinterpret_cast<const T *>(W->mat), k);
}

template <typename T>
int rbt_vectors(chol_desc *X, const chol_desc *W, int depth, bool trans, double *st) {
  EventTimer tv;
  if (int rc = tv.start()) return rc;
// ... 561 lines not shown
```

### dense_linear_app_amd/csrc/walker.h

```cpp
#pragma once
#include <algorithm>
#include <chrono>
#include <cstdlib>
#include <cstring>
#include <utility>
#include <vector>

#include "cholmi_internal.h"

namespace cholmi {

struct WaveGeo {
  int nt = 0, P = 1, Q = 1, rank = 0, pr = 0, pc = 0, lmt = 0, lnt = 0, mb = 0, nbm = 0;
  size_t esize = 8, tile_bytes = 0, winv_bytes = 0;
  std::vector<int> ge, gd;
  void init(int nt_, int mb_, int P_, int Q_, int rank_, size_t esize_) {
    nt = nt_, mb = mb_, P = P_, Q = Q_, rank = rank_, esize = esize_;
    nbm = mb / MACRO;
    pr = rank / Q, pc = rank % Q;
    lmt = nt - pr > 0 ? (nt - pr + P - 1) / P : 0;
    lnt = nt - pc > 0 ? (nt - pc + Q - 1) / Q : 0;
    tile_bytes = (size_t)mb * mb * esize;
    winv_bytes = (size_t)nbm * MACRO * MACRO * esize;
    ge.assign(nt + 2, 0);
// ... 195 lines not shown
      return 0;
    };
    for (int p2 = 0; p2 < g.P; ++p2) {
      int il0, cnt;
      g.part(k, p2, &il0, &cnt);
      p.first[p2] = il0;
      if (g.pr == p2 && g.pc == dc) {
        char *src = cnt > 0 ? o.tile(il0, k / g.Q) : pbuf[slot][p2];
        p.base[p2] = src;
        if (cnt <= 0) continue;
        WRC(before());
        for (int c2 = 0; c2 < g.Q; ++c2)
          if (c2 != dc) WRC(cm->send(1, src, (size_t)cnt * g.tile_bytes, g.rank_of(p2, c2), st));
        for (int r2 = 0; r2 < g.P; ++r2) {
          if (r2 == p2) continue;
          for (int t = 0; t < cnt;) {
            const int c = ((il0 + t) * g.P + p2) % g.Q;
            int t1 = t + 1;
            while (t1 < cnt && ((il0 + t1) * g.P + p2) % g.Q == c) ++t1;
            WRC(cm->send(1, src + (size_t)t * g.tile_bytes, (size_t)(t1 - t) * g.tile_bytes, g.rank_of(r2, c), st));
            t = t1;
          }
        }
      } else {
        char *buf = pbuf[slot][p2];
        p.base[p2] = buf;
        if (cnt <= 0) continue;
        if (g.pr == p2) {
          WRC(before());
          WRC(cm->recv(1, buf, (size_t)cnt * g.tile_bytes, g.rank_of(p2, dc), st));
        } else {
          for (int t = 0; t < cnt;) {
            if (((il0 + t) * g.P + p2) % g.Q != g.pc) {
              ++t;
              continue;
            }
            int t1 = t + 1;
            while (t1 < cnt && ((il0 + t1) * g.P + p2) % g.Q == g.pc) ++t1;
            WRC(before());
            WRC(cm->recv(1, buf + (size_t)t * g.tile_bytes, (size_t)(t1 - t) * g.tile_bytes, g.rank_of(p2, dc), st));
            t = t1;
          }
        }
      }
    }
    WRC(cm->end(1));
    if (!waited && g.pc == dc) WRC(o.wt(ST_PX, ev(k, E_TRSM)));
    return o.rec(ev(k, E_PANEL), ST_PX);
  }

  int run(long long *info_out) {
    const auto t_host0 = std::chrono::steady_clock::now();
    const int nt = g.nt, mb = g.mb, nbm = g.nbm, P = g.P, Q = g.Q;
    const bool mr = multi();
    const int sem_per_wave = 3 * nbm + 1 + flow_ctl_lines(nbm);
    WRC(o.begin(E_PER_WAVE * nt + F_FIXED + nbm + 1, nt, sem_per_wave));
    const int ev_steps = fx(F_FIXED);
    WRC(o.rec(fx(F_START), ST_MAIN));
    for (int st = ST_PANEL; st < (mr ? ST_COUNT : ST_CX + 1); ++st) WRC(o.wt(st, fx(F_START)));
    bool paired = false, cols_pending = false, had_pairs = false;
    int open_bracket = -1;
    int bnd = -1;
    bool prev_halves = false, prev_flow = false, flow_joined = false;
    const bool flags = !mr && o.counters();
    const bool flags_local = mr && o.counters();
    const bool flow_run = (double)g.tiles_in(1, nt) * cal.t_tile < sw.flow_run_fac * cal.t_panel;
    const int *wait_sem = nullptr;
    int wait_target = 0;
    const double b3 = (double)mb * mb * mb;
    const double t_tile = cal.t_tile, t_panel = cal.t_panel;
    const bool prof = o.profiling();
    for (int k = 0; k < nt; ++k) {
      const int dr = k % P, dc = k % Q, par = k & 1;
      const bool in_col = g.pc == dc, own_diag = in_col && g.pr == dr, last = k + 1 >= nt;
      int il0m = 0, cntm = 0;
      g.part(k, g.pr, &il0m, &cntm);
      if (!in_col) cntm = 0;
      const int local_tiles = g.tiles_in(k + 1, nt);
      const bool pair_first = k >= PAIR_START && ((k - PAIR_START) & 1) == 0;
      if (pair_first)
        paired = mb <= PAIR_MAX_MB && k + 2 < nt && (double)local_tiles * t_tile >= sw.pair_fac * t_panel;
      const bool plain_yield = (double)local_tiles * t_tile < sw.yfac * t_panel;
      const bool chain_bound = (double)local_tiles * t_tile < sw.pipe_fac * t_panel;
      const bool pipe = flags && !paired && !last && o.pipe_ok() && plain_yield && chain_bound;
      const bool pipe_local = flags_local && !paired && o.pipe_ok() && plain_yield && chain_bound && own_diag && cntm > 0;
      const bool flow = pipe && own_diag && cntm > 0 && flow_ctl_lines(nbm) > 0 && o.flow_ok() && flow_applies(nbm) &&
                        (sw.flow_fac > 0 ? (double)local_tiles * t_tile < sw.flow_fac * t_panel : flow_run);
      if (k > 0 && in_col) WRC(o.wt(ST_TRSM, ev(k - 1, E_U1R)));
      const char *head = nullptr;
      if (own_diag) {
        char *lkk = o.tile(k / P, k / Q);
        SyrkPipe sy;
        if (pipe_local) {
          sy.c = nullptr;
          sy.su = nullptr;
          sy.sem = o.sem(k, 0, sem_per_wave);
        }
        if (pipe) {
          if (k > 0 && !prev_halves) WRC(o.wt(ST_U1, ev(k - 1, E_U2)));
          sy.c = o.tile((k + 1) / P, (k + 1) / Q);
          sy.su = (hipStream_t)o.stream(ST_U1);
          sy.sem = o.sem(k, 0, sem_per_wave);
          if (flow) {
            sy.fc = o.sem(k, 3 * nbm + 1, sem_per_wave);
            sy.sflow = (hipStream_t)o.stream(ST_CX);
            sy.ev_flow = (hipEvent_t)o.flow_event();
            sy.join_flow = !prev_flow && (wait_sem == nullptr || !flow_joined);
          }
        }
        const bool head_mine = !last && P == 1;
        WRC(o.panel(k, lkk, o.winv(par), lkk + g.tile_bytes, cntm, ev_steps, head_mine ? ev(k, E_HEAD) : -1,
                    pipe || pipe_local ? &sy : nullptr, wait_sem, wait_target));
        if (mr && P > 1 && !last) {
          WRC(o.rec(ev(k, E_LKK), ST_PANEL));
          WRC(diag_send(k, lkk, (const char *)o.winv(par)));
        }
        if (pipe && !flow && !flow_joined && !mr && k + 2 < nt && flow_ctl_lines(nbm) > 0 && o.flow_ok() && flow_applies(nbm) &&
            (sw.flow_fac > 0 ? (double)g.tiles_in(k + 2, nt) * t_tile < sw.flow_fac * t_panel : flow_run)) {
          WRC(o.rec(fx(F_FLOWJ), ST_PANEL));
          WRC(o.wt(ST_CX, fx(F_FLOWJ)));
          flow_joined = true;
        }
      } else if (in_col && cntm > 0) {
        WRC(diag_recv(k));
        WRC(o.wt(ST_TRSM, ev(k, E_LKKR)));
        char *tiles = o.tile(il0m, k / Q);
        const char *lkk = lkk_buf[par], *wv = lkk_buf[par] + g.tile_bytes;
        const bool head_mine = !last && g.pr == (k + 1) % P;
        if (head_mine && cntm > 1 && o.can_split_trsm()) {
          WRC(o.trsm(k, tiles, 1, lkk, wv, ST_TRSM));
          WRC(o.rec(ev(k, E_HEAD), ST_TRSM));
          WRC(o.trsm(k, tiles + g.tile_bytes, cntm - 1, lkk, wv, ST_TRSM));
        } else {
          WRC(o.trsm(k, tiles, cntm, lkk, wv, ST_TRSM));
          if (head_mine) WRC(o.rec(ev(k, E_HEAD), ST_TRSM));
        }
      }
      const bool by_flags = pipe;
      prev_flow = flow;
      if (flow) ++flow_waves, ++regimes[R_FLOW];
      if (pipe || pipe_local) ++regimes[R_PIPE];
      wait_sem = by_flags ? o.sem(k, 3 * nbm, sem_per_wave) : nullptr;
      wait_target = (mb / 64) * (mb / 64 + 1) / 2;
      if (in_col) WRC(o.rec(ev(k, mr ? E_TRSM : E_PANEL), ST_TRSM));
      if (own_diag && !by_flags) {
        WRC(o.wt(ST_PANEL, ev(k, mr ? E_TRSM : E_PANEL)));
        if (mr && P > 1 && !last) WRC(o.wt(ST_PANEL, ev(k, E_CXS)));
      }
      if (last) break;
      if (mr) {
        WRC(head_move(k, &head));
        WRC(exchange(k));
      } else {
        PanelRef &p = pan[k % NBUF];
        memset(&p, 0, sizeof p);
        p.P = 1;
        p.base[0] = o.tile(0, k);
        head = o.tile(k + 1, k);
      }
      const PanelRef &pk = pan[k % NBUF];
      const bool next_diag_mine = g.rank_of((k + 1) % P, (k + 1) % Q) == g.rank;
      char *ckk = next_diag_mine ? o.tile((k + 1) / P, (k + 1) / Q) : nullptr;
      if (paired) {
        const bool odd = !pair_first;
        if (!odd && k > 0 && !had_pairs) WRC(o.wt(ST_U1, ev(k - 1, E_U2)));
        if (prev_halves) {
          WRC(o.wt(ST_MAIN, ev(k - 1, E_NEAR)));
          prev_halves = false;
        }
        const PanelRef &prev = pan[(odd ? k - 1 : k) % NBUF];
        const PanelRef *p2 = odd ? &pk : nullptr;
        const PanelRef &p1 = odd ? prev : pk;
        const int k1 = odd ? k - 1 : k, k2 = odd ? k : -1;
        const int n_c1 = g.tiles_in(k + 1, k + 2), n_ca = g.tiles_in(k + 2, k + 3), n_cb = g.tiles_in(k + 3, k + 4),
                  n_big = g.tiles_in(k + 4, nt);
        const int wave_tiles = n_c1 + (odd ? n_ca + n_cb + n_big : 0);
        const bool yield = (double)wave_tiles * t_tile * (odd ? 2 : 1) < sw.yfac * t_panel * (odd ? 2 : 1);
        if (next_diag_mine) {
          if (odd) WRC(o.diag_syrk(k - 1, k + 1, ckk, ptile(prev, k + 1), ST_U1));
          WRC(o.wt(ST_U1, ev(k, E_HEAD)));
          WRC(o.diag_syrk(k, k + 1, ckk, head, ST_U1));
          WRC(o.rec(ev(k, E_U1D), ST_U1));
          WRC(o.wt(ST_PANEL, ev(k, E_U1D)));
        }
        WRC(o.wt(ST_U1, ev(k, E_PANEL)));
        if (!odd && open_bracket < 0 && prof) WRC(o.rec(ev(k, E_P0), ST_U1));
        WRC(o.update(k1, k2, k + 1, k + 2, 1, p1, p2, yield, ST_U1));
        WRC(o.rec(ev(k, E_U1R), ST_U1));
        int timed = 0;
        double fl = 0;
        const int o_c1 = g.off_in(k + 1, k + 2);
        if (odd) {
          if (o_c1 > 0) ++timed, fl += 2.0 * o_c1;
          if (k >= 2) WRC(o.wt(ST_U1, ev(k - 2, E_U2)));
          WRC(o.update(k1, k2, k + 2, k + 3, 3, p1, p2, yield, ST_U1));
          WRC(o.update(k1, k2, k + 3, k + 4, 3, p1, p2, yield, ST_U1));
          if (n_ca > 0) ++timed, fl += 2.0 * g.off_in(k + 2, k + 3) + g.diag_in(k + 2, k + 3);
          if (n_cb > 0) ++timed, fl += 2.0 * g.off_in(k + 3, k + 4) + g.diag_in(k + 3, k + 4);
          WRC(o.rec(fx(F_COLS), ST_U1));
          cols_pending = true;
          WRC(o.wt(ST_MAIN, ev(k, E_PANEL)));
          if (prof) WRC(o.rec(ev(k, E_P0), ST_MAIN));
          WRC(o.update(k1, k2, k + 4, nt, 3, p1, p2, yield, ST_MAIN));
          if (n_big > 0) ++timed, fl += 2.0 * g.off_in(k + 4, nt) + g.diag_in(k + 4, nt);
          WRC(o.rec(ev(k, E_U2), ST_MAIN));
          open_bracket = k;
          upd_launches += timed;
          upd_flops += 2.0 * fl * b3;
        } else {
          WRC(o.rec(ev(k, E_U2), ST_MAIN));
          if (prof) {
            if (open_bracket >= 0) {
              WRC(o.wt(ST_MAIN, fx(F_COLS)));
              WRC(o.wt(ST_MAIN, ev(k, E_U1R)));
              WRC(o.rec(ev(open_bracket, E_P1), ST_MAIN));
              WRC(o.rec(ev(k, E_P0), ST_MAIN));
              WRC(o.rec(ev(k, E_P1), ST_MAIN));
// ... 136 lines not shown
```

### include/cholmi.h

```cpp
#ifndef CHOLMI_H
#define CHOLMI_H

#include <stddef.h>
#include <stdint.h>

#ifdef __cplusplus
extern "C" {
#endif

enum {
  CHOL_REAL_FLOAT = 2,
  CHOL_REAL_DOUBLE = 3,
  CHOL_NOTRANS = 111,
  CHOL_TRANS = 112,
  CHOL_UPPER = 121,
  CHOL_LOWER = 122,
  CHOL_UPPER_LOWER = 123,
  CHOL_NONUNIT = 131,
  CHOL_UNIT = 132,
  CHOL_LEFT = 141,
  CHOL_RIGHT = 142,
  CHOL_ONE_NORM = 171,
  CHOL_FROBENIUS_NORM = 174,
  CHOL_INF_NORM = 175,
// ... 59 lines not shown
int chol_posv_tile(int uplo, chol_desc_t *A, chol_desc_t *B);

int chol_dsposv_tile(int uplo, chol_desc_t *A, chol_desc_t *B, chol_desc_t *X, int *iter);
int chol_last_dsposv_stats(double *out8);

int chol_trtri_tile(int uplo, int diag, chol_desc_t *A);
int chol_potri_tile(int uplo, chol_desc_t *A);
int chol_poinv_tile(int uplo, chol_desc_t *A);

int chol_lansy_tile(int norm, int uplo, chol_desc_t *A, double *value);
int chol_pocon_tile(int uplo, chol_desc_t *A, double anorm, double *rcond);
int chol_last_pocon_stats(double *out4);

enum {
  CHOL_FACT_NONE = 0,
  CHOL_FACT_EQUILIBRATE = 1,
  CHOL_FACT_FACTORED = 2
};
int chol_poequ_tile(chol_desc_t *A, chol_desc_t *S, double *scond, double *amax);
int chol_laqsy_tile(int uplo, chol_desc_t *A, chol_desc_t *S, double scond, double amax, int *equed);
int chol_porfs_tile(int uplo, chol_desc_t *A, chol_desc_t *AF, chol_desc_t *B, chol_desc_t *X, double *ferr,
                    double *berr);
int chol_posvx_tile(int fact, int uplo, chol_desc_t *A, chol_desc_t *AF, int *equed, chol_desc_t *S,
                    chol_desc_t *B, chol_desc_t *X, double *rcond, double *ferr, double *berr);
int chol_last_posvx_stats(double *out8);
int chol_bench_refine(int uplo, chol_desc_t *A, chol_desc_t *AF, chol_desc_t *X, int path, int reps, double *ms);

int chol_pstrf_tile(int uplo, chol_desc_t *A, int *piv, int *rank, double tol);
int chol_last_pstrf_stats(double *out8);

int chol_sygst_tile(int itype, int uplo, chol_desc_t *A, chol_desc_t *B);
int chol_last_sygst_stats(double *out8);

int chol_sytrf_nopiv_tile(int uplo, chol_desc_t *A);
int chol_sytrs_nopiv_tile(int uplo, chol_desc_t *A, chol_desc_t *B);
int chol_sysv_nopiv_tile(int uplo, chol_desc_t *A, chol_desc_t *B);
int chol_last_sytrf_stats(double *out8);

int chol_rbt_apply_tile(int uplo, chol_desc_t *A, chol_desc_t *W, int depth);
int chol_sytrf_rbt_tile(int uplo, chol_desc_t *A, chol_desc_t *W, int depth, unsigned long long seed);
int chol_sytrs_rbt_tile(int uplo, chol_desc_t *A, chol_desc_t *W, int depth, chol_desc_t *B);
int chol_sysv_rbt_tile(int uplo, chol_desc_t *A, chol_desc_t *AF, chol_desc_t *W, int depth, unsigned long long seed,
                       chol_desc_t *B, chol_desc_t *X, int *iter, double *berr);
int chol_last_rbt_stats(double *out8);

int chol_lapack_to_tile(const void *A, int lda, chol_desc_t *desc);
int chol_tile_to_lapack(chol_desc_t *desc, void *A, int lda);

int chol_tile_upload(chol_desc_t *desc, int I, int J, const void *host_tile);
int chol_tile_download(chol_desc_t *desc, int I, int J, void *host_tile);

int chol_residual_plgsy(chol_desc_t *L, double bump, unsigned long long seed, double *rel);
int chol_residual_plgsy_inf(chol_desc_t *L, double bump, unsigned long long seed, double *rel_inf);

void chol_make_spd_like_chameleon(double *A, int N, int LDA, double bump, char uplo,
                                  unsigned long long seed);
void chol_enforce_strict_diag_dominance(double *A, int N, int LDA, double eps);
int chol_parse_payloads(const char *buf, const long long *off, int n, int *op, int *B, long long *id_off, int *id_len);
void chol_extract_block(const double *A, int N, int LDA, int B, int bi, int bj, double *block);

int chol_last_potrf_stats(double *total_ms, double *update_ms, int *update_launches,
                          double *update_flops);
int chol_last_potrf_regimes(int *out8, int *nt);
int chol_set_profiling(int on);

int chol_bench_update(chol_desc_t *desc, int k, int ablate, int reps, double *ms, double *flops);

int chol_debug_stamps(int enable, unsigned long long *out, int max_pairs);

int chol_mfma_probe(int dtype, int waves_per_simd, double *tflops);

int chol_debug_flow_waves(void);

int chol_debug_schedule_check(int nt, int mb, double t_tile, double t_panel, int profiling, char *report, int cap);
int chol_debug_schedule_check_grid(int nt, int mb, int p, int q, int rank, double t_tile, double t_panel, int profiling,
                                   char *report, int cap);
int chol_debug_comm_trace(int nt, int mb, int p, int q, int rank, double t_tile, double t_panel, char *out, int cap);

int chol_debug_task_record(int on, int mutate);
int chol_debug_task_check(long long *out5);

int chol_debug_calibration(double *out8);
int chol_debug_update_kernel(int dtype, char *buf, int buflen);
int chol_debug_device_counters(void);

void *chol_desc_local_ptr(chol_desc_t *desc, size_t *bytes);
int chol_desc_local_tiles(chol_desc_t *desc, int *lmt, int *lnt);

typedef struct chol_transport {
  void *ctx;
  int (*group_begin)(void *ctx);
  int (*send)(void *ctx, const void *buf, size_t bytes, int peer, void *stream);
  int (*recv)(void *ctx, void *buf, size_t bytes, int peer, void *stream);
  int (*group_end)(void *ctx);
  int (*allreduce_max)(void *ctx, long long *value);
} chol_transport_t;
int chol_set_transport(const chol_transport_t *t);
int chol_set_transport_channel(int channel, const chol_transport_t *t);
#define CHOL_RCCL_ID_BYTES 256
int chol_transport_rccl_unique_id(void *id256);
int chol_transport_rccl_init(const void *id256, int rank, int nranks);
int chol_transport_rccl_finalize(void);
int chol_transport_rccl_version(void);
int chol_dist_last_stats(double *issue_us_per_wave, long long *sends, long long *recvs, long long *bytes_sent);

int chol_dist_gather_lower(chol_desc_t *src, chol_desc_t *dst, int root);

int chol_set_transport_null(void);

int chol_transport_selftest(int self_rank, size_t bytes);

typedef struct chol_test_engine {
  void *ctx;
  void *store;
  size_t esize;
  void *(*alloc)(void *ctx, size_t bytes);
  int (*potrf)(void *ctx, int k, void *lkk);
  int (*trsm)(void *ctx, int k, const void *lkk);
  int (*update)(void *ctx, int k, int jlo, int jhi, const void *const *bases, const int *firsts, int skip_diag);
  int (*update_diag)(void *ctx, int k, int j, const void *const *bases, const int *firsts);
  int (*info)(void *ctx);
} chol_test_engine_t;
int chol_dist_factorize_with(const chol_test_engine_t *engine, const chol_transport_t *transport, int N, int B,
                             int p, int q, int rank, int mode);

int chol_dist_rehearse(int dtype, int N, int mb, int p, int q, double bump, unsigned long long seed,
                       chol_desc_t *full, double *ms);

#ifdef __cplusplus
}
#endif
#endif
```

Measured before the change: 70.65.

## Fuse TRSM panel steps via precomputed step factors and one GEMM per step

Adds a fused TRSM path for wide panels. Per step, a small kernel precomputes factor blocks W (the diagonal block inverse times the off-diagonal blocks of the diagonal tile). A single wide-tile GEMM-like kernel then applies all prior columns at once and writes the step result. This replaces the per-step solve-and-update kernels and aims to cut launches and per-step work when the panel has many tiles. It costs extra workspace, an extra small kernel per step, and a longer k-loop per step, and it applies only when the panel is wide enough and not in the yield regime.

Measured after the change: 71.31, median of 6. About the same (+0.9%).

```diff
diff --git a/dense_linear_app_amd/_lib.py b/dense_linear_app_amd/_lib.py
--- a/dense_linear_app_amd/_lib.py
+++ b/dense_linear_app_amd/_lib.py
@@ -120,6 +120,8 @@
         "chol_debug_calibration": ([C.POINTER(d)], i),
         "chol_debug_update_kernel": ([i, C.c_char_p, i], i),
         "chol_debug_device_counters": ([], i),
+        "chol_debug_trsm_panel": ([i, vp, i, vp, i, i, i], i),
+        "chol_debug_trsm_fused_steps": ([], C.c_longlong),
         "chol_dist_last_stats": ([C.POINTER(d), C.POINTER(C.c_longlong), C.POINTER(C.c_longlong), C.POINTER(C.c_longlong)], i),
         "chol_dist_factorize_with": ([vp, vp, i, i, i, i, i, i], i),
         "chol_dist_gather_lower": ([vp, vp, i], i),
diff --git a/dense_linear_app_amd/csrc/api.hip b/dense_linear_app_amd/csrc/api.hip
--- a/dense_linear_app_amd/csrc/api.hip
+++ b/dense_linear_app_amd/csrc/api.hip
@@ -757,6 +757,8 @@
   }
   r->winv_bytes = (size_t)32 * MACRO * MACRO * sizeof(double);
   HIPCHECK(hipMalloc(&r->winv, 2 * r->winv_bytes));
+  r->wstep_bytes = step_factor_elems(1024) * sizeof(double);
+  HIPCHECK(hipMalloc(&r->wstep, WSTEP_SETS * r->wstep_bytes));
   HIPCHECK(hipMalloc(&r->d_info, sizeof(int)));
   HIPCHECK(hipMemset(r->d_info, 0, sizeof(int)));
   {
@@ -820,6 +822,8 @@
   r->ev_flow = nullptr;
   r->pool.free_all();
   if (r->winv) (void)hipFree(r->winv);
+  if (r->wstep) (void)hipFree(r->wstep);
+  r->wstep = nullptr;
   if (r->d_info) (void)hipFree(r->d_info);
   if (r->d_sem) (void)hipFree(r->d_sem);
   r->winv = nullptr;
@@ -881,6 +885,7 @@
   if (g.r.device >= count) return fail(CHOL_ERR_NO_GPU, "chol_init: device index out of range");
   HIPCHECK(hipSetDevice(g.r.device));
   if (const char *e = getenv("CHOLMI_TRSM_SMALL_MAX")) cholmi::g_trsm_small_max = atoi(e);
+  if (const char *e = getenv("CHOLMI_TRSM_FUSED")) cholmi::g_trsm_fused = atoi(e);
   {
     hipDeviceProp_t prop;
     HIPCHECK(hipGetDeviceProperties(&prop, g.r.device));
@@ -1109,6 +1114,20 @@
 }
 
 template <typename T>
+static int debug_trsm_panel_impl(T *tiles, int ntiles, const T *lkk, int mb, int step, int fused) {
+  hipStream_t s = g.r.st[ST_MAIN];
+  T *winv = reinterpret_cast<T *>(g.r.winv);
+  T *ws = fused ? reinterpret_cast<T *>(wstep_set(g.r, WSTEP_MAIN, mb, sizeof(T))) : nullptr;
+  if (fused && !ws) return fail(-3, "debug_trsm_panel: tile edge beyond the fused steps' workspace");
+  launch_invert_diag<T>(s, lkk, mb, winv);
+  for (int st = step < 0 ? 0 : step; st < (step < 0 ? mb / MACRO : step + 1); ++st)
+    launch_trsm_step<T>(s, tiles, (long)mb * mb, ntiles, lkk, winv, mb, st, ws);
+  HIPCHECK(hipGetLastError());
+  HIPCHECK(hipStreamSynchronize(s));
+  return 0;
+}
+
+template <typename T>
 static int panel_fused_impl(int dtype, int mb, int n, const void *const *c_in, void *const *c_out) {
   const TaskExec::Pending p = tx.pend;
   tx.pend.on = false;
@@ -1134,7 +1153,8 @@
   if (!tx_rec.on) {
     launch_copy_ptrs(st, (const void *const *)dl, (void *const *)(dl + lb), n, (long)tb);
     launch_panel_pipelined<T>(sp, st, tx.pev, reinterpret_cast<T *>(p.a_out), mb, wset, g.d_binfo + p.slot, 0,
-                              reinterpret_cast<T *>(c_out[0]), (long)mb * mb, n, nullptr, nullptr, nullptr, 0, tile_sems());
+                              reinterpret_cast<T *>(c_out[0]), (long)mb * mb, n, nullptr, nullptr, nullptr, 0, tile_sems(),
+                              reinterpret_cast<T *>(wstep_for_panel(g.r, 0, n, mb, sizeof(T))));
   }
   (void)nbm;
   TXHIP(hipEventRecord(ev_join, st));
@@ -1795,6 +1815,19 @@
 
 int chol_debug_device_counters(void) { return g.inited && g.r.d_sem ? 1 : 0; }
 
+int chol_debug_trsm_panel(int dtype, void *tiles, int ntiles, const void *lkk, int mb, int step, int fused) {
+  if (!g.inited) return fail(CHOL_ERR_NOT_INITIALIZED, "debug_trsm_panel before chol_init");
+  const bool f64 = dtype == CHOL_REAL_DOUBLE;
+  if (!f64 && dtype != CHOL_REAL_FLOAT) return fail(-1, "debug_trsm_panel: dtype");
+  if (!tiles || !lkk || ntiles <= 0 || mb < MACRO || mb % MACRO || step >= mb / MACRO ||
+      (size_t)(mb / MACRO) * MACRO * MACRO * (f64 ? 8 : 4) > g.r.winv_bytes)
+    return fail(-2, "debug_trsm_panel: arguments");
+  return f64 ? debug_trsm_panel_impl<double>(static_cast<double *>(tiles), ntiles, static_cast<const double *>(lkk), mb, step, fused)
+             : debug_trsm_panel_impl<float>(static_cast<float *>(tiles), ntiles, static_cast<const float *>(lkk), mb, step, fused);
+}
+
+long long chol_debug_trsm_fused_steps(void) { return cholmi::g_trsm_fused_steps; }
+
 int chol_debug_update_kernel(int dtype, char *buf, int buflen) {
   if (!buf || buflen < 8) return fail(-2, "debug_update_kernel: buffer");
   const bool f64 = dtype == CHOL_REAL_DOUBLE;
diff --git a/dense_linear_app_amd/csrc/cholmi_internal.h b/dense_linear_app_amd/csrc/cholmi_internal.h
--- a/dense_linear_app_amd/csrc/cholmi_internal.h
+++ b/dense_linear_app_amd/csrc/cholmi_internal.h
@@ -55,6 +55,8 @@
   hipStream_t st[ST_COUNT] = {};
   void *winv = nullptr;
   size_t winv_bytes = 0;
+  void *wstep = nullptr;
+  size_t wstep_bytes = 0;
   int *d_info = nullptr;
   int *d_sem = nullptr;
   bool flow_ok = false;
@@ -99,6 +101,17 @@
 };
 
 extern int g_trsm_small_max;
+extern int g_trsm_fused;
+extern long long g_trsm_fused_steps;
+inline size_t step_factor_elems(int mb) { return (size_t)(mb / MACRO) * (mb / MACRO + 1) / 2 * MACRO * MACRO; }
+constexpr int WSTEP_SETS = 3, WSTEP_MAIN = 2;
+inline void *wstep_set(const RankCtx &r, int which, int mb, size_t esize) {
+  return r.wstep && step_factor_elems(mb) * esize <= r.wstep_bytes ? (char *)r.wstep + (size_t)which * r.wstep_bytes : nullptr;
+}
+constexpr int TRSM_FUSED_MIN_BLOCKS = 512;
+inline void *wstep_for_panel(const RankCtx &r, int which, int ntiles, int mb, size_t esize) {
+  return (long)ntiles * (mb / MACRO) >= TRSM_FUSED_MIN_BLOCKS ? wstep_set(r, which, mb, esize) : nullptr;
+}
 extern int g_poll_max_wgs;
 bool flow_applies(int nbm);
 extern int g_flow;
@@ -147,7 +160,7 @@
 void launch_panel_pipelined(hipStream_t sp, hipStream_t st, hipEvent_t *ev, T *lkk, int mb, T *winv,
                             int *d_info, int info_base, T *tiles, long bsiz, int ntiles,
                             hipEvent_t ev_head = nullptr, const SyrkPipe *sy = nullptr, const int *wait_sem = nullptr,
-                            int wait_target = 0, int *tile_sem = nullptr);
+                            int wait_target = 0, int *tile_sem = nullptr, T *wstep = nullptr);
 
 template <typename T>
 void launch_col_update_small(hipStream_t s, T *C, const T *A, const T *B, int mb, int ntiles, long bsiz, int *done);
@@ -159,7 +172,9 @@
 
 template <typename T>
 void launch_trsm_panel(hipStream_t s, T *tiles, long bsiz, int ntiles, const T *lkk, const T *winv,
-                       int mb, T alpha);
+                       int mb, T alpha, T *wstep = nullptr);
+template <typename T>
+void launch_trsm_step(hipStream_t s, T *tiles, long bsiz, int ntiles, const T *lkk, const T *winv, int mb, int st, T *wstep);
 
 template <typename T>
 void launch_gemm_nt_tile(hipStream_t s, const T *A, const T *B, T *C, int mb, T alpha, T beta,
diff --git a/dense_linear_app_amd/csrc/dist.hip b/dense_linear_app_amd/csrc/dist.hip
--- a/dense_linear_app_amd/csrc/dist.hip
+++ b/dense_linear_app_amd/csrc/dist.hip
@@ -117,15 +117,17 @@
     HIPRC(hipStreamWaitEvent(r.st[st], r.events[ev], 0));
     return 0;
   }
+  T *wstep(int k, bool fused) { return fused ? (T *)wstep_set(r, k & 1, g.mb, sizeof(T)) : nullptr; }
   int panel(int k, char *lkk, void *wv, char *tiles, int ntiles, int ev_steps, int ev_head, const SyrkPipe *sy,
-            const int *wait_sem, int wait_target) {
+            const int *wait_sem, int wait_target, bool fused) {
     launch_panel_pipelined<T>(r.st[ST_PANEL], r.st[ST_TRSM], &r.events[ev_steps], (T *)lkk, g.mb, (T *)wv, r.d_info,
                               k * g.mb, (T *)tiles, (long)g.mb * g.mb, ntiles, ev_head >= 0 ? r.events[ev_head] : nullptr,
-                              sy, wait_sem, wait_target);
+                              sy, wait_sem, wait_target, nullptr, wstep(k, fused));
     return launched();
   }
-  int trsm(int, char *tiles, int ntiles, const char *lkk, const char *wv, int st) {
-    launch_trsm_panel<T>(r.st[st], (T *)tiles, (long)g.mb * g.mb, ntiles, (const T *)lkk, (const T *)wv, g.mb, T(1));
+  int trsm(int k, char *tiles, int ntiles, const char *lkk, const char *wv, int st, bool fused) {
+    launch_trsm_panel<T>(r.st[st], (T *)tiles, (long)g.mb * g.mb, ntiles, (const T *)lkk, (const T *)wv, g.mb, T(1),
+                         st == ST_TRSM ? wstep(k, fused) : nullptr);
     return launched();
   }
   int diag_syrk(int, int, char *Cjj, const char *A, int st) {
@@ -191,11 +193,11 @@
   int begin(int, int, int) { return 0; }
   int rec(int, int) { return 0; }
   int wt(int, int) { return 0; }
-  int panel(int k, char *lkk, void *, char *, int ntiles, int, int, const SyrkPipe *, const int *, int) {
+  int panel(int k, char *lkk, void *, char *, int ntiles, int, int, const SyrkPipe *, const int *, int, bool) {
     WRC(cb.potrf(cb.ctx, k, lkk));
     return ntiles > 0 ? cb.trsm(cb.ctx, k, lkk) : 0;
   }
-  int trsm(int k, char *, int, const char *lkk, const char *, int) { return cb.trsm(cb.ctx, k, lkk); }
+  int trsm(int k, char *, int, const char *lkk, const char *, int, bool) { return cb.trsm(cb.ctx, k, lkk); }
   int diag_syrk(int k, int j, char *, const char *A, int) {
     std::vector<const void *> hb(g.P, A);
     std::vector<int> hf(g.P, 0);
diff --git a/dense_linear_app_amd/csrc/kernels.hip b/dense_linear_app_amd/csrc/kernels.hip
--- a/dense_linear_app_amd/csrc/kernels.hip
+++ b/dense_linear_app_amd/csrc/kernels.hip
@@ -1,5 +1,6 @@
 #include "cholmi_internal.h"
 #include "mfma_traits.h"
+#include "nn_blocks.h"
 
 #include <type_traits>
 
@@ -554,6 +555,24 @@
   }
 }
 
+template <typename T>
+__device__ __forceinline__ void w8_store(T *Cout, int ld, typename Tr<T>::acc_t (&acc)[4][2]) {
+  using vec_t = typename Tr<T>::vec_t;
+  const int t = threadIdx.x, lane = t & 63, w = t >> 6, wr = w & 1, wc = w >> 1, i = lane & 15, q = lane >> 4;
+  const int m0 = wr * 64 + 2 * i;
+#pragma unroll
+  for (int b = 0; b < 2; ++b)
+#pragma unroll
+    for (int r = 0; r < 4; ++r) {
+      T *col = Cout + (long)(wc * 32 + 2 * (q + 4 * r) + b) * ld + m0;
+#pragma unroll
+      for (int g = 0; g < 2; ++g) {
+        const vec_t v = {acc[2 * g][b][r], acc[2 * g + 1][b][r]};
+        *reinterpret_cast<vec_t *>(col + 32 * g) = v;
+      }
+    }
+}
+
 constexpr int BKF = 32;
 struct alignas(16) SmemF {
   float a[2][BKF][MACRO];
@@ -650,6 +669,18 @@
     }
 }
 
+__device__ __forceinline__ void w8f_store(float *Cout, int ld, f4_t (&acc)[4][2]) {
+  const int t = threadIdx.x, lane = t & 63, w = t >> 6, wr = w & 1, wc = w >> 1, i = lane & 15, q = lane >> 4;
+  const int m0 = wr * 64 + 4 * i;
+#pragma unroll
+  for (int b = 0; b < 2; ++b)
+#pragma unroll
+    for (int r = 0; r < 4; ++r) {
+      const f4_t v = {acc[0][b][r], acc[1][b][r], acc[2][b][r], acc[3][b][r]};
+      *reinterpret_cast<f4_t *>(Cout + (long)(wc * 32 + 2 * (4 * q + r) + b) * ld + m0) = v;
+    }
+}
+
 template <typename T_, int MODE>
 struct CoreW8 {
   using T = T_;
@@ -663,6 +694,7 @@
   static __device__ __forceinline__ void epilogue(const T *Cin, T *Cout, int ld, Acc &acc, bool lower) {
     w8_epilogue<T, OOP>(Cin, Cout, ld, acc, lower);
   }
+  static __device__ __forceinline__ void store(T *Cout, int ld, Acc &acc) { w8_store<T>(Cout, ld, acc); }
 };
 struct CoreW8F {
   using T = float;
@@ -676,6 +708,7 @@
   static __device__ __forceinline__ void epilogue(const float *Cin, float *Cout, int ld, Acc &acc, bool lower) {
     w8f_epilogue<OOP>(Cin, Cout, ld, acc, lower);
   }
+  static __device__ __forceinline__ void store(float *Cout, int ld, Acc &acc) { w8f_store(Cout, ld, acc); }
 };
 
 template <typename Core>
@@ -853,6 +886,62 @@
   nt_kloop_paired<T>(Ap, mb, Bp, mb, MACRO, acc, sm);
   nt_epilogue_paired<T>(Cp, mb, acc, T(-1), beta, false);
   guest.leave();
+}
+
+template <typename T>
+__global__ __launch_bounds__(256, 2) void k_step_factor(const T *__restrict__ lkk, int mb, int st,
+                                                        const T *__restrict__ winv, T *__restrict__ W, int *ytab,
+                                                        const int *wait_sem = nullptr, int *fail = nullptr) {
+  sem_wait(wait_sem, 1, fail);
+  GuestOnCu guest(ytab);
+  __builtin_amdgcn_s_setprio(2);
+  const int c = blockIdx.x;
+  const T *Wi = winv + (long)st * MACRO * MACRO;
+  T *out = W + (long)c * MACRO * MACRO;
+  if (c == st) {
+    for (int e = threadIdx.x; e < MACRO * MACRO * (int)sizeof(T) / 16; e += 256)
+      reinterpret_cast<uint4 *>(out)[e] = reinterpret_cast<const uint4 *>(Wi)[e];
+  } else {
+    const int w = threadIdx.x >> 6, i0 = 64 * (w & 1), j0 = 64 * (w >> 1);
+    Acc<T> acc;
+    acc_zero<T>(acc);
+    nn_acc<T, false, false>(Wi, MACRO, lkk + (long)st * MACRO + (long)c * MACRO * mb, mb, i0, j0, 0, MACRO, acc);
+    acc_store<T>(out, MACRO, i0, j0, acc, T(-1));
+  }
+  guest.leave();
+}
+
+template <typename Core>
+__device__ __forceinline__ void panel_step_block(typename Core::T *tiles, long bsiz, int mb, int nbm, int st,
+                                                 const typename Core::T *W, int *ytab, int *head_sem,
+                                                 typename Core::Smem &sm) {
+  using T = typename Core::T;
+  GuestOnCu guest(ytab);
+  __builtin_amdgcn_s_setprio(2);
+  const int tix = blockIdx.x / nbm, r = blockIdx.x % nbm;
+  T *row = tiles + (long)tix * bsiz + r * MACRO;
+  typename Core::Acc acc;
+#pragma unroll
+  for (int a = 0; a < 4; ++a)
+#pragma unroll
+    for (int b = 0; b < 2; ++b)
+#pragma unroll
+      for (int q = 0; q < 4; ++q) acc[a][b][q] = T(0);
+  Core::kloop(row, mb, W, MACRO, MACRO * (st + 1), acc, sm, nullptr);
+  Core::store(row + (long)st * MACRO * mb, mb, acc);
+  guest.leave();
+  if (tix == 0) sem_signal(head_sem);
+}
+template <typename T, int MODE>
+__global__ __launch_bounds__(512, 4) void k_panel_step_w8(T *tiles, long bsiz, int mb, int nbm, int st,
+                                                           const T *__restrict__ W, int *ytab, int *head_sem = nullptr) {
+  __shared__ SmemR<T> sm;
+  panel_step_block<CoreW8<T, MODE>>(tiles, bsiz, mb, nbm, st, W, ytab, head_sem, sm);
+}
+__global__ __launch_bounds__(512, 4) void k_panel_step_w8f(float *tiles, long bsiz, int mb, int nbm, int st,
+                                                            const float *__restrict__ W, int *ytab, int *head_sem = nullptr) {
+  __shared__ SmemF sm;
+  panel_step_block<CoreW8F>(tiles, bsiz, mb, nbm, st, W, ytab, head_sem, sm);
 }
 
 constexpr int SK = 32;
@@ -2160,6 +2249,8 @@
 int g_flow_fences = 0;
 int g_poll_max_wgs = 48;
 int g_trsm_small_max = 64;
+int g_trsm_fused = 1;
+long long g_trsm_fused_steps = 0;
 
 struct UpdateGrid {
   int unit;
@@ -2231,7 +2322,7 @@
 };
 template <typename T>
 int trsm_step(hipStream_t s, T *tiles, long bsiz, int ntiles, const T *lkk, const T *winv, int mb, int st,
-              T alpha, const StepSems &sm = StepSems()) {
+              T alpha, const StepSems &sm = StepSems(), T *wstep = nullptr) {
   const int nbm = mb / MACRO, nc = nbm - 1 - st;
   if (alpha == T(1) && ntiles * nbm <= g_trsm_small_max) {
     const bool p1 = poll_in_kernel(s, sm.diag, 1, sm.fail, (long)ntiles * nbm * 4);
@@ -2245,6 +2336,17 @@
           p2 ? sm.intile : nullptr, sm.intile_target, sm.fail);
     }
     return 4 * nbm;
+  }
+  if (wstep && g_trsm_fused && alpha == T(1)) {
+    T *W = wstep + (long)MACRO * MACRO * (st * (st + 1) / 2);
+    ++g_trsm_fused_steps;
+    const bool pf = poll_in_kernel(s, sm.diag, 1, sm.fail, st + 1);
+    k_step_factor<T><<<st + 1, 256, 0, s>>>(lkk, mb, st, winv, W, g_ytab, pf ? sm.diag : nullptr, sm.fail);
+    if constexpr (sizeof(T) == 4)
+      k_panel_step_w8f<<<ntiles * nbm, 512, 0, s>>>(tiles, bsiz, mb, nbm, st, W, g_ytab, sm.head);
+    else
+      k_panel_step_w8<T, 1><<<ntiles * nbm, 512, 0, s>>>(tiles, bsiz, mb, nbm, st, W, g_ytab, sm.head);
+    return nbm;
   }
   const bool p1 = poll_in_kernel(s, sm.diag, 1, sm.fail, (long)ntiles * nbm);
   k_panel_solve<T><<<ntiles * nbm, 256, 0, s>>>(tiles, bsiz, mb, nbm, 0, st, winv, st == 0 ? alpha : T(1), g_ytab,
@@ -2294,7 +2396,7 @@
 template <typename T>
 void launch_panel_pipelined(hipStream_t sp, hipStream_t st, hipEvent_t *ev, T *lkk, int mb, T *winv,
                             int *d_info, int info_base, T *tiles, long bsiz, int ntiles, hipEvent_t ev_head,
-                            const SyrkPipe *sy, const int *wait_sem, int wait_target, int *tile_sem) {
+                            const SyrkPipe *sy, const int *wait_sem, int wait_target, int *tile_sem, T *wstep) {
   const int nbm = mb / MACRO;
   const bool pipe = sy && ntiles > 0;
   const bool fused_plain = !pipe && tile_sem && g_intile_fused && nbm > 1;
@@ -2337,7 +2439,7 @@
       ss.intile_target = (flow ? 8 : 4) * nr;
       ss.head = sy->c ? slot(2 * nbm + s) : nullptr;
       ss.fail = d_info;
-      const int head_wgs = trsm_step<T>(st, tiles, bsiz, ntiles, lkk, winv, mb, s, T(1), ss);
+      const int head_wgs = trsm_step<T>(st, tiles, bsiz, ntiles, lkk, winv, mb, s, T(1), ss, wstep);
       if (!sy->c) continue;
       const T *xs = tiles + (long)s * MACRO * mb;
       const int n64 = mb / 64;
@@ -2350,14 +2452,15 @@
     }
     (void)hipEventRecord(ev[s], sp);
     (void)hipStreamWaitEvent(st, ev[s], 0);
-    trsm_step<T>(st, tiles, bsiz, ntiles, lkk, winv, mb, s, T(1));
+    trsm_step<T>(st, tiles, bsiz, ntiles, lkk, winv, mb, s, T(1), StepSems(), wstep);
   }
   if (ev_head) (void)hipEventRecord(ev_head, st);
 }
 template void launch_panel_pipelined<double>(hipStream_t, hipStream_t, hipEvent_t *, double *, int, double *,
-                                             int *, int, double *, long, int, hipEvent_t, const SyrkPipe *, const int *, int, int *);
+                                             int *, int, double *, long, int, hipEvent_t, const SyrkPipe *, const int *, int, int *,
+                                             double *);
 template void launch_panel_pipelined<float>(hipStream_t, hipStream_t, hipEvent_t *, float *, int, float *, int *,
-                                            int, float *, long, int, hipEvent_t, const SyrkPipe *, const int *, int, int *);
+                                            int, float *, long, int, hipEvent_t, const SyrkPipe *, const int *, int, int *, float *);
 
 template <typename T>
 void launch_invert_diag(hipStream_t s, const T *tile, int mb, T *winv) {
@@ -2382,10 +2485,15 @@
 
 template <typename T>
 void launch_trsm_panel(hipStream_t s, T *tiles, long bsiz, int ntiles, const T *lkk, const T *winv,
-                       int mb, T alpha) {
+                       int mb, T alpha, T *wstep) {
   if (ntiles <= 0) return;
   const int nbm = mb / MACRO;
-  for (int st = 0; st < nbm; ++st) trsm_step<T>(s, tiles, bsiz, ntiles, lkk, winv, mb, st, alpha);
+  for (int st = 0; st < nbm; ++st) trsm_step<T>(s, tiles, bsiz, ntiles, lkk, winv, mb, st, alpha, StepSems(), wstep);
+}
+
+template <typename T>
+void launch_trsm_step(hipStream_t s, T *tiles, long bsiz, int ntiles, const T *lkk, const T *winv, int mb, int st, T *wstep) {
+  if (ntiles > 0) trsm_step<T>(s, tiles, bsiz, ntiles, lkk, winv, mb, st, T(1), StepSems(), wstep);
 }
 
 template <typename T>
@@ -2500,7 +2608,8 @@
   template void launch_diag_syrk<T>(hipStream_t, T *, const T *, int);                               \
   template void launch_invert_diag<T>(hipStream_t, const T *, int, T *);                            \
   template void launch_invert_diag_batch<T>(hipStream_t, const T *, long, int, int, T *);            \
-  template void launch_trsm_panel<T>(hipStream_t, T *, long, int, const T *, const T *, int, T);    \
+  template void launch_trsm_panel<T>(hipStream_t, T *, long, int, const T *, const T *, int, T, T *); \
+  template void launch_trsm_step<T>(hipStream_t, T *, long, int, const T *, const T *, int, int, T *); \
   template void launch_gemm_nt_tile<T>(hipStream_t, const T *, const T *, T *, int, T, T, bool);    \
   template void launch_gemm_nt_batch<T>(hipStream_t, const T *, long, int, const T *, long, int, T *, long, long, \
                                         int, T, T);                                                 \
diff --git a/dense_linear_app_amd/csrc/sched_check.hip b/dense_linear_app_amd/csrc/sched_check.hip
--- a/dense_linear_app_amd/csrc/sched_check.hip
+++ b/dense_linear_app_amd/csrc/sched_check.hip
@@ -49,7 +49,7 @@
   TraceOps(const WaveGeo &geo, bool profiling) : g(geo), prof(profiling) {
     for (int &l : last_on) l = -1;
     local_slots = (long)g.lmt * std::max(1, g.lnt);
-    next_slot = local_slots + 2;
+    next_slot = local_slots + 4;
   }
   bool profiling() const { return prof; }
   bool pipe_ok() const { return true; }
@@ -61,6 +61,8 @@
   static int stream_id(void *s) { return (int)reinterpret_cast<uintptr_t>(s) - 1; }
   char *tile(int il, int jl) { return fake_base + ((size_t)il + (size_t)jl * g.lmt) * g.tile_bytes; }
   void *winv(int par) { return fake_base + (size_t)(local_slots + par) * g.tile_bytes; }
+  void *wstep(int k) { return fake_base + (size_t)(local_slots + 2 + (k & 1)) * g.tile_bytes; }
+  int fused_trsm = 0;
   void *alloc(size_t bytes) {
     char *p = fake_base + (size_t)next_slot * g.tile_bytes;
     next_slot += (long)((bytes + g.tile_bytes - 1) / g.tile_bytes);
@@ -81,8 +83,10 @@
       snprintf(b, sizeof b, "tile (%d,%d)", il * g.P + g.pr, jl * g.Q + g.pc);
     } else if (t < local_slots + 2) {
       snprintf(b, sizeof b, "block inverses %ld", t - local_slots);
+    } else if (t < local_slots + 4) {
+      snprintf(b, sizeof b, "fused-step factors %ld", t - local_slots - 2);
     } else {
-      snprintf(b, sizeof b, "receive buffer slot %ld", t - local_slots - 2);
+      snprintf(b, sizeof b, "receive buffer slot %ld", t - local_slots - 4);
     }
     return b;
   }
@@ -134,7 +138,8 @@
     pending[st].insert(it->second.begin(), it->second.end());
     return 0;
   }
-  int panel(int k, char *lkk, void *wv, char *tiles, int ntiles, int, int ev_head, const SyrkPipe *sy, const int *wait_sem, int) {
+  int panel(int k, char *lkk, void *wv, char *tiles, int ntiles, int, int ev_head, const SyrkPipe *sy, const int *wait_sem, int,
+            bool fused) {
     std::vector<int> extra;
     if (wait_sem && ngates++ != drop_gate) {
       auto it = producer.find(wait_sem);
@@ -170,7 +175,8 @@
     touch(acc, lkk, g.tile_bytes, false);
     touch(acc, wv, std::max<size_t>(1, g.winv_bytes), false);
     touch(acc, tiles, (size_t)ntiles * g.tile_bytes, true);
-    const int trsm = add(1u << ST_TRSM, "TRSM(" + std::to_string(k) + ")", acc, after);
+    if (fused) touch(acc, wstep(k), 1, true), ++fused_trsm;
+    const int trsm = add(1u << ST_TRSM, "TRSM(" + std::to_string(k) + ")" + (fused ? " [fused steps]" : ""), acc, after);
     cost_of(trsm, 'T', t_panel / g.nbm + 0.5 * ntiles * t_tile / g.nbm);
     if (ev_head >= 0) ev_deps[ev_head] = {trsm};
     if (sy && sy->c && sy->su) {
@@ -183,12 +189,14 @@
     }
     return 0;
   }
-  int trsm(int k, char *tiles, int ntiles, const char *lkk, const char *wv, int st) {
+  int trsm(int k, char *tiles, int ntiles, const char *lkk, const char *wv, int st, bool fused) {
     Acc acc;
     touch(acc, lkk, g.tile_bytes, false);
     touch(acc, wv, std::max<size_t>(1, g.winv_bytes), false);
     touch(acc, tiles, (size_t)ntiles * g.tile_bytes, true);
-    cost_of(add(1u << st, "TRSM(" + std::to_string(k) + ") of " + std::to_string(ntiles) + " tiles [received diagonal tile]", acc), 'T',
+    if (fused) touch(acc, wstep(k), 1, true), ++fused_trsm;
+    cost_of(add(1u << st, "TRSM(" + std::to_string(k) + ") of " + std::to_string(ntiles) + " tiles [received diagonal tile]" +
+                              (fused ? " [fused steps]" : ""), acc), 'T',
             std::max(t_panel / g.nbm * g.nbm * 0.5, 0.5 * ntiles * t_tile));
     return 0;
   }
@@ -357,8 +365,8 @@
   std::string out;
   for (auto &f : ops.findings) out += f + "\n";
   char tail[200];
-  snprintf(tail, sizeof tail, "%zu launches, %d event waits, %d counter edges, %d flow-form waves, %zu findings\n", ops.ops.size(), ops.nwaits,
-           ops.ngates, w.flow_waves, ops.findings.size());
+  snprintf(tail, sizeof tail, "%zu launches, %d event waits, %d counter edges, %d flow-form waves, %zu findings, %d fused-step TRSM launches\n",
+           ops.ops.size(), ops.nwaits, ops.ngates, w.flow_waves, ops.findings.size(), ops.fused_trsm);
   out += tail;
   if (!ops.dropped.empty()) out += ops.dropped + "\n";
   if (report && cap > 0) snprintf(report, (size_t)cap, "%s", out.size() < (size_t)cap ? out.c_str() : out.substr(out.size() - cap + 1).c_str());
diff --git a/dense_linear_app_amd/csrc/spd.hip b/dense_linear_app_amd/csrc/spd.hip
--- a/dense_linear_app_amd/csrc/spd.hip
+++ b/dense_linear_app_amd/csrc/spd.hip
@@ -85,6 +85,7 @@
   T *Z = scr, *Wt = scr + (size_t)nr * nt * bs, *Tt = Wt + bs, *tmp = Tt + (size_t)nt * bs;
   hipStream_t s = main_stream();
   T *winv = reinterpret_cast<T *>(main_rank_ctx()->winv);
+  T *wstep = reinterpret_cast<T *>(wstep_for_panel(*main_rank_ctx(), WSTEP_MAIN, nr, mb, sizeof(T)));
   auto Ltile = [&](int i, int j) { return La + ((long)i + (long)j * A->lmt) * bs; };
   auto Ztile = [&](int r, int i) { return Z + ((long)r + (long)i * nr) * bs; };
   auto Dtile = [&](int k) { return udiag ? udiag + (long)k * bs : Ltile(k, k); };
@@ -92,7 +93,7 @@
     launch_tiles_transpose<T>(s, Bm + (long)r * B->lmt * bs, bs, Ztile(r, 0), (long)nr * bs, mb, nt);
   for (int k = 0; k < nt; ++k) {
     launch_invert_diag<T>(s, Dtile(k), mb, winv);
-    launch_trsm_panel<T>(s, Ztile(0, k), bs, nr, Dtile(k), winv, mb, T(1));
+    launch_trsm_panel<T>(s, Ztile(0, k), bs, nr, Dtile(k), winv, mb, T(1), wstep);
     launch_gemm_nt_batch<T>(s, Ztile(0, k), bs, nr, Ltile(k + 1, k), bs, nt - 1 - k, Ztile(0, k + 1), bs, (long)nr * bs, mb,
                             T(-1), T(1));
   }
@@ -1063,7 +1064,8 @@
       const int nr = nt - 1 - k;
       T *P = tile(Am, k + 1, k);
       T *Lt = tile(Bm, k + 1, k);
-      launch_trsm_panel<T>(s, P, bs, nr, tile(Bm, k, k), W + (long)k * nbm * blk, e, T(1));
+      launch_trsm_panel<T>(s, P, bs, nr, tile(Bm, k, k), W + (long)k * nbm * blk, e, T(1),
+                           reinterpret_cast<T *>(wstep_for_panel(*main_rank_ctx(), WSTEP_MAIN, nr, e, sizeof(T))));
       launch_gemm_nt_batch<T>(s, Lt, bs, nr, Cs, 0, 1, P, bs, 0, e, T(-0.5), T(1));
       if ((rc = pm.mark(P_CHAIN))) return rc;
       update_cols(launch_syr2k_update<T>, A, k + 1, nt, one_panel(tile(Am, 0, k)), one_panel(tile(Bm, 0, k)));
@@ -1123,7 +1125,8 @@
     const int nr = nt - 1 - k;
     launch_ldl_tile<T>(s, tile(k, k), e, Wt, Lc, winv, dv + (long)k * e, rv + (long)k * e, d_info, k * mb, pmax);
     if (nr > 0) {
-      launch_trsm_panel<T>(s, tile(k + 1, k), bs, nr, tile(k, k), winv, e, T(1));
+      launch_trsm_panel<T>(s, tile(k + 1, k), bs, nr, tile(k, k), winv, e, T(1),
+                           reinterpret_cast<T *>(wstep_for_panel(*main_rank_ctx(), WSTEP_MAIN, nr, e, sizeof(T))));
       launch_ldl_scale<T>(s, tile(k + 1, k), Wscr, (long)nr * bs, bs, e, rv + (long)k * e, pmax);
     }
     HIPCHECK(hipGetLastError());
diff --git a/dense_linear_app_amd/csrc/walker.h b/dense_linear_app_amd/csrc/walker.h
--- a/dense_linear_app_amd/csrc/walker.h
+++ b/dense_linear_app_amd/csrc/walker.h
@@ -301,6 +301,7 @@
         paired = mb <= PAIR_MAX_MB && k + 2 < nt && (double)local_tiles * t_tile >= sw.pair_fac * t_panel;
       const bool plain_yield = (double)local_tiles * t_tile < sw.yfac * t_panel;
       const bool chain_bound = (double)local_tiles * t_tile < sw.pipe_fac * t_panel;
+      const bool trsm_fused = !plain_yield;
       const bool pipe = flags && !paired && !last && o.pipe_ok() && plain_yield && chain_bound;
       const bool pipe_local = flags_local && !paired && o.pipe_ok() && plain_yield && chain_bound && own_diag && cntm > 0;
       const bool flow = pipe && own_diag && cntm > 0 && flow_ctl_lines(nbm) > 0 && o.flow_ok() && flow_applies(nbm) &&
@@ -329,7 +330,7 @@
         }
         const bool head_mine = !last && P == 1;
         WRC(o.panel(k, lkk, o.winv(par), lkk + g.tile_bytes, cntm, ev_steps, head_mine ? ev(k, E_HEAD) : -1,
-                    pipe || pipe_local ? &sy : nullptr, wait_sem, wait_target));
+                    pipe || pipe_local ? &sy : nullptr, wait_sem, wait_target, trsm_fused));
         if (mr && P > 1 && !last) {
           WRC(o.rec(ev(k, E_LKK), ST_PANEL));
           WRC(diag_send(k, lkk, (const char *)o.winv(par)));
@@ -347,11 +348,11 @@
         const char *lkk = lkk_buf[par], *wv = lkk_buf[par] + g.tile_bytes;
         const bool head_mine = !last && g.pr == (k + 1) % P;
         if (head_mine && cntm > 1 && o.can_split_trsm()) {
-          WRC(o.trsm(k, tiles, 1, lkk, wv, ST_TRSM));
+          WRC(o.trsm(k, tiles, 1, lkk, wv, ST_TRSM, trsm_fused));
           WRC(o.rec(ev(k, E_HEAD), ST_TRSM));
-          WRC(o.trsm(k, tiles + g.tile_bytes, cntm - 1, lkk, wv, ST_TRSM));
+          WRC(o.trsm(k, tiles + g.tile_bytes, cntm - 1, lkk, wv, ST_TRSM, trsm_fused));
         } else {
-          WRC(o.trsm(k, tiles, cntm, lkk, wv, ST_TRSM));
+          WRC(o.trsm(k, tiles, cntm, lkk, wv, ST_TRSM, trsm_fused));
           if (head_mine) WRC(o.rec(ev(k, E_HEAD), ST_TRSM));
         }
       }
diff --git a/include/cholmi.h b/include/cholmi.h
--- a/include/cholmi.h
+++ b/include/cholmi.h
@@ -165,6 +165,8 @@
 
 int chol_debug_calibration(double *out8);
 int chol_debug_update_kernel(int dtype, char *buf, int buflen);
+int chol_debug_trsm_panel(int dtype, void *tiles, int ntiles, const void *lkk, int mb, int step, int fused);
+long long chol_debug_trsm_fused_steps(void);
 int chol_debug_device_counters(void);
 
 void *chol_desc_local_ptr(chol_desc_t *desc, size_t *bytes);
```
